# thunlp/OpenMatch

Measured on AMD Instinct MI355X. Metric: passages/sec encode (bert-base DPR bi-encoder, 128 tok -> 768-d) [+ queries/sec exact top-1000 over 8.8M x 768 in `search`], higher is better.
Workload: dtype f16; 1 GPU; bert-base DPR bi-encoder encode+search, MS MARCO 8.8M x 128-tok -> 768-d (BASELINE configs[1]); seq_len=128, global_batch=1024, index_rows=8841823, queries=6980, topk=1000, weights=random-init BertConfig() seed 0, parallelism=shard1

## Files before the change

### include/openmatch_hip.h

```cpp
#ifndef OPENMATCH_HIP_H
#define OPENMATCH_HIP_H

#include <stddef.h>
#include <stdint.h>

#ifdef __cplusplus
extern "C" {
#endif

#define OM_ABI_VERSION 6

#define OM_F32 0
#define OM_BF16 1
#define OM_F16 2

#define OM_ACT_NONE 0
#define OM_ACT_GELU_ERF 1
#define OM_ACT_RELU 2
#define OM_ACT_GELU_TANH 3
#define OM_ACT_SILU 5
#define OM_ACT_MUL_RESID 0x100
#define OM_ACT_PRE_GRAD 0x200

#define OM_ARCH_BERT 0
#define OM_ARCH_T5 1
#define OM_ARCH_MODERNBERT 2

#define OM_ARCH_CAUSAL 3

#define OM_ARCH_NOMICBERT 4

#define OM_POOL_NONE 0
#define OM_POOL_FIRST 1
#define OM_POOL_MEAN 2
#define OM_POOL_LAST 3

#define OM_SEARCH_F32 0
#define OM_SEARCH_F16_RESCORE 1

const char* om_last_error(void);
int om_abi_version(void);

int om_device_count(void);

#define OM_TIMING_GEMM_BF16 0
#define OM_TIMING_GEMM_F32 1
#define OM_TIMING_SCAN 2
void om_debug_gemm_trace(unsigned long long* buf);
void om_debug_gemm_gen(int gen);
#define OM_GEMM_FAMILY_V1 1
#define OM_GEMM_FAMILY_V2 2
#define OM_GEMM_FAMILY_V6 6
#define OM_GEMM_FAMILY_G7 7
#define OM_GEMM_FAMILY_G7_ONE_TILE 70
#define OM_GEMM_FAMILY_G7C16 71
#define OM_GEMM_FAMILY_G7R16 72
#define OM_GEMM_FAMILY_SKINNY 9
int om_debug_gemm_last(void);
int om_debug_gemm_plan(int in_dtype, const void* A, int64_t lda, const void* B, int64_t ldb, int out_dtype, void* C, int64_t ldc,
                       int64_t M, int64_t N, int64_t K, const float* bias, const void* resid, int64_t ldr, int act);
typedef struct OmDebugGemmEpilogue {
  const float* bias; const void* resid; int64_t ldr; int act;
  void* pre_act; int64_t ldp; float drop_p; uint64_t seed; const int* drop_rows;
  const float* ln_stats; const float* ln_colsum; const float* rln_stats; const float* rln_g; const float* rln_b; float* stats_out;
  const void* resid_lo; void* out_lo;
  const float* resid32; float* out32;
  const float* a_ln32; const float* a_ln_g; const float* a_ln_b; float* a_ln_stats_out; const float* rln32; const float* rln32_stats;
  int lo8; float ln_inv_h, ln_eps; int ln_rms; int reverse;
  const int* rows_dev;
} OmDebugGemmEpilogue;
int om_debug_gemm_ex(int in_dtype, const void* A, int64_t lda, const void* B, int64_t ldb, int out_dtype, void* C, int64_t ldc,
                     int64_t M, int64_t N, int64_t K, const OmDebugGemmEpilogue* ep, void* stream);
int om_debug_gemm_plan_ex(int in_dtype, const void* A, int64_t lda, const void* B, int64_t ldb, int out_dtype, void* C, int64_t ldc,
                          int64_t M, int64_t N, int64_t K, const OmDebugGemmEpilogue* ep);
int om_debug_gemm_splitk(int in_dtype, const void* A, int64_t lda, const void* B, int64_t ldb, float* C, int64_t ldc, int64_t M,
                         int64_t N, int64_t K, void* stream);
#define OM_OPT_ENCODER_FUSED_LN 0
#define OM_OPT_ENCODER_DEBUG 1
#define OM_OPT_ATTENTION_FAST 2
#define OM_OPT_SCAN_GEN7 3
#define OM_OPT_SCAN_GROWTH 4
#define OM_OPT_WGRAD_DEBUG 5
#define OM_OPT_GEMM_GROUP_M 6
#define OM_OPT_SCAN_QGROUP 7
#define OM_OPT_TRAIN_WGRAD_STREAM 8
#define OM_OPT_ATTENTION_DEBUG 9
#define OM_OPT_ENCODER_PINGPONG 10
#define OM_OPT_ENCODER_TWO_PLANE 11
#define OM_OPT_GEMM_VARIANT 12
#define OM_OPT_SEARCH_DEBUG 13
#define OM_OPT_TRAIN_WGRAD_BATCH 14
#define OM_OPT_GEMM_MAX_GRID 15
#define OM_OPT_GEMM_CONT 16
#define OM_OPT_TRAIN_TAPE_GRAD 17
#define OM_OPT_TRAIN_RES32 18
#define OM_OPT_GEMM_SKINNY_M 19
#define OM_OPT_GEMM_SKINNY_CFG 20
#define OM_OPT_FEW_ROWS_LN_FUSE 21
#define OM_OPT_ENCODER_SKIP_PAD 22
#define OM_OPT_ENCODER_CLS_TAIL 23
#define OM_OPT_COUNT 24
int om_debug_option(int opt, int value);
int om_debug_option_value(int opt);
int om_debug_attention(const void* qkv, void* ctx, const int64_t* mask, int64_t B, int L, int H, int heads, void* stream);
int om_debug_attention_ex(int dtype, const void* qkv, void* ctx, const int64_t* mask, const float* pos_bias, int64_t B, int L, int H,
                          int heads, float scale, float drop_p, uint64_t seed, void* stream, int reverse, const int* kmax,
                          const int* cu, int w);
int om_debug_rope(int dtype, void* qkv, int64_t M, int L, int H, float theta, void* stream);
int om_debug_rope_rows(int dtype, void* qkv, int64_t rows, int L, int H, float theta, const int* row_map, void* stream);
int om_debug_swiglu_rows(int dtype, const void* in, void* out, int64_t M, int F, void* stream);
int om_debug_embed(int dtype, const int64_t* ids, const int64_t* type_ids, const float* word, const float* pos, const float* type,
                   const float* g, const float* b, void* out, int64_t M, int L, int H, int vocab, int type_vocab, float eps, void* stream);
int om_debug_attention_causal(int dtype, const void* qkv, void* ctx, const int64_t* mask, int64_t B, int L, int n_heads, int n_kv_heads,
                              float scale, void* stream);
int om_debug_rope_gqa(int dtype, void* qkv, int64_t M, int L, int n_heads, int n_kv_heads, const float* inv_freq, float scaling, void* stream);
int om_debug_attention_causal_packed(int dtype, const void* qkv, void* ctx, const int64_t* mask, const int* cu, int64_t B, int L, int n_heads,
                                     int n_kv_heads, float scale, void* stream);
int om_debug_rope_gqa_rows(int dtype, void* qkv, int64_t rows, int L, int n_heads, int n_kv_heads, const float* inv_freq, float scaling,
                           const int* row_map, void* stream);
int om_debug_attention_causal_hd(int dtype, const void* qkv, void* ctx, const int64_t* mask, int64_t B, int L, int n_heads, int n_kv_heads,
                                 int head_dim, float scale, void* stream);
int om_debug_attention_causal_hd_packed(int dtype, const void* qkv, void* ctx, const int64_t* mask, const int* cu, int64_t B, int L,
                                        int n_heads, int n_kv_heads, int head_dim, float scale, void* stream);
int om_debug_qknorm_rope(int dtype, void* qkv, int64_t M, int L, int n_heads, int n_kv_heads, int head_dim, const float* q_norm_g,
                         const float* k_norm_g, float eps, const float* inv_freq, float scaling, void* stream);
int om_debug_qknorm_rope_rows(int dtype, void* qkv, int64_t rows, int L, int n_heads, int n_kv_heads, int head_dim, const float* q_norm_g,
                              const float* k_norm_g, float eps, const float* inv_freq, float scaling, const int* row_map, void* stream);
int om_debug_attention_gqa_d256(int dtype, const void* qkv, void* ctx, const int64_t* mask, int64_t B, int L, int n_heads, int n_kv_heads,
                                float scale, int w, void* stream);
int om_debug_qknorm_rope_d256(int dtype, void* qkv, int64_t M, int L, int n_heads, int n_kv_heads, const float* q_norm_g, const float* k_norm_g,
                              float eps, const float* inv_freq, float scaling, void* stream);
int om_debug_attention_gqa_d256_packed(int dtype, const void* qkv, void* ctx, const int64_t* mask, const int* cu, int64_t B, int L, int n_heads,
                                       int n_kv_heads, float scale, int w, void* stream);
int om_debug_qknorm_rope_d256_rows(int dtype, void* qkv, int64_t rows, int L, int n_heads, int n_kv_heads, const float* q_norm_g,
                                   const float* k_norm_g, float eps, const float* inv_freq, float scaling, const int* row_map, void* stream);
int om_debug_rmsnorm_add(int dtype, const void* h, int64_t ldh, float* x, int64_t ldx, const float* g, int64_t M, int H, float eps, void* stream);
int om_debug_mask_extent(const int64_t* mask, int64_t B, int L, int* kmax, void* stream);
int om_debug_pack_rows(const int* kmax, int64_t B, int L, int64_t rows, int* cu, int* cls_rows, int* row_map, void* stream);
#define OM_ATTN_FAMILY_GENERIC 1
#define OM_ATTN_FAMILY_FWD16 2
#define OM_ATTN_FAMILY_FWD16_KMAX4 3
#define OM_ATTN_FAMILY_FWD16C 4
#define OM_ATTN_FAMILY_LONG 5
#define OM_ATTN_FAMILY_D32 6
#define OM_ATTN_FAMILY_BAND16 7
#define OM_ATTN_FAMILY_BAND32 8
int om_debug_attention_last(void);
int om_debug_attention_plan(int dtype, int64_t B, int L, int H, int heads, int has_bias, float drop_p, int has_kmax, int has_cu, int w);
#define OM_ATTN_BWD_FAMILY_BWD16 1
#define OM_ATTN_BWD_FAMILY_GENERIC 2
#define OM_ATTN_BWD_FAMILY_LONG 3
#define OM_ATTN_BWD_FAMILY_D32 4
int om_debug_attention_bwd_last(void);
int om_debug_attention_bwd_plan(int dtype, int64_t B, int L, int H, int heads, int has_bias, int has_drel, int has_cu, int packed);
int om_debug_attention_bwd_ex(int dtype, const void* qkv, const void* ctx, const void* dctx, void* dqkv, const int64_t* mask,
                              const float* pos_bias, float* drel, float* stats, int64_t B, int L, int H, int heads, float scale,
                              float drop_p, uint64_t seed, const int* cu, int packed, void* stream);
size_t om_debug_attention_bwd_stats_bytes(int64_t B, int heads);
#define OM_ENC_PATH_BERT_FUSED 1
#define OM_ENC_PATH_BERT_PENDING_LN 2
#define OM_ENC_PATH_BERT_FEW32 3
#define OM_ENC_PATH_BERT_PLAIN 4
#define OM_ENC_PATH_MODERNBERT 5
#define OM_ENC_PATH_T5_FUSED 6
#define OM_ENC_PATH_T5_PLAIN 7
struct OmEncoderConfig;
int om_debug_encoder_plan(const struct OmEncoderConfig* cfg, int gated_ffn, int has_rel_bias, int64_t B, int64_t L, int64_t packed_rows,
                          int want_hidden);
int om_debug_encoder_skip_pad(const struct OmEncoderConfig* cfg, int gated_ffn, int has_rel_bias, int64_t B, int64_t L, int want_hidden);
int om_debug_encoder_cls_tail(const struct OmEncoderConfig* cfg, int gated_ffn, int has_rel_bias, int64_t B, int64_t L, int64_t packed_rows,
                              int want_hidden);
int om_debug_gather_rows(const void* src0, void* dst0, const void* src1, void* dst1, const void* src2, void* dst2, const float* stats_src,
                         float* stats_dst, const int* rows, int64_t B, int64_t L, int64_t Mc, int H, void* stream);
int om_debug_attn_drop_keep(uint64_t seed, int64_t b, int h, int heads, int Lm, int q, int key, float p);
int om_debug_wave_sum_check(const float* in, float* out_shuffle, float* out_dpp, int64_t groups, void* stream);
#define OM_ROW_FWD_GENERIC 1
#define OM_ROW_FWD_X8 2
#define OM_ROW_LN_BWD 3
int om_debug_row_kernel_last(void);
int om_debug_layernorm(int dtype, const void* x, int64_t ldx, void* y, int64_t ldy, const float* g, const float* b, int64_t M, int H,
                       float eps, int rms, const void* x_lo, int lo8, void* stream);
int om_debug_layernorm_f32out(int dtype, const void* x, int64_t ldx, float* y, int64_t ldy, const float* g, const float* b, int64_t M,
                              int H, float eps, int rms, const void* x_lo, const int* rows, int lo8, void* stream);
int om_debug_layernorm_from_f32(int dtype, const float* x, int64_t ldx, void* y, int64_t ldy, const float* g, const float* b, int64_t M,
                                int H, float eps, int rms, void* stream);
int om_debug_layernorm_dual(int dtype, const float* x, int64_t ldx, void* y, float* y32, int64_t ldy, const float* g, const float* b,
                            int64_t M, int H, float eps, void* stream);
int om_debug_norm_bwd(int dtype, const void* dy, const void* x, const float* g, void* dx, float* dg, float* db, int64_t M, int H,
                      float eps, int rms, const void* add, void* stream);
int om_debug_ln_bwd_drop(int dtype, const void* dy, const void* x, const float* g, void* dx, void* dx_drop, float drop_p,
                         uint64_t drop_seed, float* dg, float* db, int64_t M, int H, float eps, const float* dy32, const float* x32,
                         float* partial, int* partial_blocks , const int* drop_rows, void* stream);
typedef struct OmLnSite { const float* partial; float* dg; float* db; int blocks; } OmLnSite;
int om_debug_ln_param_reduce(const OmLnSite* sites , int n, int H, void* stream);
int om_debug_embed_bwd(int dtype, const void* dy, const int64_t* ids, const int64_t* type_ids, const float* word, const float* pos,
                       const float* type, const float* g, float* dword, float* dpos, float* dtype_, float* dg, float* db, int64_t M,
                       int L, int H, int vocab, int type_vocab, float eps, const int* cu, void* stream);
int om_debug_pool(int dtype, const void* x, const int64_t* mask, float* out, int64_t B, int L, int H, int mode, const int* cu,
                  void* stream);
int om_debug_pool_bwd(int dtype, const float* dp, const int64_t* mask, void* dh, int64_t B, int L, int H, int mode, const int* cu,
                      void* stream);
int om_debug_l2norm(const float* x, float* y, int64_t M, int D, void* stream);
int om_debug_l2norm_bwd(const float* x, const float* dy, float* dx, int64_t M, int D, void* stream);
int om_debug_colsum(int dtype, const void* x, int64_t ld, int64_t M, int N, float* out, void* stream);
int om_debug_dropout(int dtype, const void* x, void* y, int64_t n, float p, uint64_t seed, const int* rows, int H, void* stream);
int om_debug_ln_fold(int dtype, const void* W, const float* gamma, const float* beta, const float* b, void* Wf, float* colsum,
                     float* bf, int N, int K, void* stream);
int om_debug_ln_stats_reduce(const float* slots, int nslots, int64_t M, float* out, void* stream);
int om_kernel_timing_enable(int enable);
int om_kernel_timing_read(int kernel_class, double* total_ms, int64_t* launches, double* flops);

int om_gemm_nt(int in_dtype, const void* A, int64_t lda, const void* B, int64_t ldb,
               int out_dtype, void* C, int64_t ldc, int64_t M, int64_t N, int64_t K,
               const float* bias, const void* resid, int64_t ldr, int act, void* stream);

int om_gemm_tn_acc(int in_dtype, const void* A, int64_t lda, const void* B, int64_t ldb,
                   float* C, int64_t ldc, float* bias, int64_t M, int64_t N, int64_t K, void* stream);

typedef struct OmTnProblem {
  const void* A; const void* B; float* C; float* bias;
  int64_t lda, ldb, ldc, N, K;
} OmTnProblem;
int om_gemm_tn_acc_batch(int in_dtype, const OmTnProblem* problems, int n, int64_t M, void* stream);

typedef struct OmLayerWeights {
  const void* qkv_w;
  const float* qkv_b;
  const void* o_w;
  const float* o_b;
  const float* ln1_g;
  const float* ln1_b;
  const void* ffn1_w;
  const float* ffn1_b;
  const void* ffn1g_w;
  const void* ffn2_w;
  const float* ffn2_b;
  const float* ln2_g;
  const float* ln2_b;
} OmLayerWeights;

typedef struct OmEncoderConfig {
  int arch;
  int dtype;
  int hidden;
  int n_layers;
  int n_heads;
  int head_dim;
  int ffn;
  int vocab;
  int max_pos;
  int type_vocab;
  int act;
  float ln_eps;
  int rel_buckets;
  int rel_max_dist;
  int pooling;
  int head_in;
  int head_out;
  int normalize;
  float rope_theta_global;
  float rope_theta_local;
  int half_window;
  uint64_t sliding_layers;
} OmEncoderConfig;

typedef struct OmEncoderWeights {
  const float* word_emb;
  const float* pos_emb;
  const float* type_emb;
  const float* emb_ln_g;
  const float* emb_ln_b;
  const OmLayerWeights* layers_host;
  const float* final_ln_g;
  const float* rel_bias;
  const float* head_w;
  const void* folded;
  const float* final_ln_b;
} OmEncoderWeights;

size_t om_encoder_fold_bytes(const OmEncoderConfig* cfg);
int om_encoder_fold_weights(const OmEncoderConfig* cfg, const OmEncoderWeights* w, void* folded, size_t bytes, void* stream);

size_t om_encoder_workspace_bytes(const OmEncoderConfig* cfg, int64_t B, int64_t L);

int om_t5_relative_bucket(int relative_position, int num_buckets, int max_distance);

int om_encoder_forward(const OmEncoderConfig* cfg, const OmEncoderWeights* w,
                       const int64_t* input_ids, const int64_t* attention_mask,
                       const int64_t* token_type_ids, int64_t B, int64_t L,
                       void* out_hidden, float* out_reps, void* workspace,
                       size_t workspace_bytes, void* stream);

int om_encoder_packed_supported(const OmEncoderConfig* cfg, int gated_ffn, int64_t B, int64_t L, int64_t packed_rows);
size_t om_encoder_workspace_bytes_packed(const OmEncoderConfig* cfg, int64_t B, int64_t L, int64_t packed_rows);
int om_encoder_forward_packed(const OmEncoderConfig* cfg, const OmEncoderWeights* w,
                              const int64_t* input_ids, const int64_t* attention_mask,
                              const int64_t* token_type_ids, int64_t B, int64_t L, int64_t packed_rows,
                              float* out_reps, void* workspace, size_t workspace_bytes, void* stream);

typedef struct OmCausalConfig {
  OmEncoderConfig base;
  int n_kv_heads;
  float rope_attention_scaling;
  float inv_freq[32];
} OmCausalConfig;
size_t om_causal_encoder_workspace_bytes(const OmCausalConfig* cfg, int64_t B, int64_t L);
int om_causal_encoder_forward(const OmCausalConfig* cfg, const OmEncoderWeights* w, const int64_t* input_ids,
                              const int64_t* attention_mask, int64_t B, int64_t L, void* out_hidden, float* out_reps,
                              void* workspace, size_t workspace_bytes, void* stream);
int om_causal_encoder_packed_supported(const OmCausalConfig* cfg, int64_t B, int64_t L, int64_t packed_rows);
size_t om_causal_encoder_workspace_bytes_packed(const OmCausalConfig* cfg, int64_t B, int64_t L, int64_t packed_rows);
int om_causal_encoder_forward_packed(const OmCausalConfig* cfg, const OmEncoderWeights* w, const int64_t* input_ids,
                                     const int64_t* attention_mask, int64_t B, int64_t L, int64_t packed_rows, float* out_reps,
                                     void* workspace, size_t workspace_bytes, void* stream);

typedef struct OmCausalConfig2 {
  OmCausalConfig base;
  int qk_norm;
  int reserved;
  float inv_freq[64];
} OmCausalConfig2;
typedef struct OmCausalQkNorm {
  const float* q_norm_g;
  const float* k_norm_g;
} OmCausalQkNorm;
size_t om_causal2_encoder_workspace_bytes(const OmCausalConfig2* cfg, int64_t B, int64_t L);
int om_causal2_encoder_forward(const OmCausalConfig2* cfg, const OmEncoderWeights* w, const OmCausalQkNorm* qk_norm_host,
                               const int64_t* input_ids, const int64_t* attention_mask, int64_t B, int64_t L, void* out_hidden,
                               float* out_reps, void* workspace, size_t workspace_bytes, void* stream);
int om_causal2_encoder_packed_supported(const OmCausalConfig2* cfg, int64_t B, int64_t L, int64_t packed_rows);
size_t om_causal2_encoder_workspace_bytes_packed(const OmCausalConfig2* cfg, int64_t B, int64_t L, int64_t packed_rows);
int om_causal2_encoder_forward_packed(const OmCausalConfig2* cfg, const OmEncoderWeights* w, const OmCausalQkNorm* qk_norm_host,
                                      const int64_t* input_ids, const int64_t* attention_mask, int64_t B, int64_t L, int64_t packed_rows,
                                      float* out_reps, void* workspace, size_t workspace_bytes, void* stream);

#define OM_ARCH_GEMMA3 5
typedef struct OmGemma3Config {
  OmCausalConfig base;
  float attn_scale;
  int half_window;
  uint64_t sliding_layers;
  float full_scaling;
  float sliding_scaling;
  float attn_logit_softcapping;
  int bidirectional;
  float full_inv_freq[128];
  float sliding_inv_freq[128];
} OmGemma3Config;
typedef struct OmGemma3Norms {
  const float* q_norm_g;
  const float* k_norm_g;
  const float* post_attention_norm_g;
  const float* post_feedforward_norm_g;
} OmGemma3Norms;
size_t om_gemma3_encoder_workspace_bytes(const OmGemma3Config* cfg, int64_t B, int64_t L);
int om_gemma3_encoder_forward(const OmGemma3Config* cfg, const OmEncoderWeights* w, const OmGemma3Norms* norms_host, const int64_t* input_ids,
                              const int64_t* attention_mask, int64_t B, int64_t L, void* out_hidden, float* out_reps, void* workspace,
                              size_t workspace_bytes, void* stream);
int om_gemma3_encoder_packed_supported(const OmGemma3Config* cfg, int64_t B, int64_t L, int64_t packed_rows);
size_t om_gemma3_encoder_workspace_bytes_packed(const OmGemma3Config* cfg, int64_t B, int64_t L, int64_t packed_rows);
int om_gemma3_encoder_forward_packed(const OmGemma3Config* cfg, const OmEncoderWeights* w, const OmGemma3Norms* norms_host,
                                     const int64_t* input_ids, const int64_t* attention_mask, int64_t B, int64_t L, int64_t packed_rows,
                                     float* out_reps, void* workspace, size_t workspace_bytes, void* stream);

typedef struct OmT5DecoderLayer {
  const void* sa_v_w;
  const void* sa_o_w;
  const float* sa_ln_g;
  const void* ca_q_w;
  const void* ca_kv_w;
  const void* ca_o_w;
  const float* ca_ln_g;
  const void* ffn1_w;
  const void* ffn1g_w;
  const void* ffn2_w;
  const float* ffn_ln_g;
} OmT5DecoderLayer;
typedef struct OmT5DecoderWeights {
  const float* start_emb;
  const float* final_ln_g;
  const OmT5DecoderLayer* layers_host;
  int n_layers;
} OmT5DecoderWeights;
size_t om_t5_decoder_workspace_bytes(const OmEncoderConfig* cfg, int64_t B, int64_t L);
int om_t5_decoder_step(const OmEncoderConfig* cfg, const OmT5DecoderWeights* w, const void* enc_hidden,
                       const int64_t* attention_mask, int64_t B, int64_t L, float* out_hidden,
                       void* workspace, size_t workspace_bytes, void* stream);

typedef struct OmT5DecoderLayerGrads {
  float* sa_v_w;  float* sa_o_w; float* sa_ln_g;
  float* ca_q_w;  float* ca_kv_w; float* ca_o_w; float* ca_ln_g;
  float* ffn1_w;  float* ffn1g_w; float* ffn2_w; float* ffn_ln_g;
} OmT5DecoderLayerGrads;
typedef struct OmT5DecoderGrads {
  float* start_emb;
  float* final_ln_g;
  const OmT5DecoderLayerGrads* layers_host;
} OmT5DecoderGrads;
size_t om_t5_decoder_tape_bytes(const OmEncoderConfig* cfg, int n_layers, int64_t B, int64_t L);
size_t om_t5_decoder_train_workspace_bytes(const OmEncoderConfig* cfg, int n_layers, int64_t B, int64_t L);
int om_t5_decoder_train_forward(const OmEncoderConfig* cfg, const OmT5DecoderWeights* w, const void* enc_hidden,
                                const int64_t* attention_mask, int64_t B, int64_t L, float dropout, uint64_t seed,
                                void* tape, size_t tape_bytes, float* out_hidden, void* workspace,
                                size_t workspace_bytes, void* stream);
int om_t5_decoder_train_backward(const OmEncoderConfig* cfg, const OmT5DecoderWeights* w, const void* enc_hidden,
                                 const int64_t* attention_mask, int64_t B, int64_t L, float dropout, uint64_t seed,
                                 const void* tape, const float* d_out, const OmT5DecoderGrads* grads,
                                 void* d_enc_hidden, void* workspace, size_t workspace_bytes, void* stream);

int om_linear_f32_backward(const float* dy, const float* x, const float* w, float* dw, float* dx, int B, int D, int K,
                           void* stream);

typedef struct OmLayerGrads {
  float* qkv_w;  float* qkv_b;  float* o_w;    float* o_b;   float* ln1_g; float* ln1_b;
  float* ffn1_w; float* ffn1_b; float* ffn2_w; float* ffn2_b; float* ln2_g; float* ln2_b;
  float* ffn1g_w;
} OmLayerGrads;

typedef struct OmEncoderGrads {
  float* word_emb; float* pos_emb; float* type_emb; float* emb_ln_g; float* emb_ln_b;
  const OmLayerGrads* layers_host;
  float* head_w;
  float* final_ln_g;
  float* rel_bias;
} OmEncoderGrads;

size_t om_encoder_tape_bytes(const OmEncoderConfig* cfg, int64_t B, int64_t L);
size_t om_encoder_train_workspace_bytes(const OmEncoderConfig* cfg, int64_t B, int64_t L);

int om_encoder_train_forward(const OmEncoderConfig* cfg, const OmEncoderWeights* w,
                             const int64_t* input_ids, const int64_t* attention_mask,
                             const int64_t* token_type_ids, int64_t B, int64_t L,
                             float hidden_dropout, float attn_dropout, uint64_t seed, void* tape,
                             size_t tape_bytes, float* out_reps, void* workspace,
                             size_t workspace_bytes, void* stream);

int om_encoder_train_backward(const OmEncoderConfig* cfg, const OmEncoderWeights* w,
                              const int64_t* input_ids, const int64_t* attention_mask,
                              const int64_t* token_type_ids, int64_t B, int64_t L,
                              float hidden_dropout, float attn_dropout, uint64_t seed,
                              const void* tape, const float* d_reps, const OmEncoderGrads* grads,
                              void* workspace, size_t workspace_bytes, void* stream);

int om_encoder_train_packed_supported(const OmEncoderConfig* cfg, int64_t B, int64_t L, int64_t packed_rows);
size_t om_encoder_tape_bytes_packed(const OmEncoderConfig* cfg, int64_t B, int64_t L, int64_t packed_rows);
size_t om_encoder_train_workspace_bytes_packed(const OmEncoderConfig* cfg, int64_t B, int64_t L, int64_t packed_rows);
int om_encoder_train_forward_packed(const OmEncoderConfig* cfg, const OmEncoderWeights* w,
                                    const int64_t* input_ids, const int64_t* attention_mask,
                                    const int64_t* token_type_ids, int64_t B, int64_t L, int64_t packed_rows,
                                    float hidden_dropout, float attn_dropout, uint64_t seed,
                                    void* tape, size_t tape_bytes, float* out_reps,
                                    void* workspace, size_t workspace_bytes, void* stream);
int om_encoder_train_backward_packed(const OmEncoderConfig* cfg, const OmEncoderWeights* w,
                                     const int64_t* input_ids, const int64_t* attention_mask,
                                     const int64_t* token_type_ids, int64_t B, int64_t L, int64_t packed_rows,
                                     float hidden_dropout, float attn_dropout, uint64_t seed,
                                     const void* tape, const float* d_reps, const OmEncoderGrads* grads,
                                     void* workspace, size_t workspace_bytes, void* stream);

int om_encoder_train_forward_hidden(const OmEncoderConfig* cfg, const OmEncoderWeights* w,
                                    const int64_t* input_ids, const int64_t* attention_mask,
                                    const int64_t* token_type_ids, int64_t B, int64_t L,
                                    float hidden_dropout, float attn_dropout, uint64_t seed, void* tape,
                                    size_t tape_bytes, void* out_hidden, void* workspace,
                                    size_t workspace_bytes, void* stream);
int om_encoder_train_backward_hidden(const OmEncoderConfig* cfg, const OmEncoderWeights* w,
                                     const int64_t* input_ids, const int64_t* attention_mask,
                                     const int64_t* token_type_ids, int64_t B, int64_t L,
                                     float hidden_dropout, float attn_dropout, uint64_t seed,
                                     const void* tape, const void* d_hidden, const OmEncoderGrads* grads,
                                     void* workspace, size_t workspace_bytes, void* stream);

int om_encoder_train_set_layer_events(void* const* events, int n);

#define OM_ADAM_CHUNK 16384
typedef struct OmAdamTensor {
  float* p; const float* g; float* m; float* v;
  void* shadow0; void* shadow1;
  int64_t n;
  float weight_decay;
  int shadow0_dtype, shadow1_dtype, reserved;
} OmAdamTensor;
int om_grad_sqnorm(const OmAdamTensor* tensors, const int32_t* chunks, int n_chunks, float* partial, float* out_sq, void* stream);
int om_adamw_step(const OmAdamTensor* tensors, const int32_t* chunks, int n_chunks, float lr, float beta1, float beta2, float eps,
                  int64_t step, const float* gnorm_sq, float max_norm, float grad_scale, int skip_nonfinite,
                  const float* scale_state ,
                  void* stream);
int om_loss_scale_update(const float* gnorm_sq, float* state4, int growth_interval, void* stream);


int om_index_to_f16(const float* rows_f32, int64_t N, int d, void* rows_f16, float* stats,
                    void* stream);

size_t om_sim_topk_workspace_bytes(int64_t n_queries, int d, int k);

int om_sim_topk(int mode, const float* queries, int64_t n_queries, const float* index_f32,
                const void* index_f16, const float* stats, int64_t N, int d, int k,
                int64_t id_offset, float* out_scores, int64_t* out_ids, void* workspace,
                size_t workspace_bytes, void* stream);

void om_sim_topk_info(int64_t out[8]);

#define OM_SCAN_FAMILY_GENERIC 1
#define OM_SCAN_FAMILY_WIDE 2
#define OM_SCAN_FAMILY_STREAM32 3
#define OM_SCAN_FAMILY_STREAM16 4
int om_debug_scan_plan(int half, int64_t nq, int d, int out[4]);
int om_debug_sim_stream(const void* rows16, int64_t nrows, uint32_t row_base, const void* queries16, int64_t nq, int d, const float* thr,
                        uint64_t* keys, unsigned* cnt, int grid, void* stream);

int om_topk_merge(const float* part_scores, const int64_t* part_ids, int W, int64_t n_queries,
                  int k_in, int k_out, float* out_scores, int64_t* out_ids, void* stream);

int om_contrastive_fwd_bwd(const float* q, const float* p, int Qg, int Pg, int d, int n_psg,
                           float loss_scale, int q_row0, int q_rows, int p_row0, int p_rows,
                           float* loss, float* scores, float* d_q, float* d_p, float* workspace,
                           void* stream);

int om_contrastive_fwd_bwd_ex(const float* q, const float* p, int Qg, int Pg, int d, const int64_t* target, int n_psg,
                              int reduction, const float* row_grad, float loss_scale, int q_row0, int q_rows,
                              int p_row0, int p_rows, float* loss, float* scores, float* d_q, float* d_p,
                              float* workspace, void* stream);

#define OM_COMM_ID_BYTES 128
int om_comm_unique_id(void* id128);
int om_comm_init(const void* id128, int world, int rank, void** comm);
int om_comm_destroy(void* comm);
int om_comm_count(void* comm, int* count);
int om_allgather_rows(void* comm, const void* send, void* recv, int64_t rows, int64_t row_bytes, void* stream);
int om_allreduce_grads(void* comm, float* buf, int64_t n, int average, void* stream);
int om_exchange_topk(void* comm, int world, const float* D, const int64_t* I, int64_t q_block, int k, float* recvD,
                     int64_t* recvI, void* stream);

#ifdef __cplusplus
}
#endif
#endif
```

### openmatch_amd/csrc/abi.cpp

```cpp
#include "common.h"

static thread_local std::string g_last_error;
void om_set_error(const std::string& msg) { g_last_error = msg; }

extern "C" const char* om_last_error(void) { return g_last_error.c_str(); }
extern "C" int om_abi_version(void) { return OM_ABI_VERSION; }
extern "C" int om_device_count(void) {
  int n = 0;
  hipError_t e = hipGetDeviceCount(&n);
  if (e != hipSuccess) {
    om_set_error(std::string("hipGetDeviceCount: ") + hipGetErrorString(e));
    return -1;
  }
  return n;
}

#include <mutex>
#include <vector>
namespace {
struct Span { hipEvent_t a, b; };
struct ClassStat { std::vector<Span> spans; double flops = 0; size_t used = 0; };
bool g_timing = false;
ClassStat g_stat[3];
std::mutex g_mu;
}
bool om_timing_on() { return g_timing; }
void om_timing_begin(int c, hipStream_t s) {
  std::lock_guard<std::mutex> lk(g_mu);
  ClassStat& st = g_stat[c];
  if (st.used == st.spans.size()) {
    Span sp;
    (void)hipEventCreate(&sp.a);
    (void)hipEventCreate(&sp.b);
    st.spans.push_back(sp);
  }
  (void)hipEventRecord(st.spans[st.used].a, s);
}
void om_timing_end(int c, hipStream_t s, double flops) {
  std::lock_guard<std::mutex> lk(g_mu);
  ClassStat& st = g_stat[c];
  (void)hipEventRecord(st.spans[st.used].b, s);
  st.used++;
  st.flops += flops;
}
extern "C" int om_kernel_timing_enable(int enable) { g_timing = enable != 0; return 0; }
extern "C" int om_kernel_timing_read(int c, double* total_ms, int64_t* launches, double* flops) {
  if (c < 0 || c > 2) { om_set_error("om_kernel_timing_read: bad class"); return 1; }
  std::lock_guard<std::mutex> lk(g_mu);
  ClassStat& st = g_stat[c];
  double ms = 0;
  for (size_t i = 0; i < st.used; ++i) {
    hipError_t e = hipEventSynchronize(st.spans[i].b);
    float t = 0;
    if (e == hipSuccess) e = hipEventElapsedTime(&t, st.spans[i].a, st.spans[i].b);
    if (e != hipSuccess) { om_set_error(std::string("om_kernel_timing_read: ") + hipGetErrorString(e)); return 1; }
    ms += t;
  }
  if (total_ms) *total_ms = ms;
  if (launches) *launches = (int64_t)st.used;
  if (flops) *flops = st.flops;
  st.used = 0; st.flops = 0;
  return 0;
}

#include <atomic>
#include <map>
#include <tuple>
namespace {
std::atomic<int> g_opt[OM_OPT_COUNT];
std::atomic<bool> g_opt_init{false};
std::mutex g_opt_mu;
void opt_init() {
  std::lock_guard<std::mutex> lk(g_opt_mu);
  if (g_opt_init.load()) return;
  const char* e = getenv("OM_ENCODER_FUSED_LN");
  g_opt[OM_OPT_ENCODER_FUSED_LN] = e ? atoi(e) : 1;
  g_opt[OM_OPT_ENCODER_DEBUG] = getenv("OM_ENCODER_DEBUG") ? 1 : 0;
  e = getenv("OM_ATTENTION_FAST");
  g_opt[OM_OPT_ATTENTION_FAST] = e ? atoi(e) : 1;
  e = getenv("OM_SCAN_GEN7");
  g_opt[OM_OPT_SCAN_GEN7] = e ? atoi(e) : 1;
  e = getenv("OM_SCAN_GROWTH");
  g_opt[OM_OPT_SCAN_GROWTH] = e ? atoi(e) : 60;
  g_opt[OM_OPT_WGRAD_DEBUG] = 0;
  g_opt[OM_OPT_ATTENTION_DEBUG] = 0;
  e = getenv("OM_ENCODER_PINGPONG");
  g_opt[OM_OPT_ENCODER_PINGPONG] = e ? atoi(e) : 1;
  e = getenv("OM_TRAIN_WGRAD_STREAM");
  g_opt[OM_OPT_TRAIN_WGRAD_STREAM] = e ? atoi(e) : 1;
  e = getenv("OM_SCAN_QGROUP");
  g_opt[OM_OPT_SCAN_QGROUP] = e ? atoi(e) : 8;
  e = getenv("OM_GEMM_GROUP_M");
  g_opt[OM_OPT_GEMM_GROUP_M] = e ? atoi(e) : 8;
  e = getenv("OM_ENCODER_TWO_PLANE");
  g_opt[OM_OPT_ENCODER_TWO_PLANE] = e ? atoi(e) : 3;
  e = getenv("OM_GEMM_VARIANT");
  g_opt[OM_OPT_GEMM_VARIANT] = e ? atoi(e) : 0;
  e = getenv("OM_SEARCH_DEBUG");
  g_opt[OM_OPT_SEARCH_DEBUG] = e ? (atoi(e) ? atoi(e) : 1) : 0;
  e = getenv("OM_TRAIN_WGRAD_BATCH");
  g_opt[OM_OPT_TRAIN_WGRAD_BATCH] = e ? atoi(e) : 4;
  e = getenv("OM_GEMM_MAX_GRID");
  g_opt[OM_OPT_GEMM_MAX_GRID] = e ? atoi(e) : 0;
  e = getenv("OM_TRAIN_TAPE_GRAD");
  g_opt[OM_OPT_TRAIN_TAPE_GRAD] = e ? atoi(e) : 1;
  e = getenv("OM_TRAIN_RES32");
  g_opt[OM_OPT_TRAIN_RES32] = e ? atoi(e) : 1;
  e = getenv("OM_GEMM_CONT");
  g_opt[OM_OPT_GEMM_CONT] = e ? atoi(e) : 495;
  e = getenv("OM_GEMM_SKINNY_M");
  g_opt[OM_OPT_GEMM_SKINNY_M] = e ? atoi(e) : 1024;
  e = getenv("OM_FEW_ROWS_LN_FUSE");
  g_opt[OM_OPT_FEW_ROWS_LN_FUSE] = e ? atoi(e) : 64;
  e = getenv("OM_ENCODER_SKIP_PAD");
  g_opt[OM_OPT_ENCODER_SKIP_PAD] = e ? atoi(e) : 1;
  e = getenv("OM_ENCODER_CLS_TAIL");
  g_opt[OM_OPT_ENCODER_CLS_TAIL] = e ? atoi(e) : 1;
  g_opt_init.store(true);
}
}
bool om_option_is_set(int opt) {
  if (opt == OM_OPT_SCAN_GROWTH) return getenv("OM_SCAN_GROWTH") != nullptr;
  return false;
}
int om_option(int opt) {
  if (!g_opt_init.load(std::memory_order_acquire)) opt_init();
  return g_opt[opt].load(std::memory_order_relaxed);
}
extern "C" int om_debug_option(int opt, int value) {
  if (opt < 0 || opt >= OM_OPT_COUNT) { om_set_error("om_debug_option: unknown option"); return 1; }
  if (!g_opt_init.load(std::memory_order_acquire)) opt_init();
  g_opt[opt].store(value);
  return 0;
}
extern "C" int om_debug_option_value(int opt) {
  if (opt < 0 || opt >= OM_OPT_COUNT) { om_set_error("om_debug_option_value: unknown option"); return -1; }
  return om_option(opt);
}

int om_t5_lut_device(int L, int buckets, int max_dist, const int** out) {
  static std::mutex mu;
  static std::map<std::tuple<int, int, int, int>, int*> cache;
  int dev = 0;
  OM_HIP(hipGetDevice(&dev));
  std::lock_guard<std::mutex> lk(mu);
  auto key = std::make_tuple(dev, L, buckets, max_dist);
  auto it = cache.find(key);
  if (it == cache.end()) {
    std::vector<int> lut(2 * L);
    for (int rel = -(L - 1); rel <= L - 1; ++rel) lut[rel + (L - 1)] = om_t5_relative_bucket(rel, buckets, max_dist);
    int* d = nullptr;
    OM_HIP(hipMalloc(&d, (size_t)(2 * L) * sizeof(int)));
    OM_HIP(hipMemcpy(d, lut.data(), (size_t)(2 * L - 1) * sizeof(int), hipMemcpyHostToDevice));
    it = cache.emplace(key, d).first;
  }
  *out = it->second;
  return 0;
}
```

### openmatch_amd/csrc/encoder.hip

```cpp
#include <math.h>

#include <stdlib.h>

#include <algorithm>
#include <map>
#include <mutex>
#include <utility>
#include <vector>

#include "encoder_plan.h"

namespace {
struct FoldSlot { size_t w, cs, bf; };
struct FoldLayout { size_t per_layer, total; FoldSlot qkv, ffn1; };
FoldLayout fold_layout(const OmEncoderConfig* c) {
  const size_t H = c->hidden, F = enc_ffn1_cols(c);
  size_t off = 0;
  auto take = [&](size_t bytes) { size_t o = off; off = align_up(off + bytes, 256); return o; };
  FoldLayout L;
  L.qkv.w = take(3 * H * H * 2); L.qkv.cs = take(3 * H * 4); L.qkv.bf = take(3 * H * 4);
  L.ffn1.w = take(F * H * 2); L.ffn1.cs = take(F * 4); L.ffn1.bf = take(F * 4);
  L.per_layer = off;
  L.total = off * (size_t)c->n_layers;
  return L;
}
bool fold_applies(const OmEncoderConfig* c) {
  return c->arch != OM_ARCH_MODERNBERT && (c->dtype == OM_BF16 || c->dtype == OM_F16) && c->n_layers > 0 && c->hidden % 256 == 0 && c->ffn % 256 == 0;
}
}

extern "C" size_t om_encoder_fold_bytes(const OmEncoderConfig* cfg) {
  if (!cfg || !fold_applies(cfg)) return 0;
  return fold_layout(cfg).total;
}

extern "C" int om_encoder_fold_weights(const OmEncoderConfig* c, const OmEncoderWeights* w, void* blob, size_t bytes, void* stream) {
  if (!c || !w || !blob) OM_FAIL("null argument");
  if (!fold_applies(c)) OM_FAIL("nothing to fold for this configuration (om_encoder_fold_bytes is 0)");
  const FoldLayout L = fold_layout(c);
  if (bytes < L.total || ((uintptr_t)blob & 255)) OM_FAIL("fold buffer too small or not 256-byte aligned");
  const OmLayerWeights* Ls = w->layers_host;
  if (!Ls) OM_FAIL("layers_host is null");
  hipStream_t s = (hipStream_t)stream;
  const int H = c->hidden, F = enc_ffn1_cols(c);
  const bool bert = enc_bert_family(c);
  for (int l = 0; l < c->n_layers; ++l) {
    char* base = (char*)blob + (size_t)l * L.per_layer;
    const OmLayerWeights& lw = Ls[l];
    if (l > 0) {
      const float* g = bert ? Ls[l - 1].ln2_g : lw.ln1_g;
      const float* beta = bert ? Ls[l - 1].ln2_b : nullptr;
      if (omk_ln_fold(c->dtype, lw.qkv_w, g, beta, bert ? lw.qkv_b : nullptr, base + L.qkv.w, (float*)(base + L.qkv.cs),
                      (float*)(base + L.qkv.bf), 3 * H, H, s)) return 1;
    }
    if (!lw.ffn1g_w) {
      const float* g = bert ? lw.ln1_g : lw.ln2_g;
      const float* beta = bert ? lw.ln1_b : nullptr;
      if (omk_ln_fold(c->dtype, lw.ffn1_w, g, beta, bert ? lw.ffn1_b : nullptr, base + L.ffn1.w, (float*)(base + L.ffn1.cs),
                      (float*)(base + L.ffn1.bf), F, H, s)) return 1;
    }
  }
  return 0;
}

static int folded_weights(const OmEncoderConfig* c, const OmEncoderWeights* w, int layer, bool ffn1, const void* W, const float* g,
                          const float* beta, const float* b, int N, int K, void* scratch_w, float* scratch_cs, float* scratch_bf,
                          hipStream_t s, const void** Wf, const float** cs, const float** bf) {
  if (w->folded) {
    const FoldLayout L = fold_layout(c);
    const char* base = (const char*)w->folded + (size_t)layer * L.per_layer;
    const FoldSlot& sl = ffn1 ? L.ffn1 : L.qkv;
    *Wf = base + sl.w; *cs = (const float*)(base + sl.cs); *bf = (const float*)(base + sl.bf);
    return 0;
  }
  if (omk_ln_fold(c->dtype, W, g, beta, b, scratch_w, scratch_cs, scratch_bf, N, K, s)) return 1;
  *Wf = scratch_w; *cs = scratch_cs; *bf = scratch_bf;
  return 0;
}

struct EncWs {
  char *x, *y, *x1, *qkv, *ctx, *ff, *ff2;
  float *pooled, *headout, *posbias;
  float* final32;
  int* lut;
  int* kmax;
  int *cu, *cls_rows, *row_map;
  char* wfold;
  float *colsum, *bfold, *stats1, *stats2, *slots;
  char *y_lo, *x1_lo;
  float *r32a, *r32b, *y32;
  size_t total;
};

static EncWs carve(const OmEncoderConfig* c, const EncPlan& p, int64_t B, int64_t L, int64_t packed_rows, char* base) {
  const bool half = c->dtype == OM_BF16 || c->dtype == OM_F16;
  const size_t es = half ? 2 : 4;
  const size_t Mreal = (size_t)p.M, M = (size_t)p.Mp, H = c->hidden, F = c->ffn, F1 = enc_ffn1_cols(c);
  const bool bertf = enc_bert_family(c);
  size_t off = 0;
  auto take = [&](size_t bytes) { size_t o = off; off = align_up(off + bytes, 256); return base + o; };
  EncWs w;
  w.x = take(M * H * es);
  w.y = take(M * H * es);
  w.x1 = take(M * H * es);
  w.qkv = take(M * 3 * H * es);
  w.ctx = take(M * H * es);
  w.ff = take(M * F1 * es);
  w.ff2 = take(c->arch == OM_ARCH_T5 || c->arch == OM_ARCH_MODERNBERT || c->arch == OM_ARCH_NOMICBERT ? M * F * es : 0);
  w.pooled = (float*)take((size_t)B * H * 4);
  w.headout = (float*)take((size_t)B * (c->head_out > 0 ? c->head_out : 1) * 4);
  const bool rel = c->arch == OM_ARCH_T5 || (c->arch == OM_ARCH_BERT && c->rel_buckets > 0);
  w.posbias = (float*)take(rel ? (size_t)c->n_heads * L * L * 4 : 0);
  w.lut = (int*)take(rel ? (size_t)(2 * L) * 4 : 0);
  w.kmax = (int*)take((size_t)B * 4);
  w.cu = (int*)take(packed_rows > 0 ? (size_t)(B + 2) * 4 : 0);
  w.cls_rows = (int*)take(packed_rows > 0 ? (size_t)B * 4 : 0);
  w.row_map = (int*)take(packed_rows > 0 ? (size_t)packed_rows * 4 : 0);
  w.final32 = (float*)take(half && c->pooling != OM_POOL_NONE ? (c->pooling == OM_POOL_FIRST ? (size_t)B : Mreal) * H * 4 : 0);
  const bool fuse = half && c->arch != OM_ARCH_MODERNBERT;
  const size_t wide = std::max((size_t)3 * H, F1);
  w.wfold = take(fuse ? wide * H * es : 0);
  w.colsum = (float*)take(fuse ? wide * 4 : 0);
  w.bfold = (float*)take(fuse ? wide * 4 : 0);
  w.stats1 = (float*)take(fuse ? (size_t)2 * c->n_layers * M * 8 : 0);
  w.stats2 = w.stats1 ? w.stats1 + (size_t)c->n_layers * M * 2 : nullptr;
  w.slots = (float*)take(fuse ? (size_t)2 * ((H + 255) / 256) * M * 8 : 0);
  const bool two = fuse && bertf;
  w.y_lo = take(two ? M * H * es : 0);
  w.x1_lo = take(two ? M * H * es : 0);
  w.r32a = (float*)take(p.alloc_few32 ? Mreal * H * 4 : 0);
  w.r32b = (float*)take(p.alloc_few32 ? Mreal * H * 4 : 0);
  w.y32 = (float*)take(p.alloc_few32 ? Mreal * H * 4 : 0);
  w.total = off;
  return w;
}

static size_t workspace_bytes(const OmEncoderConfig* c, int64_t B, int64_t L, int64_t packed_rows) {
  const EncPlan p = encoder_plan_checked(EncPlanIn{c, B, L, packed_rows, false, false, false, false}, encoder_switches());
  return carve(c, p, B, L, packed_rows, nullptr).total;
}

extern "C" size_t om_encoder_workspace_bytes(const OmEncoderConfig* cfg, int64_t B, int64_t L) {
  if (!cfg || B <= 0 || L <= 0) return 0;
  return workspace_bytes(cfg, B, L, 0);
}

extern "C" size_t om_encoder_workspace_bytes_packed(const OmEncoderConfig* cfg, int64_t B, int64_t L, int64_t packed_rows) {
  if (!cfg || B <= 0 || L <= 0 || packed_rows <= 0) return 0;
  return workspace_bytes(cfg, B, L, packed_rows);
}

extern "C" int om_encoder_packed_supported(const OmEncoderConfig* c, int gated_ffn, int64_t B, int64_t L, int64_t packed_rows) {
  return encoder_packed_ok(c, gated_ffn != 0, B, L, packed_rows, encoder_switches()) ? 1 : 0;
}

extern "C" int om_debug_encoder_plan(const OmEncoderConfig* c, int gated_ffn, int has_rel_bias, int64_t B, int64_t L, int64_t packed_rows,
                                     int want_hidden) {
  if (!c) {
    om_set_error("om_debug_encoder_plan: null argument");
    return -1;
  }
  const EncPlan p = encoder_plan(EncPlanIn{c, B, L, packed_rows, want_hidden != 0, gated_ffn != 0, has_rel_bias != 0, c->type_vocab > 0},
                                 encoder_switches());
  if (p.error) {
    om_set_error(std::string("om_debug_encoder_plan: ") + p.error);
    return -1;
  }
  return p.path | (int)p.few_rows << 8 | (int)p.two << 9 | p.lo8 << 10;
}

extern "C" int om_debug_encoder_skip_pad(const OmEncoderConfig* c, int gated_ffn, int has_rel_bias, int64_t B, int64_t L, int want_hidden) {
  if (!c) {
    om_set_error("om_debug_encoder_skip_pad: null argument");
    return -1;
  }
  const EncPlanIn in = {c, B, L, 0, want_hidden != 0, gated_ffn != 0, has_rel_bias != 0, c->type_vocab > 0};
  const EncSwitches sw = encoder_switches();
  return encoder_skip_pad(in, encoder_plan(in, sw), sw) ? 1 : 0;
}

extern "C" int om_debug_encoder_cls_tail(const OmEncoderConfig* c, int gated_ffn, int has_rel_bias, int64_t B, int64_t L, int64_t packed_rows,
                                         int want_hidden) {
  if (!c) {
    om_set_error("om_debug_encoder_cls_tail: null argument");
    return -1;
  }
  const EncPlanIn in = {c, B, L, packed_rows, want_hidden != 0, gated_ffn != 0, has_rel_bias != 0, c->type_vocab > 0};
  const EncSwitches sw = encoder_switches();
  return encoder_cls_tail(in, encoder_plan(in, sw), sw) ? 1 : 0;
}

extern "C" int om_t5_relative_bucket(int relative_position, int num_buckets, int max_distance) {
  int nb = num_buckets / 2;
  int bucket = relative_position > 0 ? nb : 0;
  const int n = relative_position < 0 ? -relative_position : relative_position;
  const int max_exact = nb / 2;
  if (n < max_exact) return bucket + n;
  const double v = log((double)n / max_exact) / log((double)max_distance / max_exact) * (nb - max_exact);
  int large = max_exact + (int)v;
  if (large > nb - 1) large = nb - 1;
  return bucket + large;
}

static int check_cfg(const OmEncoderConfig* c) {
  if (const char* why = encoder_cfg_error(c)) OM_FAIL(why);
  return 0;
}

struct EncCall {
  const OmEncoderConfig* c;
  const OmEncoderWeights* w;
  const int64_t* mask;
  int64_t B, L;
  const EncPlan& p;
  const EncWs& ws;
  const float* posbias;
  const int* cu;
  const int* row_map;
  void* out_hidden;
  hipStream_t s;
  const int* rows_dev;
  int64_t cls_mc;
};

struct EncStream {
  const void* x;
  const void* x_lo;
  int lo8;
  const float *g, *b;
  int rms;
  void* spare;
  char* hidden;
  const float* rows32;
  bool cls_compact;
};

#define GEMM(A_, lda_, W_, ldw_, C_, ldc_, N_, K_, bias_, res_, ldr_, act_)                        \
  do {                                                                                             \
    if (om_gemm_nt(dt, A_, lda_, W_, ldw_, dt, C_, ldc_, Mg, N_, K_, bias_, res_, ldr_, act_, s)) \
      return 1;                                                                                    \
  } while (0)
#define RUN(expr) do { if (expr) return 1; } while (0)
#define ENC_LOCALS                                                                                                   \
  const OmEncoderConfig* c = k.c; const EncWs& ws = k.ws; const OmLayerWeights* Ls = k.w->layers_host; hipStream_t s = k.s;     \
  const int dt = c->dtype, H = c->hidden, F = c->ffn, nh = c->n_heads;                                              \
  const int64_t B = k.B, L = k.L, M = k.p.M, Mg = k.p.Mg
#define NOMIC_LOCALS                                                                                                 \
  const bool nomic = c->arch == OM_ARCH_NOMICBERT;                                                                   \
  const int F1 = enc_ffn1_cols(c), act1 = nomic ? OM_ACT_NONE : c->act;                                             \
  const void* const ffa = nomic ? ws.ff2 : ws.ff
#define NOMIC_ROPE() do { if (nomic) RUN(omk_rope(dt, ws.qkv, M, (int)L, H, c->rope_theta_global, s, k.row_map)); } while (0)
#define NOMIC_SWIGLU(rows_) do { if (nomic) RUN(omk_swiglu_rows(dt, ws.ff, ws.ff2, rows_, F, s)); } while (0)

static int bert_fused(const EncCall& k, EncStream* out) {
  ENC_LOCALS;
  NOMIC_LOCALS;
  const float scale = 1.0f / sqrtf((float)c->head_dim);
  const float inv_h = 1.0f / (float)H;
  const bool two = k.p.two;
  const int lo8 = k.p.lo8;
  const int nslots = 2 * (H / 256);
  const bool pingpong = k.p.pingpong;
  int walk = 1;
  const int64_t Mc = k.cls_mc;
  const size_t cplane = (size_t)Mc * H * 2;
  char* const cbase = ws.qkv;
  float* const cst2p = (float*)(cbase + 7 * cplane);
  float* const cst1 = cst2p + 2 * Mc;
  if (Mc > 0 && ((char*)(cst1 + 2 * Mc) > ws.qkv + (size_t)Mg * 3 * H * 2 || Mc > Mg || c->n_layers < 2 || lo8))
    OM_FAIL("[CLS] tail: the compact buffers do not fit the qkv area");
#define OM_WALK() (pingpong ? (walk ^= 1, walk ^ 1) : 0)
  for (int l = 0; l < c->n_layers; ++l) {
    const OmLayerWeights& lw = Ls[l];
    const bool last = l == c->n_layers - 1, tail = last && Mc > 0;
    float* st1 = tail ? cst1 : ws.stats1 + (size_t)l * Mg * 2;
    float* st2 = ws.stats2 + (size_t)l * Mg * 2;
    const float* st2p = l ? ws.stats2 + (size_t)(l - 1) * Mg * 2 : nullptr;
    const int64_t Mr = tail ? Mc : Mg;
    const int* const rdev = tail ? nullptr : k.rows_dev;
    const char *ctx = ws.ctx, *xin = ws.x1, *xin_lo = ws.x1_lo;
    char *y = ws.y, *y_lo = ws.y_lo, *xout = ws.x1, *xout_lo = ws.x1_lo;
    GemmEpilogue e = {};
    if (l == 0) {
      e.bias = lw.qkv_b; e.reverse = OM_WALK(); e.rows_dev = k.rows_dev;
      RUN(omk_gemm(dt, ws.x, H, lw.qkv_w, H, dt, ws.qkv, 3 * H, Mg, 3 * H, H, e, s));
    } else {
      const OmLayerWeights& pw = Ls[l - 1];
      const void* wf; const float *cs, *bfp;
      RUN(folded_weights(c, k.w, l, false, lw.qkv_w, pw.ln2_g, pw.ln2_b, lw.qkv_b, 3 * H, H, ws.wfold, ws.colsum, ws.bfold, s, &wf, &cs, &bfp));
      e.bias = bfp; e.ln_stats = st2p; e.ln_colsum = cs; e.ln_inv_h = inv_h; e.ln_eps = c->ln_eps; e.reverse = OM_WALK(); e.rows_dev = k.rows_dev;
      RUN(omk_gemm(dt, ws.x1, H, wf, H, dt, ws.qkv, 3 * H, Mg, 3 * H, H, e, s));
    }
    NOMIC_ROPE();
    RUN(omk_attention(dt, ws.qkv, ws.ctx, k.mask, k.posbias, B, (int)L, H, nh, scale, 0.f, 0, s, OM_WALK(), ws.kmax, k.cu));
    if (tail) {
      const GatherPlane planes[3] = {{ws.ctx, cbase}, {ws.x1, cbase + cplane}, {two ? ws.x1_lo : nullptr, cbase + 2 * cplane}};
      RUN(omk_gather_rows(planes, st2p, cst2p, k.cu ? ws.cls_rows : nullptr, B, L, Mc, H, s));
      ctx = cbase; xin = cbase + cplane; xin_lo = cbase + 2 * cplane; st2p = cst2p;
      y = cbase + 3 * cplane; y_lo = cbase + 4 * cplane; xout = cbase + 5 * cplane; xout_lo = cbase + 6 * cplane;
    }
    e = GemmEpilogue{};
    e.bias = lw.o_b; e.ldr = H; e.stats_out = ws.slots; e.ln_inv_h = inv_h; e.ln_eps = c->ln_eps;
    if (two) { e.out_lo = y_lo; e.lo8 = lo8; }
    if (l == 0) {
      e.resid = ws.x;
    } else {
      const OmLayerWeights& pw = Ls[l - 1];
      e.resid = xin; e.rln_stats = st2p; e.rln_g = pw.ln2_g; e.rln_b = pw.ln2_b;
      if (two) e.resid_lo = xin_lo;
    }
    e.reverse = OM_WALK(); e.rows_dev = rdev;
    RUN(omk_gemm(dt, ctx, H, lw.o_w, H, dt, y, H, Mr, H, H, e, s));
    RUN(omk_ln_stats_reduce(ws.slots, nslots, Mr, st1, s));
    const void* wf1; const float *cs1, *bf1;
    RUN(folded_weights(c, k.w, l, true, lw.ffn1_w, lw.ln1_g, lw.ln1_b, lw.ffn1_b, F1, H, ws.wfold, ws.colsum, ws.bfold, s, &wf1, &cs1, &bf1));
    e = GemmEpilogue{};
    e.bias = bf1; e.act = act1; e.ln_stats = st1; e.ln_colsum = cs1; e.ln_inv_h = inv_h; e.ln_eps = c->ln_eps;
    e.reverse = OM_WALK(); e.rows_dev = rdev;
    RUN(omk_gemm(dt, y, H, wf1, H, dt, ws.ff, F1, Mr, F1, H, e, s));
    NOMIC_SWIGLU(Mr);
    e = GemmEpilogue{};
    e.bias = lw.ffn2_b; e.resid = y; e.ldr = H; e.rln_stats = st1; e.rln_g = lw.ln1_g; e.rln_b = lw.ln1_b;
    e.stats_out = ws.slots; e.ln_inv_h = inv_h; e.ln_eps = c->ln_eps;
    if (two) { e.resid_lo = y_lo; e.out_lo = xout_lo; e.lo8 = lo8; }
    e.reverse = OM_WALK(); e.rows_dev = rdev;
    RUN(omk_gemm(dt, ffa, F, lw.ffn2_w, F, dt, xout, H, Mr, H, F, e, s));
    if (!last) RUN(omk_ln_stats_reduce(ws.slots, nslots, Mg, st2, s));
  }
#undef OM_WALK
  const OmLayerWeights& lastw = Ls[c->n_layers - 1];
  *out = EncStream{ws.x1, two ? ws.x1_lo : nullptr, lo8, lastw.ln2_g, lastw.ln2_b, 0, ws.x};
  if (Mc > 0) { out->x = cbase + 5 * cplane; out->x_lo = two ? cbase + 6 * cplane : nullptr; out->cls_compact = true; }
  return 0;
}

static int bert_pending_ln(const EncCall& k, EncStream* out) {
  ENC_LOCALS;
  NOMIC_LOCALS;
  const float scale = 1.0f / sqrtf((float)c->head_dim);
  float* const y_a = ws.y32;
  float* const y_b = ws.r32b;
  for (int l = 0; l < c->n_layers; ++l) {
    const OmLayerWeights& lw = Ls[l];
    float* const st1 = ws.stats1 + (size_t)l * M * 2;
    float* const st2p = l ? ws.stats2 + (size_t)(l - 1) * M * 2 : nullptr;
    GemmEpilogue e = {};
    e.bias = lw.qkv_b; e.ln_eps = c->ln_eps;
    if (l) { e.a_ln32 = y_b; e.a_ln_g = Ls[l - 1].ln2_g; e.a_ln_b = Ls[l - 1].ln2_b; e.a_ln_stats_out = st2p; }
    RUN(omk_gemm(dt, ws.x, H, lw.qkv_w, H, dt, ws.qkv, 3 * H, Mg, 3 * H, H, e, s));
    NOMIC_ROPE();
    RUN(omk_attention(dt, ws.qkv, ws.ctx, k.mask, k.posbias, B, (int)L, H, nh, scale, 0.f, 0, s, 0, ws.kmax));
    e = GemmEpilogue{};
    e.bias = lw.o_b; e.ldr = H; e.out32 = y_a; e.ln_eps = c->ln_eps;
    if (l) { e.rln32 = y_b; e.rln32_stats = st2p; e.rln_g = Ls[l - 1].ln2_g; e.rln_b = Ls[l - 1].ln2_b; }
    else e.resid32 = ws.r32a;
    RUN(omk_gemm(dt, ws.ctx, H, lw.o_w, H, dt, ws.y, H, Mg, H, H, e, s));
    e = GemmEpilogue{};
    e.bias = lw.ffn1_b; e.act = act1; e.ln_eps = c->ln_eps;
    e.a_ln32 = y_a; e.a_ln_g = lw.ln1_g; e.a_ln_b = lw.ln1_b; e.a_ln_stats_out = st1;
    RUN(omk_gemm(dt, ws.x1, H, lw.ffn1_w, H, dt, ws.ff, F1, Mg, F1, H, e, s));
    NOMIC_SWIGLU(Mg);
    e = GemmEpilogue{};
    e.bias = lw.ffn2_b; e.ldr = H; e.out32 = y_b; e.ln_eps = c->ln_eps;
    e.rln32 = y_a; e.rln32_stats = st1; e.rln_g = lw.ln1_g; e.rln_b = lw.ln1_b;
    RUN(omk_gemm(dt, ffa, F, lw.ffn2_w, F, dt, ws.y, H, Mg, H, F, e, s));
  }
  const OmLayerWeights& last = Ls[c->n_layers - 1];
  void* dst = k.out_hidden ? k.out_hidden : (void*)ws.x;
  RUN(omk_layernorm_dual(dt, y_b, H, dst, ws.r32a, H, last.ln2_g, last.ln2_b, M, H, c->ln_eps, s));
  *out = EncStream{};
  out->hidden = (char*)dst; out->rows32 = ws.r32a;
  return 0;
}

static int bert_few32(const EncCall& k, EncStream* out) {
  ENC_LOCALS;
  NOMIC_LOCALS;
  const float scale = 1.0f / sqrtf((float)c->head_dim);
  void* dst = ws.x;
  for (int l = 0; l < c->n_layers; ++l) {
    const OmLayerWeights& lw = Ls[l];
    GEMM(ws.x, H, lw.qkv_w, H, ws.qkv, 3 * H, 3 * H, H, lw.qkv_b, nullptr, 0, OM_ACT_NONE);
    NOMIC_ROPE();
    RUN(omk_attention(dt, ws.qkv, ws.ctx, k.mask, k.posbias, B, (int)L, H, nh, scale, 0.f, 0, s, 0, ws.kmax));
    GemmEpilogue e = {};
    e.bias = lw.o_b; e.resid32 = ws.r32a; e.ldr = H; e.out32 = ws.y32;
    RUN(omk_gemm(dt, ws.ctx, H, lw.o_w, H, dt, ws.y, H, Mg, H, H, e, s));
    RUN(omk_layernorm_dual(dt, ws.y32, H, ws.x1, ws.r32b, H, lw.ln1_g, lw.ln1_b, M, H, c->ln_eps, s));
    GEMM(ws.x1, H, lw.ffn1_w, H, ws.ff, F1, F1, H, lw.ffn1_b, nullptr, 0, act1);
    NOMIC_SWIGLU(Mg);
    e = GemmEpilogue{};
    e.bias = lw.ffn2_b; e.resid32 = ws.r32b; e.ldr = H; e.out32 = ws.y32;
    RUN(omk_gemm(dt, ffa, F, lw.ffn2_w, F, dt, ws.y, H, Mg, H, F, e, s));
    if (l == c->n_layers - 1 && k.out_hidden) dst = k.out_hidden;
    RUN(omk_layernorm_dual(dt, ws.y32, H, dst, ws.r32a, H, lw.ln2_g, lw.ln2_b, M, H, c->ln_eps, s));
  }
  *out = EncStream{};
  out->hidden = (char*)dst; out->rows32 = ws.r32a;
  return 0;
}

static int bert_plain(const EncCall& k, EncStream* out) {
  ENC_LOCALS;
  NOMIC_LOCALS;
  const float scale = 1.0f / sqrtf((float)c->head_dim);
  for (int l = 0; l < c->n_layers; ++l) {
    const OmLayerWeights& lw = Ls[l];
    if (l) RUN(omk_layernorm(dt, ws.y, H, ws.x, H, Ls[l - 1].ln2_g, Ls[l - 1].ln2_b, M, H, c->ln_eps, 0, s));
    GEMM(ws.x, H, lw.qkv_w, H, ws.qkv, 3 * H, 3 * H, H, lw.qkv_b, nullptr, 0, OM_ACT_NONE);
    NOMIC_ROPE();
    RUN(omk_attention(dt, ws.qkv, ws.ctx, k.mask, k.posbias, B, (int)L, H, nh, scale, 0.f, 0, s, 0, ws.kmax));
    GEMM(ws.ctx, H, lw.o_w, H, ws.y, H, H, H, lw.o_b, ws.x, H, OM_ACT_NONE);
    RUN(omk_layernorm(dt, ws.y, H, ws.x1, H, lw.ln1_g, lw.ln1_b, M, H, c->ln_eps, 0, s));
    GEMM(ws.x1, H, lw.ffn1_w, H, ws.ff, F1, F1, H, lw.ffn1_b, nullptr, 0, act1);
    NOMIC_SWIGLU(Mg);
    GEMM(ffa, F, lw.ffn2_w, F, ws.y, H, H, F, lw.ffn2_b, ws.x1, H, OM_ACT_NONE);
  }
  *out = EncStream{};
  if (c->n_layers > 0) *out = EncStream{ws.y, nullptr, 0, Ls[c->n_layers - 1].ln2_g, Ls[c->n_layers - 1].ln2_b, 0, ws.x};
  else out->hidden = ws.x;
  return 0;
}

static int modernbert(const EncCall& k, EncStream* out) {
  ENC_LOCALS;
  const float scale = 1.0f / sqrtf((float)c->head_dim);
  for (int l = 0; l < c->n_layers; ++l) {
    const OmLayerWeights& lw = Ls[l];
    if (!lw.ffn1g_w) OM_FAIL("ModernBERT layers need the gate half of Wi (ffn1g_w)");
    const void* a_in = ws.x;
    if (lw.ln1_g) {
      RUN(omk_layernorm(dt, ws.x, H, ws.y, H, lw.ln1_g, lw.ln1_b, M, H, c->ln_eps, 0, s));
      a_in = ws.y;
    }
    GEMM(a_in, H, lw.qkv_w, H, ws.qkv, 3 * H, 3 * H, H, lw.qkv_b, nullptr, 0, OM_ACT_NONE);
    const bool sliding = ((c->sliding_layers >> l) & 1) != 0;
    RUN(omk_rope(dt, ws.qkv, M, (int)L, H, sliding ? c->rope_theta_local : c->rope_theta_global, s));
    RUN(omk_attention(dt, ws.qkv, ws.ctx, k.mask, nullptr, B, (int)L, H, nh, scale, 0.f, 0, s, 0, ws.kmax, nullptr, sliding ? c->half_window : 0));
    GEMM(ws.ctx, H, lw.o_w, H, ws.x, H, H, H, lw.o_b, ws.x, H, OM_ACT_NONE);
    RUN(omk_layernorm(dt, ws.x, H, ws.y, H, lw.ln2_g, lw.ln2_b, M, H, c->ln_eps, 0, s));
    GEMM(ws.y, H, lw.ffn1g_w, H, ws.ff2, F, F, H, nullptr, nullptr, 0, OM_ACT_NONE);
    GEMM(ws.y, H, lw.ffn1_w, H, ws.ff, F, F, H, lw.ffn1_b, ws.ff2, F, c->act | OM_ACT_MUL_RESID);
    GEMM(ws.ff, F, lw.ffn2_w, F, ws.x, H, H, F, lw.ffn2_b, ws.x, H, OM_ACT_NONE);
  }
  *out = EncStream{ws.x, nullptr, 0, k.w->final_ln_g, k.w->final_ln_b, 0, ws.y};
  return 0;
}

static int t5_fused(const EncCall& k, EncStream* out) {
  ENC_LOCALS;
  const float inv_h = 1.0f / (float)H;
  const int nslots = 2 * (H / 256);
  auto folded = [&](int layer_, bool ffn1_, const void* A_, const void* W_, const float* g_, const float* stats_, void* C_, int N_, int act_,
                    const void* res_, int64_t ldr_) -> int {
    const void* wf; const float *cs, *bfp;
    if (folded_weights(c, k.w, layer_, ffn1_, W_, g_, nullptr, nullptr, N_, H, ws.wfold, ws.colsum, ws.bfold, s, &wf, &cs, &bfp)) return 1;
    (void)cs; (void)bfp;
    GemmEpilogue e = {};
    e.act = act_; e.resid = res_; e.ldr = ldr_;
    e.ln_stats = stats_; e.ln_rms = 1; e.ln_inv_h = inv_h; e.ln_eps = c->ln_eps; e.rows_dev = k.rows_dev;
    return omk_gemm(dt, A_, H, wf, H, dt, C_, N_, Mg, N_, H, e, s);
  };
  for (int l = 0; l < c->n_layers; ++l) {
    const OmLayerWeights& lw = Ls[l];
    float* st1 = ws.stats1 + (size_t)l * Mg * 2;
    float* st2 = ws.stats2 + (size_t)l * Mg * 2;
    if (l == 0) {
      RUN(omk_layernorm(dt, ws.x, H, ws.y, H, lw.ln1_g, nullptr, M, H, c->ln_eps, 1, s));
      GemmEpilogue e0 = {};
      e0.rows_dev = k.rows_dev;
      RUN(omk_gemm(dt, ws.y, H, lw.qkv_w, H, dt, ws.qkv, 3 * H, Mg, 3 * H, H, e0, s));
    } else {
      RUN(folded(l, false, ws.x, lw.qkv_w, lw.ln1_g, ws.stats2 + (size_t)(l - 1) * Mg * 2, ws.qkv, 3 * H, OM_ACT_NONE, nullptr, 0));
    }
    RUN(omk_attention(dt, ws.qkv, ws.ctx, k.mask, k.posbias, B, (int)L, H, nh, 1.0f, 0.f, 0, s, 0, ws.kmax, k.cu));
    GemmEpilogue e = {};
    e.resid = ws.x; e.ldr = H; e.stats_out = ws.slots; e.ln_inv_h = inv_h; e.ln_eps = c->ln_eps; e.rows_dev = k.rows_dev;
    RUN(omk_gemm(dt, ws.ctx, H, lw.o_w, H, dt, ws.x, H, Mg, H, H, e, s));
    RUN(omk_ln_stats_reduce(ws.slots, nslots, Mg, st1, s));
    RUN(folded(l, true, ws.x, lw.ffn1_w, lw.ln2_g, st1, ws.ff, F, c->act, nullptr, 0));
    e = GemmEpilogue{};
    e.resid = ws.x; e.ldr = H; e.stats_out = ws.slots; e.ln_inv_h = inv_h; e.ln_eps = c->ln_eps; e.rows_dev = k.rows_dev;
    RUN(omk_gemm(dt, ws.ff, F, lw.ffn2_w, F, dt, ws.x, H, Mg, H, F, e, s));
    RUN(omk_ln_stats_reduce(ws.slots, nslots, Mg, st2, s));
  }
  *out = EncStream{ws.x, nullptr, 0, k.w->final_ln_g, nullptr, 1, ws.y};
  return 0;
}

static int t5_plain(const EncCall& k, EncStream* out) {
  ENC_LOCALS;
  for (int l = 0; l < c->n_layers; ++l) {
    const OmLayerWeights& lw = Ls[l];
    RUN(omk_layernorm(dt, ws.x, H, ws.y, H, lw.ln1_g, nullptr, M, H, c->ln_eps, 1, s));
    GEMM(ws.y, H, lw.qkv_w, H, ws.qkv, 3 * H, 3 * H, H, nullptr, nullptr, 0, OM_ACT_NONE);
    RUN(omk_attention(dt, ws.qkv, ws.ctx, k.mask, k.posbias, B, (int)L, H, nh, 1.0f, 0.f, 0, s, 0, ws.kmax));
    GEMM(ws.ctx, H, lw.o_w, H, ws.x, H, H, H, nullptr, ws.x, H, OM_ACT_NONE);
    RUN(omk_layernorm(dt, ws.x, H, ws.y, H, lw.ln2_g, nullptr, M, H, c->ln_eps, 1, s));
    if (lw.ffn1g_w) {
      GEMM(ws.y, H, lw.ffn1g_w, H, ws.ff2, F, F, H, nullptr, nullptr, 0, OM_ACT_NONE);
      GEMM(ws.y, H, lw.ffn1_w, H, ws.ff, F, F, H, nullptr, ws.ff2, F, c->act | OM_ACT_MUL_RESID);
    } else {
      GEMM(ws.y, H, lw.ffn1_w, H, ws.ff, F, F, H, nullptr, nullptr, 0, c->act);
    }
    GEMM(ws.ff, F, lw.ffn2_w, F, ws.x, H, H, F, nullptr, ws.x, H, OM_ACT_NONE);
  }
  *out = EncStream{ws.x, nullptr, 0, k.w->final_ln_g, nullptr, 1, ws.y};
  return 0;
}

static int final_norm(const EncCall& k, const EncStream& n, char** hidden, const float** rows32, int64_t* n32) {
  const OmEncoderConfig* c = k.c; const EncWs& ws = k.ws; hipStream_t s = k.s;
  const int dt = c->dtype, H = c->hidden;
  const int64_t B = k.B, L = k.L, M = k.p.M;
  const bool pooled32 = dt != OM_F32 && c->pooling != OM_POOL_NONE;
  *hidden = n.hidden; *rows32 = ws.final32; *n32 = 0;
  if (!n.x) {
    if (n.rows32 && c->pooling != OM_POOL_NONE) { *rows32 = n.rows32; *n32 = M; }
    return 0;
  }
  if (k.out_hidden || !pooled32) {
    void* dst = k.out_hidden ? k.out_hidden : n.spare;
    RUN(omk_layernorm(dt, n.x, H, dst, H, n.g, n.b, M, H, c->ln_eps, n.rms, s, n.x_lo, n.lo8));
    *hidden = (char*)dst;
  }
  if (pooled32 && c->pooling == OM_POOL_FIRST) {
    const int* rows = k.cu && !n.cls_compact ? ws.cls_rows : nullptr;
    RUN(omk_layernorm_f32out(dt, n.x, rows || n.cls_compact ? H : L * H, ws.final32, H, n.g, n.b, B, H, c->ln_eps, n.rms, s, n.x_lo, rows, n.lo8));
    *n32 = B;
  } else if (pooled32) {
    RUN(omk_layernorm_f32out(dt, n.x, H, ws.final32, H, n.g, n.b, M, H, c->ln_eps, n.rms, s, n.x_lo, nullptr, n.lo8));
    *n32 = M;
  }
  return 0;
}

int omk_pooled_tail(const OmEncoderConfig* c, const OmEncoderWeights* w, const float* pooled, float* out_reps, int64_t B, const int* cu,
                    int64_t packed_rows, hipStream_t s) {
  int D = c->hidden;
  if (c->head_in > 0 && w->head_w) {
    D = c->head_out;
    RUN(om_gemm_nt(OM_F32, pooled, c->hidden, w->head_w, c->head_in, OM_F32, out_reps, D, B, D, c->head_in, nullptr, nullptr, 0, OM_ACT_NONE, s));
  }
  if (c->normalize) RUN(omk_l2norm(out_reps, out_reps, B, D, s));
  if (cu) RUN(omk_pack_overflow_poison(cu, B, packed_rows, out_reps, B * (int64_t)D, s));
  return 0;
}

static int skip_pad_buffer(hipStream_t s, size_t ints, int** out) {
  struct Buf { int* p = nullptr; size_t n = 0; bool captured = false; };
  static std::mutex mu;
  static std::map<std::pair<int, hipStream_t>, Buf> bufs;
  *out = nullptr;
  int dev = 0;
  OM_HIP(hipGetDevice(&dev));
  hipStreamCaptureStatus st = hipStreamCaptureStatusNone;
  if (hipStreamIsCapturing(s, &st) != hipSuccess) {
    (void)hipGetLastError();
    return 0;
  }
  const bool capturing = st != hipStreamCaptureStatusNone;
  std::lock_guard<std::mutex> lk(mu);
  Buf& b = bufs[std::make_pair(dev, s)];
  if (b.n < ints) {
    if (capturing) return 0;
    if (b.p && !b.captured) { OM_HIP(hipDeviceSynchronize()); OM_HIP(hipFree(b.p)); }
    b = Buf{};
    OM_HIP(hipMalloc(&b.p, ints * sizeof(int)));
    b.n = ints;
  }
  b.captured |= capturing;
  *out = b.p;
  return 0;
}

static int encoder_forward_impl(const OmEncoderConfig* c, const OmEncoderWeights* w,
                                const int64_t* input_ids, const int64_t* attention_mask,
                                const int64_t* token_type_ids, int64_t B, int64_t L,
                                void* out_hidden, float* out_reps, void* workspace,
                                size_t workspace_bytes, void* stream, int64_t packed_rows) {
  if (!c || !w || !input_ids || !attention_mask) OM_FAIL("null argument");
  if (check_cfg(c)) return 1;
  if (B <= 0) return 0;
  const OmLayerWeights* Ls = w->layers_host;
  if (!Ls) OM_FAIL("layers_host is null");
  const EncPlanIn plan_in = {c, B, L, packed_rows, out_hidden != nullptr, c->n_layers > 0 && Ls[0].ffn1g_w != nullptr, w->rel_bias != nullptr,
                             w->type_emb != nullptr};
  const EncSwitches sw = encoder_switches();
  const EncPlan plan = encoder_plan_checked(plan_in, sw);
  const bool bert = enc_bert_family(c);
  if (om_option(OM_OPT_ENCODER_DEBUG) && plan.path && bert)
    fprintf(stderr, "om_encoder_forward: M=%ld fused_ln=%d packed=%d few_rows=%d pending_ln=%d L=%ld head_dim=%d rel_bias=%d\n", (long)plan.M,
            (int)(plan.path == OM_ENC_PATH_BERT_FUSED), (int)(packed_rows > 0), (int)plan.few_rows, (int)(plan.path == OM_ENC_PATH_BERT_PENDING_LN), (long)L,
            c->head_dim, (int)plan.rel_bias);
  if (om_option(OM_OPT_ENCODER_DEBUG) && plan.path && c->arch == OM_ARCH_T5)
    fprintf(stderr, "om_encoder_forward (t5): M=%ld fused_norm=%d packed=%d\n", (long)plan.M, (int)(plan.path == OM_ENC_PATH_T5_FUSED), (int)(packed_rows > 0));
  if (plan.error) OM_FAIL(plan.error);
  if (c->arch == OM_ARCH_T5 && !w->final_ln_g) OM_FAIL("T5 needs rel_bias and final_ln_g");
  if (c->arch == OM_ARCH_MODERNBERT && (!w->emb_ln_g || !w->final_ln_g)) OM_FAIL("ModernBERT needs emb_ln_g and final_ln_g");
  if (c->arch == OM_ARCH_NOMICBERT && (!w->type_emb || w->pos_emb || w->rel_bias)) OM_FAIL("NomicBERT needs type_emb and takes no pos_emb or rel_bias");
  if (!workspace || ((uintptr_t)workspace & 255)) OM_FAIL("workspace must be 256-byte aligned");
  EncWs ws = carve(c, plan, B, L, packed_rows, (char*)workspace);
  if (ws.total > workspace_bytes) OM_FAIL("workspace too small");
  if (c->pooling != OM_POOL_NONE && !out_reps) OM_FAIL("out_reps required when pooling is set");
  hipStream_t s = (hipStream_t)stream;
  const int dt = c->dtype, H = c->hidden;
  const int64_t M = plan.M;
  int64_t pack_bound = packed_rows;
  bool skip = false;
  if (encoder_skip_pad(plan_in, plan, sw)) {
    int* side = nullptr;
    RUN(skip_pad_buffer(s, (size_t)(plan.Mp + 2 * B + 2), &side));
    if (side) {
      skip = true;
      pack_bound = plan.Mp;
      ws.cu = side; ws.cls_rows = side + (B + 2); ws.row_map = ws.cls_rows + B;
    }
  }
  const bool packed = pack_bound > 0;
  int64_t cls_mc = 0;
  if (!encoder_cls_tail(plan_in, plan, sw, &cls_mc)) cls_mc = 0;
  const int* const row_map = packed ? ws.row_map : nullptr;

  RUN(omk_mask_extent(attention_mask, B, (int)L, ws.kmax, s));
  if (packed) RUN(omk_pack_rows(ws.kmax, B, (int)L, pack_bound, ws.cu, ws.cls_rows, ws.row_map, s));
  if (plan.rel_bias) {
    const int* lut = nullptr;
    RUN(om_t5_lut_device((int)L, c->rel_buckets, c->rel_max_dist, &lut));
    RUN(omk_t5_bias(w->rel_bias, lut, ws.posbias, (int)L, c->n_heads, s));
  }
  const bool few32 = plan.path == OM_ENC_PATH_BERT_FEW32 || plan.path == OM_ENC_PATH_BERT_PENDING_LN;
  if (bert)
    RUN(omk_embed(dt, input_ids, token_type_ids, w->word_emb, w->pos_emb, w->type_emb, w->emb_ln_g, w->emb_ln_b, ws.x, M, (int)L, H,
                  c->vocab, c->type_vocab, c->ln_eps, 1, s, row_map, few32 ? ws.r32a : nullptr));
  else if (c->arch == OM_ARCH_MODERNBERT)
    RUN(omk_embed(dt, input_ids, nullptr, w->word_emb, nullptr, nullptr, w->emb_ln_g, w->emb_ln_b, ws.x, M, (int)L, H, c->vocab, 1, c->ln_eps, 1, s));
  else
    RUN(omk_embed(dt, input_ids, nullptr, w->word_emb, nullptr, nullptr, nullptr, nullptr, ws.x, M, (int)L, H, c->vocab, 1, c->ln_eps, 0, s, row_map));

  const EncCall k = {c, w, attention_mask, B, L, plan, ws, plan.rel_bias ? ws.posbias : nullptr, packed ? ws.cu : nullptr, row_map, out_hidden, s,
                     skip ? ws.cu + B : nullptr, cls_mc};
  EncStream stream_out = {};
  switch (plan.path) {
    case OM_ENC_PATH_BERT_FUSED: RUN(bert_fused(k, &stream_out)); break;
    case OM_ENC_PATH_BERT_PENDING_LN: RUN(bert_pending_ln(k, &stream_out)); break;
    case OM_ENC_PATH_BERT_FEW32: RUN(bert_few32(k, &stream_out)); break;
    case OM_ENC_PATH_BERT_PLAIN: RUN(bert_plain(k, &stream_out)); break;
    case OM_ENC_PATH_MODERNBERT: RUN(modernbert(k, &stream_out)); break;
    case OM_ENC_PATH_T5_FUSED: RUN(t5_fused(k, &stream_out)); break;
    case OM_ENC_PATH_T5_PLAIN: RUN(t5_plain(k, &stream_out)); break;
    default: OM_FAIL("no path planned");
  }
  char* final_hidden;
  const float* f32_rows;
  int64_t final32_rows;
  RUN(final_norm(k, stream_out, &final_hidden, &f32_rows, &final32_rows));

  if (c->pooling != OM_POOL_NONE) {
    float* pooled = c->head_in > 0 && w->head_w ? ws.pooled : out_reps;
    if (final32_rows == B && c->pooling == OM_POOL_FIRST && (f32_rows == ws.final32 || L == 1))
      OM_HIP(hipMemcpyAsync(pooled, f32_rows, (size_t)B * H * 4, hipMemcpyDeviceToDevice, s));
    else if (final32_rows == M)
      RUN(omk_pool(OM_F32, f32_rows, attention_mask, pooled, B, (int)L, H, c->pooling, s, k.cu));
    else
      RUN(omk_pool(dt, final_hidden, attention_mask, pooled, B, (int)L, H, c->pooling, s));
    RUN(omk_pooled_tail(c, w, pooled, out_reps, B, k.cu, pack_bound, s));
  }
  return 0;
}
#undef NOMIC_SWIGLU
#undef NOMIC_ROPE
#undef NOMIC_LOCALS
#undef ENC_LOCALS
#undef GEMM
#undef RUN

extern "C" int om_encoder_forward(const OmEncoderConfig* c, const OmEncoderWeights* w,
                                  const int64_t* input_ids, const int64_t* attention_mask,
                                  const int64_t* token_type_ids, int64_t B, int64_t L,
                                  void* out_hidden, float* out_reps, void* workspace,
                                  size_t workspace_bytes, void* stream) {
  return encoder_forward_impl(c, w, input_ids, attention_mask, token_type_ids, B, L, out_hidden, out_reps, workspace, workspace_bytes, stream, 0);
}

extern "C" int om_encoder_forward_packed(const OmEncoderConfig* c, const OmEncoderWeights* w,
                                         const int64_t* input_ids, const int64_t* attention_mask,
                                         const int64_t* token_type_ids, int64_t B, int64_t L, int64_t packed_rows,
                                         float* out_reps, void* workspace, size_t workspace_bytes, void* stream) {
  if (packed_rows <= 0) OM_FAIL("packed_rows must be positive");
  return encoder_forward_impl(c, w, input_ids, attention_mask, token_type_ids, B, L, nullptr, out_reps, workspace, workspace_bytes, stream, packed_rows);
}
```

### openmatch_amd/csrc/encoder_plan.h

```cpp
#pragma once
#include <algorithm>

#include "kernels.h"

bool omk_gemm_skinny_ok(int in_dtype, int out_dtype, int64_t M, int64_t N, int64_t K, const GemmEpilogue& ep, int max_m);

struct EncSwitches {
  int fused_ln;
  int two_plane;
  int pingpong;
  int skinny_m;
  int few_ln_fuse;
  int attention_fast;
  int skip_pad;
  int cls_tail;
};

static EncSwitches encoder_switches() {
  return EncSwitches{om_option(OM_OPT_ENCODER_FUSED_LN), om_option(OM_OPT_ENCODER_TWO_PLANE), om_option(OM_OPT_ENCODER_PINGPONG),
                     om_option(OM_OPT_GEMM_SKINNY_M), om_option(OM_OPT_FEW_ROWS_LN_FUSE), om_option(OM_OPT_ATTENTION_FAST),
                     om_option(OM_OPT_ENCODER_SKIP_PAD), om_option(OM_OPT_ENCODER_CLS_TAIL)};
}

struct EncPlanIn {
  const OmEncoderConfig* c;
  int64_t B, L, packed_rows;
  bool want_hidden;
  bool gated_ffn, has_rel_bias, has_type_emb;
};

struct EncPlan {
  int path;
  const char* error;
  int64_t M;
  int64_t Mp;
  int64_t Mg;
  bool few_rows;
  bool two;
  int lo8;
  bool pingpong;
  bool rel_bias;
  bool alloc_few32;
};

static const char* encoder_cfg_error(const OmEncoderConfig* c) {
  if (c->dtype != OM_F32 && c->dtype != OM_BF16 && c->dtype != OM_F16) return "dtype must be OM_F32, OM_BF16 or OM_F16";
  if (c->dtype == OM_F16 && c->arch == OM_ARCH_BERT && c->act != OM_ACT_GELU_ERF) return "float16 mode: erf-GELU BERT-family encoders only";
  if (c->dtype == OM_F16 && c->arch == OM_ARCH_T5 && c->act != OM_ACT_RELU && c->act != OM_ACT_GELU_TANH)
    return "float16 mode: T5 feed-forwards with ReLU or tanh-GELU only";
  if (c->arch != OM_ARCH_BERT && c->arch != OM_ARCH_T5 && c->arch != OM_ARCH_MODERNBERT && c->arch != OM_ARCH_NOMICBERT) return "unknown arch";
  if (c->arch == OM_ARCH_NOMICBERT) {
    if (c->head_dim != 64 || c->n_heads * 64 != c->hidden) return "NomicBERT: only head_dim 64 with n_heads*64 == hidden is supported";
    if (c->act != OM_ACT_SILU) return "NomicBERT: hidden_act must be \"silu\"";
    if (!(c->rope_theta_global > 0.f)) return "NomicBERT: a positive rope theta";
    if (c->rel_buckets != 0) return "NomicBERT: no relative position bias (rel_buckets must be 0)";
    if (c->hidden % 64 || c->ffn % 64 || c->ffn < 64) return "NomicBERT: hidden and ffn must be multiples of 64";
  }
  if (c->arch == OM_ARCH_MODERNBERT) {
    if (c->head_dim != 64 || c->n_heads * 64 != c->hidden) return "ModernBERT: only head_dim 64 with n_heads*64 == hidden is supported";
    if (c->act != OM_ACT_GELU_ERF) return "ModernBERT: hidden_activation must be \"gelu\" (erf)";
    if (c->n_layers > 64) return "ModernBERT: at most 64 layers";
    if (!(c->rope_theta_global > 0.f) || !(c->rope_theta_local > 0.f) || c->half_window < 0)
      return "ModernBERT: positive rope thetas and a non-negative half window";
  }
  if (c->arch == OM_ARCH_T5 && (c->head_dim != 64 || c->n_heads * 64 != c->hidden))
    return "T5 encoders: only d_kv 64 with n_heads*64 == d_model is supported";
  if ((c->head_dim != 32 && c->head_dim != 64) || c->n_heads * c->head_dim != c->hidden)
    return "head_dim must be 32 or 64 with n_heads*head_dim == hidden";
  if (c->arch == OM_ARCH_BERT && c->rel_buckets != 0 && (c->rel_buckets < 4 || c->rel_buckets % 2 || c->rel_max_dist <= c->rel_buckets / 4))
    return "relative position bias: an even number of buckets >= 4 and a maximum distance beyond the exact buckets";
  const int es = c->dtype == OM_F32 ? 4 : 2;
  if ((c->hidden * es) % 128 || (c->ffn * es) % 128) return "hidden/ffn rows must be multiples of 128 bytes";
  if (c->head_in > 0 && ((c->head_in * 4) % 128 || c->head_in != c->hidden)) return "head_in must equal hidden";
  return nullptr;
}

static inline bool enc_bert_family(const OmEncoderConfig* c) { return c->arch == OM_ARCH_BERT || c->arch == OM_ARCH_NOMICBERT; }
static inline int enc_ffn1_cols(const OmEncoderConfig* c) { return c->arch == OM_ARCH_NOMICBERT ? 2 * c->ffn : c->ffn; }

static bool enc_ln_fusable(int dt, int64_t rows, int H, int F, int F1) {
  return omk_gemm_ln_fusable(dt, rows, H, H) && omk_gemm_ln_fusable(dt, rows, F1, H) && omk_gemm_ln_fusable(dt, rows, 3 * H, H) &&
         omk_gemm_ln_fusable(dt, rows, H, F);
}

static bool enc_pending_ln_ok(int dt, int64_t M, int H, int F, int F1, int act, int max_m) {
  static const float one = 1.f;
  GemmEpilogue a = {}, r = {};
  a.a_ln32 = &one; a.a_ln_g = &one; a.a_ln_b = &one;
  r.rln32 = &one; r.rln32_stats = &one; r.rln_g = &one; r.rln_b = &one; r.out32 = const_cast<float*>(&one);
  GemmEpilogue f = a;
  f.act = act;
  return omk_gemm_skinny_ok(dt, dt, M, 3 * (int64_t)H, H, a, max_m) && omk_gemm_skinny_ok(dt, dt, M, F1, H, f, max_m) &&
         omk_gemm_skinny_ok(dt, dt, M, H, H, r, max_m) && omk_gemm_skinny_ok(dt, dt, M, H, F, r, max_m);
}

static EncPlan encoder_plan_checked(const EncPlanIn& in, const EncSwitches sw) {
  const OmEncoderConfig* c = in.c;
  EncPlan p = {};
  auto run = [&](int path) { p.path = path; return p; };
  auto refuse = [&](const char* why) { p.error = why; return p; };
  const int dt = c->dtype, H = c->hidden, F = c->ffn, F1 = enc_ffn1_cols(c);
  const bool half = dt == OM_BF16 || dt == OM_F16, packed = in.packed_rows > 0, bert = enc_bert_family(c), nomic = c->arch == OM_ARCH_NOMICBERT;
  p.M = packed ? in.packed_rows : in.B * in.L;
  p.Mp = half && p.M >= 512 ? (p.M + 255) / 256 * 256 : p.M;
  p.alloc_few32 = half && bert && !packed && p.M <= (int64_t)std::max(0, sw.skinny_m);
  if (in.B <= 0) return p;
  if (in.L < 1 || in.L > 1024) return refuse("sequence length must be in [1,1024]");
  if (packed) {
    if (dt == OM_F32 || in.want_hidden || c->pooling == OM_POOL_NONE || c->n_layers < 1)
      return refuse("packed rows: 16-bit inference that returns representations only");
    if (in.packed_rows % 256 || in.packed_rows < 512 || in.packed_rows > in.B * in.L + 255)
      return refuse("packed_rows: a multiple of 256 in [512, B * L + 255]");
  }
  p.few_rows = !packed && half && p.M <= (int64_t)sw.skinny_m && !(dt == OM_BF16 && bert && p.M >= 512 && (sw.two_plane & 1) != 0);
  p.Mg = p.few_rows ? p.M : p.Mp;
  const bool fusable = sw.fused_ln != 0 && !p.few_rows && c->n_layers > 0 && H % 8 == 0 && enc_ln_fusable(dt, p.Mg, H, F, F1);
  if (c->arch == OM_ARCH_MODERNBERT) {
    if (packed) return refuse("packed rows: not for ModernBERT (om_encoder_packed_supported is 0)");
    return run(OM_ENC_PATH_MODERNBERT);
  }
  if (!bert) {
    if (!in.has_rel_bias) return refuse("T5 needs rel_bias and final_ln_g");
    p.rel_bias = true;
    p.path = fusable && !in.gated_ffn ? OM_ENC_PATH_T5_FUSED : OM_ENC_PATH_T5_PLAIN;
    if (packed && p.path != OM_ENC_PATH_T5_FUSED) return refuse("packed rows need the fused 16-bit path (T5: widths of 256, no gated feed-forward)");
    return p;
  }
  if (in.L > c->max_pos) return refuse(nomic ? "NomicBERT: sequence longer than max_pos (max_position_embeddings)" : "sequence longer than the position table");
  if (in.has_rel_bias != (c->rel_buckets > 0)) return refuse("relative position bias: rel_bias and rel_buckets must be set together");
  if (in.has_type_emb && c->type_vocab <= 0) return refuse("token types: a type_emb table needs type_vocab > 0");
  p.rel_bias = in.has_rel_bias;
  const bool plane = (sw.two_plane & (dt == OM_BF16 ? 1 : 2)) != 0;
  if (fusable && (c->act == OM_ACT_GELU_ERF || nomic)) {
    p.two = plane;
    p.lo8 = plane && dt == OM_F16 && (sw.two_plane & 4) ? 1 : 0;
    p.pingpong = sw.pingpong != 0;
    return run(OM_ENC_PATH_BERT_FUSED);
  }
  const bool few32 = p.few_rows && c->n_layers > 0 && plane;
  p.path = !few32 ? OM_ENC_PATH_BERT_PLAIN
           : p.M <= (int64_t)sw.few_ln_fuse && enc_pending_ln_ok(dt, p.Mg, H, F, F1, nomic ? OM_ACT_NONE : c->act, sw.skinny_m) ? OM_ENC_PATH_BERT_PENDING_LN
                                                                                                       : OM_ENC_PATH_BERT_FEW32;
  if (packed) return refuse("packed rows need the fused 16-bit path (hidden, ffn multiples of 256; erf-GELU)");
  return p;
}

static EncPlan encoder_plan(const EncPlanIn& in, const EncSwitches sw) {
  if (const char* why = encoder_cfg_error(in.c)) {
    EncPlan p = {};
    p.error = why;
    return p;
  }
  return encoder_plan_checked(in, sw);
}

static bool encoder_packed_ok(const OmEncoderConfig* c, bool gated_ffn, int64_t B, int64_t L, int64_t packed_rows, const EncSwitches sw) {
  if (!c || B <= 0 || packed_rows <= 0) return false;
  if ((c->dtype != OM_BF16 && c->dtype != OM_F16) || (!enc_bert_family(c) && c->arch != OM_ARCH_T5)) return false;
  if (B * L <= (int64_t)sw.skinny_m) return false;
  if (c->dtype == OM_BF16 && !sw.attention_fast) return false;
  if (c->arch == OM_ARCH_T5 && c->dtype == OM_F16 && c->act != OM_ACT_RELU) return false;
  OmEncoderConfig q = *c;
  q.pooling = OM_POOL_FIRST;
  q.max_pos = 1024;
  const bool rel = c->arch == OM_ARCH_T5 || c->rel_buckets > 0;
  const EncPlan p = encoder_plan_checked(EncPlanIn{&q, B, L, packed_rows, false, gated_ffn, rel, false}, sw);
  return p.path && !p.error;
}

static bool encoder_skip_pad(const EncPlanIn& in, const EncPlan& p, const EncSwitches sw) {
  if (!sw.skip_pad || in.packed_rows != 0 || in.want_hidden || in.c->pooling == OM_POOL_NONE) return false;
  if (p.error || (p.path != OM_ENC_PATH_BERT_FUSED && p.path != OM_ENC_PATH_T5_FUSED)) return false;
  return encoder_packed_ok(in.c, in.gated_ffn, in.B, in.L, p.Mp, sw);
}

static bool encoder_cls_tail(const EncPlanIn& in, const EncPlan& p, const EncSwitches sw, int64_t* Mc = nullptr) {
  if (!sw.cls_tail || p.error || p.path != OM_ENC_PATH_BERT_FUSED || p.lo8) return false;
  if (in.c->pooling != OM_POOL_FIRST || in.want_hidden || in.c->n_layers < 2 || in.B < 512) return false;
  const int64_t mc = (in.B + 255) / 256 * 256;
  if (4 * mc > p.Mp) return false;
  if (Mc) *Mc = mc;
  return true;
}
```

### openmatch_amd/csrc/gemm.hip

```cpp
#include "gemm_core2.h"
#include "gemm_epilogue.h"
#include "gemm_plan.h"

template <typename T, typename OutT>
__global__ __launch_bounds__(GEMM_THREADS) void gemm_nt_kernel(
    const T* __restrict__ A, int64_t lda, const T* __restrict__ B, int64_t ldb, OutT* C,
    int64_t ldc, int64_t M, int64_t N, int64_t K, GemmEpilogue ep, int group_m) {
  extern __shared__ __attribute__((aligned(16))) char smem[];
  const int64_t ntm = (M + GEMM_BM - 1) / GEMM_BM, ntn = (N + GEMM_BN - 1) / GEMM_BN;
  int64_t tm, tn;
  gemm_tile_coords(ntm, ntn, group_m, tm, tn);
  const int64_t m0 = tm * GEMM_BM, n0 = tn * GEMM_BN;
  f32x16_t acc[2][2];
  gemm_mainloop<T>(A, lda, B, ldb, M, N, K, m0, n0, smem, acc);

  const int lane = threadIdx.x & 63, wave = threadIdx.x >> 6;
  const int wm = wave >> 1, wn = wave & 1;
  const EpiScalars es(ep);
#define OM_V1_CALL(A, TR) store_direct<OutT, A, TR>(acc[0][0], acc[0][1], acc[1][0], acc[1][1], m0 + wm * 64, n0 + wn * 64, C, ldc, M, N, ep, es)
  OM_EPI_SWITCH(es.act, es.train, OM_V1_CALL)
#undef OM_V1_CALL
}

template <typename T>
__global__ __launch_bounds__(GEMM_THREADS) void gemm_nt_splitk_kernel(
    const T* __restrict__ A, int64_t lda, const T* __restrict__ B, int64_t ldb, float* __restrict__ C,
    int64_t ldc, int64_t M, int64_t N, int64_t K, int steps_per_slice) {
  extern __shared__ __attribute__((aligned(16))) char smem[];
  const int64_t ntn = (N + GEMM_BN - 1) / GEMM_BN;
  const int64_t m0 = (blockIdx.x / ntn) * GEMM_BM, n0 = (blockIdx.x % ntn) * GEMM_BN;
  f32x16_t acc[2][2];
  gemm_mainloop<T>(A, lda, B, ldb, M, N, K, m0, n0, smem, acc,
                   (int64_t)blockIdx.y * steps_per_slice * GEMM_ROW_BYTES, steps_per_slice);
  const int lane = threadIdx.x & 63, wave = threadIdx.x >> 6;
  const int wm = wave >> 1, wn = wave & 1;
#pragma unroll
  for (int ni = 0; ni < 2; ++ni) {
    const int64_t n = n0 + wn * 64 + ni * 32 + (lane & 31);
    if (n >= N) continue;
#pragma unroll
    for (int mi = 0; mi < 2; ++mi) {
      const int64_t mbase = m0 + wm * 64 + mi * 32 + 4 * (lane >> 5);
#pragma unroll
      for (int r = 0; r < 16; ++r) {
        const int64_t m = mbase + (r & 3) + 8 * (r >> 2);
        if (m < M) atomicAdd(C + m * ldc + n, acc[mi][ni][r]);
      }
    }
  }
}

template <typename T, typename OutT>
__global__ __launch_bounds__(G2_THREADS) void gemm_nt_kernel2(
    const T* __restrict__ A, int64_t lda, const T* __restrict__ B, int64_t ldb, OutT* C,
    int64_t ldc, int64_t M, int64_t N, int64_t K, GemmEpilogue ep, int group_m) {
  extern __shared__ __attribute__((aligned(16))) char smem[];
  int64_t m0, n0;
  g2_tile_coords(M, N, group_m, m0, n0);
  f32x16_t acc[2][2];
  unsigned long long* tr = ep.trace ? ep.trace + (size_t)blockIdx.x * 32 : nullptr;
  if (tr && threadIdx.x == 0) tr[0] = clock64();
  gemm_mainloop2<T>(A, lda, B, ldb, M, N, K, m0, n0, smem, acc, tr);
  if (tr && threadIdx.x == 0) tr[15] = clock64();

  const int lane = threadIdx.x & 63, wave = threadIdx.x >> 6;
  const int wm = wave >> 1, wn = wave & 1;
  const EpiScalars es(ep);
  const int64_t nc = n0 + wn * 64;
  const float b0 = (ep.bias && nc + (lane & 31) < N) ? ep.bias[nc + (lane & 31)] : 0.f;
  const float b1 = (ep.bias && nc + 32 + (lane & 31) < N) ? ep.bias[nc + 32 + (lane & 31)] : 0.f;
  char* region = smem + wave * (32 * PATCH_STRIDE);
  __syncthreads();
#define OM_V2_CALL(A, TR)                                                                                   \
  store_patch<OutT, A, TR>(acc[0][0], acc[0][1], b0, b1, m0 + wm * 64, nc, C, ldc, M, N, ep, es, region);    \
  store_patch<OutT, A, TR>(acc[1][0], acc[1][1], b0, b1, m0 + wm * 64 + 32, nc, C, ldc, M, N, ep, es, region)
  OM_EPI_SWITCH(es.act, es.train, OM_V2_CALL)
#undef OM_V2_CALL
  if (tr && threadIdx.x == 0) { tr[28] = clock64(); tr[29] = blockIdx.x; }
}

static thread_local int g_gemm_last = 0;
void omk_gemm_note(int family) { g_gemm_last = family; }
extern "C" int om_debug_gemm_last(void) { return g_gemm_last; }

OM_DEFINE_LAUNCHER(launch_gemm, gemm_nt_kernel, GEMM_THREADS, GEMM_LDS_BYTES, GEMM_BM, GEMM_BN, OM_GEMM_FAMILY_V1)
OM_DEFINE_LAUNCHER(launch_gemm2, gemm_nt_kernel2, G2_THREADS, G2_LDS_BYTES, G2_BM, G2_BN, OM_GEMM_FAMILY_V2)

static unsigned long long* g_trace = nullptr;
extern "C" void om_debug_gemm_trace(unsigned long long* buf) { g_trace = buf; }
unsigned long long* omk_debug_trace() { return g_trace; }
static int g_debug_gen = 0;
extern "C" void om_debug_gemm_gen(int gen) { g_debug_gen = gen; }

bool omk_gemm_ln_fusable(int dtype, int64_t M, int64_t N, int64_t K) { return g7_shape_ok(dtype, M, N, K, gemm_switches(g_debug_gen)); }

int omk_gemm_wide7_f16(const GemmPlan& p, const void* A, int64_t lda, const void* B, int64_t ldb, void* C, int64_t ldc, int64_t M,
                       int64_t N, int64_t K, const GemmEpilogue& ep, hipStream_t s);
int omk_gemm_wide7(const GemmPlan& p, const void* A, int64_t lda, const void* B, int64_t ldb, void* C, int64_t ldc, int64_t M,
                   int64_t N, int64_t K, const GemmEpilogue& ep, hipStream_t s);
int omk_gemm_skinny(int dtype, const void* A, int64_t lda, const void* W, int64_t ldw, void* C, int64_t ldc, int64_t M, int64_t N,
                    int64_t K, const GemmEpilogue& ep, hipStream_t s);

int omk_gemm(int in_dtype, const void* A, int64_t lda, const void* B, int64_t ldb, int out_dtype, void* C, int64_t ldc, int64_t M,
             int64_t N, int64_t K, const GemmEpilogue& ep_in, hipStream_t s) {
  GemmEpilogue ep = ep_in;
  ep.trace = g_trace, g_gemm_last = 0;
  const GemmPlan p = gemm_plan(in_dtype, (uintptr_t)A, lda, (uintptr_t)B, ldb, out_dtype, (uintptr_t)C, ldc, M, N, K, ep, gemm_switches(g_debug_gen));
  if (p.error) OM_FAIL(p.error);
#define OM_GEMM_GO(TI, TO)                                                                                      \
  return p.family == OM_GEMM_FAMILY_V2 ? launch_gemm2<TI, TO>(A, lda, B, ldb, C, ldc, M, N, K, ep, s)           \
                                       : launch_gemm<TI, TO>(A, lda, B, ldb, C, ldc, M, N, K, ep, s)
  switch (p.family) {
    case 0: return 0;
    case OM_GEMM_FAMILY_SKINNY: return omk_gemm_skinny(in_dtype, A, lda, B, ldb, C, ldc, M, N, K, ep, s);
    case OM_GEMM_FAMILY_G7: case OM_GEMM_FAMILY_G7_ONE_TILE: case OM_GEMM_FAMILY_G7C16: case OM_GEMM_FAMILY_G7R16:
      return in_dtype == OM_F16 ? omk_gemm_wide7_f16(p, A, lda, B, ldb, C, ldc, M, N, K, ep, s)
                                : omk_gemm_wide7(p, A, lda, B, ldb, C, ldc, M, N, K, ep, s);
    case OM_GEMM_FAMILY_V6:
      return in_dtype == OM_F32 ? omk_gemm_wide6_f32(in_dtype, A, lda, B, ldb, out_dtype, C, ldc, M, N, K, ep, s)
                                : omk_gemm_wide6_b16(in_dtype, A, lda, B, ldb, out_dtype, C, ldc, M, N, K, ep, s);
    case OM_GEMM_FAMILY_V1: case OM_GEMM_FAMILY_V2:
      if (in_dtype == OM_F16 && out_dtype == OM_F16) OM_GEMM_GO(f16_t, f16_t);
      if (in_dtype == OM_BF16 && out_dtype == OM_BF16) OM_GEMM_GO(bf16_t, bf16_t);
      if (in_dtype == OM_BF16 && out_dtype == OM_F32) OM_GEMM_GO(bf16_t, float);
      if (in_dtype == OM_F32 && out_dtype == OM_F32) OM_GEMM_GO(float, float);
      if (in_dtype == OM_F16 && out_dtype == OM_F32) OM_GEMM_GO(f16_t, float);
      if (in_dtype == OM_F32 && out_dtype == OM_BF16) return launch_gemm<float, bf16_t>(A, lda, B, ldb, C, ldc, M, N, K, ep, s);
  }
#undef OM_GEMM_GO
  OM_FAIL("the plan names no launcher");
}

extern "C" int om_debug_gemm_plan(int in_dtype, const void* A, int64_t lda, const void* B, int64_t ldb, int out_dtype, void* C,
                                  int64_t ldc, int64_t M, int64_t N, int64_t K, const float* bias, const void* resid, int64_t ldr, int act) {
  GemmEpilogue ep = {};
  ep.bias = bias; ep.resid = resid; ep.ldr = ldr; ep.act = act;
  const GemmPlan p = gemm_plan(in_dtype, (uintptr_t)A, lda, (uintptr_t)B, ldb, out_dtype, (uintptr_t)C, ldc, M, N, K, ep, gemm_switches(g_debug_gen));
  return p.error ? -1 : p.family;
}

static GemmEpilogue debug_epilogue(const OmDebugGemmEpilogue& d) {
  GemmEpilogue ep = {};
  ep.bias = d.bias; ep.resid = d.resid; ep.ldr = d.ldr; ep.act = d.act;
  ep.pre_act = d.pre_act; ep.ldp = d.ldp; ep.drop_p = d.drop_p; ep.seed = d.seed; ep.drop_rows = d.drop_rows;
  ep.ln_stats = d.ln_stats; ep.ln_colsum = d.ln_colsum; ep.rln_stats = d.rln_stats; ep.rln_g = d.rln_g; ep.rln_b = d.rln_b;
  ep.stats_out = d.stats_out;
  ep.resid_lo = d.resid_lo; ep.out_lo = d.out_lo;
  ep.resid32 = d.resid32; ep.out32 = d.out32;
  ep.a_ln32 = d.a_ln32; ep.a_ln_g = d.a_ln_g; ep.a_ln_b = d.a_ln_b; ep.a_ln_stats_out = d.a_ln_stats_out;
  ep.rln32 = d.rln32; ep.rln32_stats = d.rln32_stats;
  ep.lo8 = d.lo8; ep.ln_inv_h = d.ln_inv_h; ep.ln_eps = d.ln_eps; ep.ln_rms = d.ln_rms; ep.reverse = d.reverse;
  ep.rows_dev = d.rows_dev;
  return ep;
}
extern "C" int om_debug_gemm_ex(int in_dtype, const void* A, int64_t lda, const void* B, int64_t ldb, int out_dtype, void* C, int64_t ldc,
                                int64_t M, int64_t N, int64_t K, const OmDebugGemmEpilogue* ep, void* stream) {
  if (!ep) OM_FAIL("om_debug_gemm_ex: null epilogue");
  return omk_gemm(in_dtype, A, lda, B, ldb, out_dtype, C, ldc, M, N, K, debug_epilogue(*ep), (hipStream_t)stream);
}
extern "C" int om_debug_gemm_plan_ex(int in_dtype, const void* A, int64_t lda, const void* B, int64_t ldb, int out_dtype, void* C,
                                     int64_t ldc, int64_t M, int64_t N, int64_t K, const OmDebugGemmEpilogue* ep) {
  if (!ep) return -1;
  const GemmPlan p = gemm_plan(in_dtype, (uintptr_t)A, lda, (uintptr_t)B, ldb, out_dtype, (uintptr_t)C, ldc, M, N, K, debug_epilogue(*ep),
                               gemm_switches(g_debug_gen));
  return p.error ? -1 : p.family;
}

int omk_gemm_splitk(int in_dtype, const void* A, int64_t lda, const void* B, int64_t ldb, float* C,
                    int64_t ldc, int64_t M, int64_t N, int64_t K, hipStream_t s) {
  if (M <= 0 || N <= 0 || K <= 0) return 0;
  const int64_t es = in_dtype == OM_F32 ? 4 : 2;
  if ((K * es) % GEMM_ROW_BYTES != 0) OM_FAIL("K*sizeof(elem) must be a multiple of 128 bytes");
  const int64_t tiles = ((M + GEMM_BM - 1) / GEMM_BM) * ((N + GEMM_BN - 1) / GEMM_BN);
  const int nk = (int)(K * es / GEMM_ROW_BYTES);
  int slices = (int)((1024 + tiles - 1) / tiles);
  if (slices > nk / 4) slices = nk / 4 > 0 ? nk / 4 : 1;
  const int per = (nk + slices - 1) / slices;
  slices = (nk + per - 1) / per;
  static std::atomic<bool> attr_bf16{false}, attr_f32{false};
  const bool timing = om_timing_on();
  const int tclass = es == 2 ? OM_TIMING_GEMM_BF16 : OM_TIMING_GEMM_F32;
  if (timing) om_timing_begin(tclass, s);
  if (in_dtype == OM_BF16) {
    if (!attr_bf16) { OM_HIP(hipFuncSetAttribute((const void*)gemm_nt_splitk_kernel<bf16_t>, hipFuncAttributeMaxDynamicSharedMemorySize, GEMM_LDS_BYTES)); attr_bf16 = true; }
    hipLaunchKernelGGL((gemm_nt_splitk_kernel<bf16_t>), dim3((unsigned)tiles, slices), dim3(GEMM_THREADS), GEMM_LDS_BYTES, s,
                       (const bf16_t*)A, lda, (const bf16_t*)B, ldb, C, ldc, M, N, K, per);
  } else if (in_dtype == OM_F16) {
    static std::atomic<bool> attr_f16{false};
    if (!attr_f16) { OM_HIP(hipFuncSetAttribute((const void*)gemm_nt_splitk_kernel<f16_t>, hipFuncAttributeMaxDynamicSharedMemorySize, GEMM_LDS_BYTES)); attr_f16 = true; }
    hipLaunchKernelGGL((gemm_nt_splitk_kernel<f16_t>), dim3((unsigned)tiles, slices), dim3(GEMM_THREADS), GEMM_LDS_BYTES, s,
                       (const f16_t*)A, lda, (const f16_t*)B, ldb, C, ldc, M, N, K, per);
  } else if (in_dtype == OM_F32) {
    if (!attr_f32) { OM_HIP(hipFuncSetAttribute((const void*)gemm_nt_splitk_kernel<float>, hipFuncAttributeMaxDynamicSharedMemorySize, GEMM_LDS_BYTES)); attr_f32 = true; }
    hipLaunchKernelGGL((gemm_nt_splitk_kernel<float>), dim3((unsigned)tiles, slices), dim3(GEMM_THREADS), GEMM_LDS_BYTES, s,
                       (const float*)A, lda, (const float*)B, ldb, C, ldc, M, N, K, per);
  } else {
    OM_FAIL("unsupported dtype");
  }
  if (timing) om_timing_end(tclass, s, 2.0 * (double)M * (double)N * (double)K);
  OM_LAUNCH_CHECK();
  return 0;
}
extern "C" int om_debug_gemm_splitk(int in_dtype, const void* A, int64_t lda, const void* B, int64_t ldb, float* C, int64_t ldc, int64_t M,
                                    int64_t N, int64_t K, void* stream) {
  return omk_gemm_splitk(in_dtype, A, lda, B, ldb, C, ldc, M, N, K, (hipStream_t)stream);
}

extern "C" int om_gemm_nt(int in_dtype, const void* A, int64_t lda, const void* B, int64_t ldb,
                          int out_dtype, void* C, int64_t ldc, int64_t M, int64_t N, int64_t K,
                          const float* bias, const void* resid, int64_t ldr, int act,
                          void* stream) {
  GemmEpilogue ep = {};
  ep.bias = bias; ep.resid = resid; ep.ldr = ldr; ep.act = act;
  return omk_gemm(in_dtype, A, lda, B, ldb, out_dtype, C, ldc, M, N, K, ep, (hipStream_t)stream);
}
```

### openmatch_amd/csrc/gemm_plan.h

```cpp
#pragma once
#include "kernels.h"

bool omk_gemm_wide7_has(int act, bool resid, int lnf);
bool omk_gemm_wide7_f16_has(int act, bool resid, int lnf);
bool omk_gemm_wide7_train_ok(int64_t M, int64_t N, int64_t K, int64_t ldc, const GemmEpilogue& ep);
bool omk_gemm_skinny_ok(int in_dtype, int out_dtype, int64_t M, int64_t N, int64_t K, const GemmEpilogue& ep, int max_m);

struct GemmSwitches {
  int variant;
  int cont;
  int skinny_m;
  int debug_gen;
};

static GemmSwitches gemm_switches(int debug_gen) {
  return GemmSwitches{om_option(OM_OPT_GEMM_VARIANT), om_option(OM_OPT_GEMM_CONT), om_option(OM_OPT_GEMM_SKINNY_M), debug_gen};
}

static bool g7_ring_ok(int64_t K) { return K * 2 >= 3 * 128; }

static bool g7_shape_ok(int dtype, int64_t M, int64_t N, int64_t K, const GemmSwitches& sw) {
  return M >= 512 && gemm_whole_tiles(M, N, K) && sw.variant == 0 && (dtype == OM_F16 || (dtype == OM_BF16 && sw.debug_gen != 6));
}

static bool g7_admits(int dtype, bool wide, int64_t M, int64_t N, int64_t K, const GemmEpilogue& ep, const GemmPlan& p, const GemmSwitches& sw) {
  const bool f16 = dtype == OM_F16;
  if (!wide || !g7_shape_ok(dtype, M, N, K, sw) || p.train || ((uintptr_t)ep.bias & 15)) return false;
  if (ep.ln_stats && (ep.rln_stats || ep.stats_out)) return false;
  if (p.lnf >= 2 && !ep.stats_out) return false;
  if (p.resid && (ep.ldr * 2) % 128 != 0) return false;
  if (f16 && (ep.act & OM_ACT_MUL_RESID) && (p.lnf != 0 || !p.resid)) return false;
  return f16 ? omk_gemm_wide7_f16_has(p.act, p.resid, p.lnf) : omk_gemm_wide7_has(p.act, p.resid, p.lnf);
}

static int g7_kernel(int dtype, int64_t K, const GemmPlan& p, const GemmSwitches& sw) {
  if (sw.debug_gen == 70 && dtype == OM_BF16 && p.lnf == 0 && !p.resid && (p.act == OM_ACT_NONE || p.act == OM_ACT_GELU_ERF))
    return OM_GEMM_FAMILY_G7_ONE_TILE;
  const bool ring = g7_ring_ok(K);
  if (!p.resid && p.lnf <= 1 && ring && (sw.cont & 1)) return OM_GEMM_FAMILY_G7C16;
  if (p.resid && (p.lnf == 0 || p.lnf == 2) && ring && (sw.cont & 2)) return OM_GEMM_FAMILY_G7R16;
  if (p.lnf == 4) return ring ? OM_GEMM_FAMILY_G7R16 : 0;
  if (p.resid && p.lnf == 3 && ring && (sw.cont & (dtype == OM_BF16 ? 512 : 256))) return OM_GEMM_FAMILY_G7R16;
  return OM_GEMM_FAMILY_G7;
}

static GemmPlan gemm_plan(int in_dtype, uintptr_t A, int64_t lda, uintptr_t B, int64_t ldb, int out_dtype, uintptr_t C, int64_t ldc,
                          int64_t M, int64_t N, int64_t K, const GemmEpilogue ep, const GemmSwitches sw) {
  const bool f16 = in_dtype == OM_F16, b16 = f16 || in_dtype == OM_BF16;
  GemmPlan p = {0, nullptr, ep.act & 0xff, ep.resid != nullptr, ep.pre_act != nullptr || ep.drop_p > 0.f, gemm_lnf(ep, f16)};
  auto run = [&](int family) { p.family = family; return p; };
  auto refuse = [&](const char* why) { p.error = why; return p; };
  if (M <= 0 || N <= 0) return p;
  if (K <= 0) return refuse("K must be positive");
  const int64_t es = in_dtype == OM_F32 ? 4 : 2;
  if ((K * es) % 128 != 0) return refuse("K*sizeof(elem) must be a multiple of 128 bytes");
  if ((lda * es) % 16 != 0 || (ldb * es) % 16 != 0) return refuse("lda/ldb must keep rows 16-byte aligned");
  if ((A & 15) || (B & 15)) return refuse("A/B must be 16-byte aligned");
  if (p.act == OM_ACT_GELU_ERF_GRAD && !p.resid) return refuse("gelu-grad epilogue needs resid");
  if (sw.variant == 0 && sw.debug_gen == 0 && omk_gemm_skinny_ok(in_dtype, out_dtype, M, N, K, ep, sw.skinny_m)) return run(OM_GEMM_FAMILY_SKINNY);
  if (ep.resid32 || ep.out32 || ep.a_ln32 || ep.rln32) return refuse("f32 residual / f32 sum / pending-LayerNorm epilogue: the few-rows kernel only (gemm_skinny.hip)");
  if ((ep.out_lo || ep.resid_lo) && p.lnf < 3) return refuse("two-plane residual stream: only with the output-side LayerNorm epilogue");
  const int64_t vec = out_dtype == OM_F32 ? 4 : 8;
  const bool wide = sw.variant != 1 && M >= 512 && N % vec == 0 && ldc % vec == 0 && (C & 15) == 0 &&
                    (!p.resid || (ep.ldr % vec == 0 && ((uintptr_t)ep.resid & 15) == 0));
  int gen = 1;
  if (wide) {
    auto rounds = [&](int64_t bm, int64_t bn, int64_t slots) {
      const int64_t tiles = ((M + bm - 1) / bm) * ((N + bn - 1) / bn);
      return (double)((tiles + slots - 1) / slots);
    };
    const double c4 = N >= 256 ? rounds(256, 256, 256) * (256.0 * 256.0) / 1.00 : 1e30;
    const double c2 = rounds(256, 128, 256) * (256.0 * 128.0) / 0.92;
    const double c1 = rounds(128, 128, 512) * (2 * 128.0 * 128.0) / 0.70;
    gen = c4 <= c2 && c4 <= c1 ? 6 : (c2 <= c1 ? 2 : 1);
    if (sw.variant == 2) gen = 2;
    if (sw.variant == 6) gen = N >= 256 ? 6 : 2;
    const bool plain16 = (in_dtype == OM_BF16 || (f16 && (sw.cont & 128))) && out_dtype == in_dtype && !ep.pre_act && ep.drop_p == 0.f &&
                         gemm_whole_tiles(M, N, K) && g7_ring_ok(K);
    if ((sw.cont & 16) && plain16) gen = 6;
    if ((sw.cont & 64) && plain16 && gen == 2 && sw.variant == 0) {
      const double c7 = rounds(256, 256, 256) * (256.0 * 256.0), c2r = rounds(256, 128, 256) * (256.0 * 128.0) / 0.55;
      if (c7 < c2r) gen = 6;
    }
  }
  if (wide && b16 && out_dtype == in_dtype && sw.variant == 0 && sw.debug_gen != 6 && (sw.cont & 32) && omk_gemm_wide7_train_ok(M, N, K, ldc, ep))
    return run(OM_GEMM_FAMILY_G7C16);
  if (f16 && out_dtype == OM_F16) {
    if (g7_admits(in_dtype, wide, M, N, K, ep, p, sw) && (p.lnf != 0 || gen == 6 || !(sw.cont & 128))) {
      const int k7 = g7_kernel(in_dtype, K, p, sw);
      return k7 ? run(k7) : refuse("two-plane residual epilogue with the eight-bit plane: K >= 192");
    }
    if (p.lnf) return refuse("float16: the fused LayerNorm epilogues need whole 256 x 256 tiles");
    return run(wide && gen != 1 ? OM_GEMM_FAMILY_V2 : OM_GEMM_FAMILY_V1);
  }
  if (p.lnf && !(wide && in_dtype == OM_BF16 && out_dtype == OM_BF16 && N >= 256)) return refuse("fused LayerNorm epilogue needs the 256x256 bf16 kernel");
  if (p.lnf) gen = 6;
  if (gen == 6) {
    const bool aligned = (((uintptr_t)ep.bias & 15) == 0) && (ep.ldp % 2 == 0) && (((uintptr_t)ep.pre_act & 3) == 0);
    if (!aligned && p.lnf) return refuse("fused LayerNorm epilogue needs 16-byte aligned bias");
    if (!aligned) gen = 2;
    else if (in_dtype == OM_BF16 && out_dtype == OM_BF16 && g7_admits(in_dtype, wide, M, N, K, ep, p, sw)) return run(g7_kernel(in_dtype, K, p, sw));
    else if (p.lnf) return refuse("fused LayerNorm epilogue: whole 256 x 256 tiles of bf16, inference only (generation 7)");
    else if (omk_gemm_wide6_b16_has(in_dtype, out_dtype, p.act, p.train, p.resid) || omk_gemm_wide6_f32_has(in_dtype, out_dtype, p.act, p.train, p.resid))
      return run(OM_GEMM_FAMILY_V6);
    else gen = 2;
  }
  if (in_dtype == OM_F32 && out_dtype == OM_BF16) return run(OM_GEMM_FAMILY_V1);
  if (!(out_dtype == OM_F32 ? (in_dtype == OM_F32 || b16) : (in_dtype == OM_BF16 && out_dtype == OM_BF16))) return refuse("unsupported dtype combination");
  return run(gen == 2 ? OM_GEMM_FAMILY_V2 : OM_GEMM_FAMILY_V1);
}
```

### openmatch_amd/csrc/kernels.h

```cpp
#pragma once
#include "common.h"

int omk_ln_fold(int dtype , const void* W, const float* gamma, const float* beta, const float* b, void* Wf,
                float* colsum, float* bf, int N, int K, hipStream_t s);
int omk_layernorm(int dtype, const void* x, int64_t ldx, void* y, int64_t ldy, const float* g,
                  const float* b, int64_t M, int H, float eps, int rms, hipStream_t s,
                  const void* x_lo = nullptr ,
                  int lo8 = 0 );
int omk_layernorm_dual(int dtype, const float* x, int64_t ldx, void* y, float* y32, int64_t ldy, const float* g, const float* b,
                       int64_t M, int H, float eps, hipStream_t s);
int omk_layernorm_f32out(int dtype, const void* x, int64_t ldx, float* y, int64_t ldy, const float* g, const float* b,
                         int64_t M, int H, float eps, int rms, hipStream_t s, const void* x_lo = nullptr,
                         const int* rows = nullptr ,
                         int lo8 = 0 );
int omk_layernorm_from_f32(int dtype, const float* x, int64_t ldx, void* y, int64_t ldy, const float* g, const float* b, int64_t M, int H,
                           float eps, int rms, hipStream_t s);
int omk_embed(int dtype, const int64_t* ids, const int64_t* type_ids, const float* word,
              const float* pos, const float* type, const float* g, const float* b, void* out,
              int64_t M, int L, int H, int vocab, int type_vocab, float eps, int bert,
              hipStream_t s, const int* row_map = nullptr ,
              float* out32 = nullptr );
int omk_pool(int dtype, const void* x, const int64_t* mask, float* out, int64_t B, int L, int H,
             int mode, hipStream_t s, const int* cu = nullptr );
int omk_l2norm(const float* x, float* y, int64_t M, int D, hipStream_t s);
int omk_swiglu_rows(int dtype, const void* in, void* out, int64_t M, int F, hipStream_t s);
void omk_row_note(int word);
int omk_t5_bias(const float* table, const int* lut, float* out, int L, int heads, hipStream_t s);

int omk_attention(int dtype, const void* qkv, void* ctx, const int64_t* mask,
                  const float* pos_bias, int64_t B, int L, int H, int heads, float scale,
                  float drop_p, uint64_t seed, hipStream_t s, int reverse = 0 ,
                  const int* kmax = nullptr ,
                  const int* cu = nullptr ,
                  int w = 0 );
struct AttnPlan;
int omk_attention_d32(const AttnPlan& p, int dtype, const void* qkv, void* ctx, const int64_t* mask, const float* pos_bias, int64_t B, int L,
                      int H, int heads, float scale, float drop_p, uint64_t seed, hipStream_t s, int reverse, const int* kmax, const int* cu);
int omk_rope(int dtype, void* qkv, int64_t M, int L, int H, float theta, hipStream_t s,
             const int* row_map = nullptr );
int omk_attention_band(int dtype, const void* qkv, void* ctx, const int64_t* mask, int64_t B, int L, int H, int heads, float scale,
                       int w, const int* kmax, hipStream_t s);
int omk_rope_gqa(int dtype, void* qkv, int64_t M, int L, int heads, int kv_heads, const float* inv_freq_host, float scaling, hipStream_t s,
                 const int* row_map = nullptr );
int omk_attention_causal(int dtype, const void* qkv, void* ctx, const int64_t* mask, int64_t B, int L, int heads, int kv_heads, float scale,
                         const int* kmax, hipStream_t s);
int omk_attention_causal_packed(int dtype, const void* qkv, void* ctx, const int64_t* mask, int64_t B, int L, int heads, int kv_heads, float scale,
                                const int* cu, hipStream_t s);
int omk_attention_causal_d128(int dtype, const void* qkv, void* ctx, const int64_t* mask, int64_t B, int L, int heads, int kv_heads, float scale,
                              const int* kmax, hipStream_t s);
int omk_attention_causal_d128_packed(int dtype, const void* qkv, void* ctx, const int64_t* mask, int64_t B, int L, int heads, int kv_heads,
                                     float scale, const int* cu, hipStream_t s);
int omk_qknorm_rope(int dtype, void* qkv, int64_t M, int L, int heads, int kv_heads, int head_dim, const float* q_norm_g, const float* k_norm_g,
                    float eps, const float* inv_freq_host, float scaling, hipStream_t s, const int* row_map = nullptr,
                    int gemma = 0 );
int omk_attention_gqa_d256(int dtype, const void* qkv, void* ctx, const int64_t* mask, int64_t B, int L, int heads, int kv_heads, float scale, int w,
                           const int* kmax, hipStream_t s);
int omk_attention_gqa_d256_packed(int dtype, const void* qkv, void* ctx, const int64_t* mask, int64_t B, int L, int heads, int kv_heads, float scale,
                                  int w, const int* cu, hipStream_t s);
int omk_rmsnorm_add(int dtype, const void* h, int64_t ldh, float* x, int64_t ldx, const float* g, int64_t M, int H, float eps, hipStream_t s);
int omk_rope_table(const float* inv_freq, int n, float scaling, const float2** out);
int omk_causal_debug_kmax(int64_t B, int** out);
int omk_pack_rows(const int* kmax, int64_t B, int L, int64_t rows, int* cu, int* cls_rows, int* row_map, hipStream_t s);
int omk_pack_overflow_poison(const int* cu, int64_t B, int64_t rows, float* out, int64_t n, hipStream_t s);
int omk_mask_extent(const int64_t* mask, int64_t B, int L, int* kmax, hipStream_t s);
int omk_pooled_tail(const OmEncoderConfig* c, const OmEncoderWeights* w, const float* pooled, float* out_reps, int64_t B, const int* cu,
                    int64_t packed_rows, hipStream_t s);

#define OM_ACT_GELU_ERF_GRAD 4
struct GemmEpilogue {
  const float* bias;
  const void* resid;
  int64_t ldr;
  int act;
  void* pre_act;
  int64_t ldp;
  float drop_p;
  uint64_t seed;
  const int* drop_rows;
  unsigned long long* trace;
  const float* ln_stats;
  const float* ln_colsum;
  const float* rln_stats;
  const float* rln_g;
  const float* rln_b;
  float* stats_out;
  const void* resid_lo;
  void* out_lo;
  const float* resid32;
  float* out32;
  const float* a_ln32;
  const float* a_ln_g;
  const float* a_ln_b;
  float* a_ln_stats_out;
  const float* rln32;
  const float* rln32_stats;
  int lo8;
  float ln_inv_h, ln_eps;
  int ln_rms;
  int reverse;
  const int* rows_dev;
};
__host__ __device__ inline size_t omk_lo8_offset(int64_t m, int64_t n, int64_t N) {
  const int64_t tile = (m >> 8) * (N >> 8) + (n >> 8);
  const int wave = (int)(((m >> 7) & 1) * 2 + ((n >> 7) & 1));
  const int r = (int)(m & 127), c = (int)(n & 127);
  const int P = 2 * (r >> 5) + (c >> 6);
  const int G = 2 * ((r >> 4) & 1) + ((c >> 5) & 1);
  const int lane = ((c >> 2) & 3) * 16 + (r & 15);
  return ((size_t)((tile * 4 + wave) * 8 + P)) * 2048 + (size_t)((G >> 1) * 1024 + lane * 16 + (G & 1) * 8 + ((c >> 4) & 1) * 4 + (c & 3));
}
int omk_ln_stats_reduce(const float* slots, int nslots, int64_t M, float* out, hipStream_t s);
struct GatherPlane { const void* src; void* dst; };
int omk_gather_rows(const GatherPlane (&planes)[3], const float* stats_src, float* stats_dst, const int* rows, int64_t B, int64_t L, int64_t Mc,
                    int H, hipStream_t s);
struct GemmPlan { int family; const char* error; int act ; bool resid, train ; int lnf ; };
inline int gemm_lnf(const GemmEpilogue& ep, bool f16) {
  return ep.ln_stats ? 1 : ((ep.rln_stats || ep.stats_out) ? (ep.out_lo ? (ep.lo8 && f16 ? 4 : 3) : 2) : 0);
}
inline bool gemm_whole_tiles(int64_t M, int64_t N, int64_t K) { return M % 256 == 0 && N % 256 == 0 && (K * 2) % 128 == 0; }
bool omk_gemm_ln_fusable(int dtype, int64_t M, int64_t N, int64_t K);
unsigned long long* omk_debug_trace();
bool omk_gemm_tn_ok(int dtype, int64_t M, int64_t N, int64_t K, int64_t lda, int64_t ldb);
int omk_gemm_tn(int dtype, const void* A, int64_t lda, const void* B, int64_t ldb, float* C, int64_t ldc, float* bias,
                int64_t M, int64_t N, int64_t K, hipStream_t s);
bool omk_gemm_tn_batch_ok(int dtype, int64_t M, int64_t N, int64_t K, int64_t lda, int64_t ldb);
int omk_gemm_tn_batch(int dtype, const OmTnProblem* probs, int n, int64_t M, hipStream_t s);
bool omk_gemm_wide6_b16_has(int in_dtype, int out_dtype, int act, bool train, bool resid);
int omk_gemm_wide6_b16(int in_dtype, const void* A, int64_t lda, const void* B, int64_t ldb, int out_dtype,
                       void* C, int64_t ldc, int64_t M, int64_t N, int64_t K, const GemmEpilogue& ep, hipStream_t s);
bool omk_gemm_wide6_f32_has(int in_dtype, int out_dtype, int act, bool train, bool resid);
int omk_gemm_wide6_f32(int in_dtype, const void* A, int64_t lda, const void* B, int64_t ldb, int out_dtype,
                       void* C, int64_t ldc, int64_t M, int64_t N, int64_t K, const GemmEpilogue& ep, hipStream_t s);
int omk_gemm(int in_dtype, const void* A, int64_t lda, const void* B, int64_t ldb, int out_dtype,
             void* C, int64_t ldc, int64_t M, int64_t N, int64_t K, const GemmEpilogue& ep,
             hipStream_t s);
void omk_gemm_note(int family);

int omk_gemm_splitk(int in_dtype, const void* A, int64_t lda, const void* B, int64_t ldb, float* C,
                    int64_t ldc, int64_t M, int64_t N, int64_t K, hipStream_t s);

__host__ __device__ inline uint64_t om_hash64(uint64_t seed, uint64_t idx) {
  uint64_t x = idx * 0x9E3779B97F4A7C15ull + seed;
  x ^= x >> 32; x *= 0xD6E8FEB86659FD93ull;
  x ^= x >> 32; x *= 0xD6E8FEB86659FD93ull;
  x ^= x >> 32;
  return x;
}
struct DropCfg {
  uint32_t thresh;
  float keep_scale;
  __host__ __device__ explicit DropCfg(float p) {
    thresh = p > 0.f ? (uint32_t)(p * 65536.0f + 0.5f) : 0u;
    if (thresh > 65535u) thresh = 65535u;
    keep_scale = 65536.0f / (float)(65536u - thresh);
  }
};
__host__ __device__ inline uint64_t dropout_bits(uint64_t seed, uint64_t group) { return om_hash64(seed, group); }
__host__ __device__ inline bool dropout_field(uint64_t bits, int e, uint32_t thresh) {
  return ((uint32_t)(bits >> (16 * e)) & 0xffffu) >= thresh;
}
__host__ __device__ inline bool dropout_keep(uint64_t seed, uint64_t idx, uint32_t thresh) {
  return dropout_field(dropout_bits(seed, idx >> 2), (int)(idx & 3), thresh);
}
```

### openmatch_amd/native.py

```python
import ctypes as C
import os

import torch

_HERE = os.path.dirname(os.path.abspath(__file__))
LIB_PATH = os.path.join(_HERE, "csrc", "libopenmatch_hip.so")

OM_F32, OM_BF16, OM_F16 = 0, 1, 2
ACT_NONE, ACT_GELU_ERF, ACT_RELU, ACT_GELU_TANH = 0, 1, 2, 3
ACT_SILU = 5
ACT_MUL_RESID = 0x100
ACT_GELU_ERF_GRAD, ACT_PRE_GRAD = 4, 0x200
ARCH_BERT, ARCH_T5, ARCH_MODERNBERT, ARCH_CAUSAL, ARCH_NOMICBERT, ARCH_GEMMA3 = 0, 1, 2, 3, 4, 5
POOL_NONE, POOL_FIRST, POOL_MEAN, POOL_LAST = 0, 1, 2, 3
OPT_TRAIN_WGRAD_BATCH, OPT_GEMM_MAX_GRID, OPT_GEMM_CONT = 14, 15, 16
OPT_GEMM_GROUP_M, OPT_GEMM_VARIANT, OPT_GEMM_SKINNY_M = 6, 12, 19
GEMM_FAMILY = {"v1": 1, "v2": 2, "v6": 6, "g7": 7, "g7_one_tile": 70, "7c16": 71, "7r16": 72, "skinny": 9}
ATTN_FAMILY = {"generic": 1, "fwd16": 2, "fwd16_kmax4": 3, "fwd16c": 4, "long": 5, "d32": 6, "band16": 7, "band32": 8}
ATTN_BWD_FAMILY = {"bwd16": 1, "generic": 2, "long": 3, "d32": 4}
ENC_PATH = {"bert_fused": 1, "bert_pending_ln": 2, "bert_few32": 3, "bert_plain": 4, "modernbert": 5, "t5_fused": 6, "t5_plain": 7}
SCAN_FAMILY = {"dense": 0, "generic": 1, "wide": 2, "stream32": 3, "stream16": 4}
SCAN_FAMILY_NAME = {v: k for k, v in SCAN_FAMILY.items()}
OPT_SCAN_GEN7 = 3
OPT_ATTENTION_FAST = 2
SEARCH_F32, SEARCH_F16_RESCORE = 0, 1
ABI_VERSION = 6

c_void_p, c_int, c_int64, c_float, c_size_t = C.c_void_p, C.c_int, C.c_int64, C.c_float, C.c_size_t


class OmLayerWeights(C.Structure):
    _fields_ = [(n, c_void_p) for n in (
        "qkv_w", "qkv_b", "o_w", "o_b", "ln1_g", "ln1_b", "ffn1_w", "ffn1_b", "ffn1g_w",
        "ffn2_w", "ffn2_b", "ln2_g", "ln2_b")]


class OmEncoderConfig(C.Structure):
    _fields_ = [("arch", c_int), ("dtype", c_int), ("hidden", c_int), ("n_layers", c_int),
                ("n_heads", c_int), ("head_dim", c_int), ("ffn", c_int), ("vocab", c_int),
                ("max_pos", c_int), ("type_vocab", c_int), ("act", c_int), ("ln_eps", c_float),
                ("rel_buckets", c_int), ("rel_max_dist", c_int), ("pooling", c_int),
                ("head_in", c_int), ("head_out", c_int), ("normalize", c_int),
                ("rope_theta_global", c_float), ("rope_theta_local", c_float), ("half_window", c_int),
                ("sliding_layers", C.c_uint64)]


class OmCausalConfig(C.Structure):
    _fields_ = [("base", OmEncoderConfig), ("n_kv_heads", c_int), ("rope_attention_scaling", c_float), ("inv_freq", c_float * 32)]


class OmCausalConfig2(C.Structure):
    _fields_ = [("base", OmCausalConfig), ("qk_norm", c_int), ("reserved", c_int), ("inv_freq", c_float * 64)]


class OmCausalQkNorm(C.Structure):
    _fields_ = [("q_norm_g", c_void_p), ("k_norm_g", c_void_p)]


class OmGemma3Config(C.Structure):
    _fields_ = [("base", OmCausalConfig), ("attn_scale", c_float), ("half_window", c_int), ("sliding_layers", C.c_uint64),
                ("full_scaling", c_float), ("sliding_scaling", c_float), ("attn_logit_softcapping", c_float), ("bidirectional", c_int),
                ("full_inv_freq", c_float * 128), ("sliding_inv_freq", c_float * 128)]


class OmGemma3Norms(C.Structure):
    _fields_ = [(n, c_void_p) for n in ("q_norm_g", "k_norm_g", "post_attention_norm_g", "post_feedforward_norm_g")]


class OmEncoderWeights(C.Structure):
    _fields_ = [("word_emb", c_void_p), ("pos_emb", c_void_p), ("type_emb", c_void_p),
                ("emb_ln_g", c_void_p), ("emb_ln_b", c_void_p),
                ("layers_host", C.POINTER(OmLayerWeights)), ("final_ln_g", c_void_p),
                ("rel_bias", c_void_p), ("head_w", c_void_p), ("folded", c_void_p), ("final_ln_b", c_void_p)]


class OmTnProblem(C.Structure):
    _fields_ = [("A", c_void_p), ("B", c_void_p), ("C", c_void_p), ("bias", c_void_p),
                ("lda", c_int64), ("ldb", c_int64), ("ldc", c_int64), ("N", c_int64), ("K", c_int64)]


class OmT5DecoderLayer(C.Structure):
    _fields_ = [(n, c_void_p) for n in (
        "sa_v_w", "sa_o_w", "sa_ln_g", "ca_q_w", "ca_kv_w", "ca_o_w", "ca_ln_g", "ffn1_w", "ffn1g_w", "ffn2_w", "ffn_ln_g")]


class OmT5DecoderWeights(C.Structure):
    _fields_ = [("start_emb", c_void_p), ("final_ln_g", c_void_p),
                ("layers_host", C.POINTER(OmT5DecoderLayer)), ("n_layers", c_int)]


class OmT5DecoderLayerGrads(C.Structure):
    _fields_ = [(n, c_void_p) for n in (
        "sa_v_w", "sa_o_w", "sa_ln_g", "ca_q_w", "ca_kv_w", "ca_o_w", "ca_ln_g", "ffn1_w", "ffn1g_w", "ffn2_w", "ffn_ln_g")]


class OmT5DecoderGrads(C.Structure):
    _fields_ = [("start_emb", c_void_p), ("final_ln_g", c_void_p), ("layers_host", C.POINTER(OmT5DecoderLayerGrads))]


class OmAdamTensor(C.Structure):
    _fields_ = [("p", c_void_p), ("g", c_void_p), ("m", c_void_p), ("v", c_void_p), ("shadow0", c_void_p), ("shadow1", c_void_p),
                ("n", c_int64), ("weight_decay", c_float), ("shadow0_dtype", c_int), ("shadow1_dtype", c_int), ("reserved", c_int)]


class OmDebugGemmEpilogue(C.Structure):
    _fields_ = [("bias", c_void_p), ("resid", c_void_p), ("ldr", c_int64), ("act", c_int),
                ("pre_act", c_void_p), ("ldp", c_int64), ("drop_p", c_float), ("seed", C.c_uint64), ("drop_rows", c_void_p),
                ("ln_stats", c_void_p), ("ln_colsum", c_void_p), ("rln_stats", c_void_p), ("rln_g", c_void_p), ("rln_b", c_void_p),
                ("stats_out", c_void_p), ("resid_lo", c_void_p), ("out_lo", c_void_p), ("resid32", c_void_p), ("out32", c_void_p),
                ("a_ln32", c_void_p), ("a_ln_g", c_void_p), ("a_ln_b", c_void_p), ("a_ln_stats_out", c_void_p), ("rln32", c_void_p),
                ("rln32_stats", c_void_p), ("lo8", c_int), ("ln_inv_h", c_float), ("ln_eps", c_float), ("ln_rms", c_int),
                ("reverse", c_int), ("rows_dev", c_void_p)]


class OmLnSite(C.Structure):
    _fields_ = [("partial", c_void_p), ("dg", c_void_p), ("db", c_void_p), ("blocks", c_int)]


ROW_KERNEL = {"fwd_generic": 1, "fwd_x8": 2, "ln_bwd": 3}
OPT_TRAIN_WGRAD_STREAM = 8
ADAM_CHUNK = 16384


class OmLayerGrads(C.Structure):
    _fields_ = [(n, c_void_p) for n in (
        "qkv_w", "qkv_b", "o_w", "o_b", "ln1_g", "ln1_b", "ffn1_w", "ffn1_b", "ffn2_w", "ffn2_b",
        "ln2_g", "ln2_b", "ffn1g_w")]


class OmEncoderGrads(C.Structure):
    _fields_ = [("word_emb", c_void_p), ("pos_emb", c_void_p), ("type_emb", c_void_p),
                ("emb_ln_g", c_void_p), ("emb_ln_b", c_void_p),
                ("layers_host", C.POINTER(OmLayerGrads)), ("head_w", c_void_p),
                ("final_ln_g", c_void_p), ("rel_bias", c_void_p)]


_SIGNATURES = {
    "om_last_error": (C.c_char_p, []),
    "om_abi_version": (c_int, []),
    "om_device_count": (c_int, []),
    "om_debug_gemm_trace": (None, [c_void_p]),
    "om_debug_gemm_gen": (None, [c_int]),
    "om_debug_option": (c_int, [c_int, c_int]),
    "om_debug_option_value": (c_int, [c_int]),
    "om_debug_gemm_last": (c_int, []),
    "om_debug_gemm_plan": (c_int, [c_int, c_void_p, c_int64, c_void_p, c_int64, c_int, c_void_p, c_int64,
                                   c_int64, c_int64, c_int64, c_void_p, c_void_p, c_int64, c_int]),
    "om_debug_gemm_ex": (c_int, [c_int, c_void_p, c_int64, c_void_p, c_int64, c_int, c_void_p, c_int64,
                                 c_int64, c_int64, c_int64, C.POINTER(OmDebugGemmEpilogue), c_void_p]),
    "om_debug_gemm_plan_ex": (c_int, [c_int, c_void_p, c_int64, c_void_p, c_int64, c_int, c_void_p, c_int64,
                                      c_int64, c_int64, c_int64, C.POINTER(OmDebugGemmEpilogue)]),
    "om_debug_gemm_splitk": (c_int, [c_int, c_void_p, c_int64, c_void_p, c_int64, c_void_p, c_int64, c_int64, c_int64, c_int64, c_void_p]),
    "om_debug_attention": (c_int, [c_void_p, c_void_p, c_void_p, c_int64, c_int, c_int, c_int, c_void_p]),
    "om_debug_attention_ex": (c_int, [c_int, c_void_p, c_void_p, c_void_p, c_void_p, c_int64, c_int, c_int, c_int, c_float, c_float,
                                      C.c_uint64, c_void_p, c_int, c_void_p, c_void_p, c_int]),
    "om_debug_rope": (c_int, [c_int, c_void_p, c_int64, c_int, c_int, c_float, c_void_p]),
    "om_debug_rope_rows": (c_int, [c_int, c_void_p, c_int64, c_int, c_int, c_float, c_void_p, c_void_p]),
    "om_debug_swiglu_rows": (c_int, [c_int, c_void_p, c_void_p, c_int64, c_int, c_void_p]),
    "om_debug_embed": (c_int, [c_int, c_void_p, c_void_p, c_void_p, c_void_p, c_void_p, c_void_p, c_void_p, c_void_p, c_int64, c_int, c_int,
                               c_int, c_int, c_float, c_void_p]),
    "om_debug_attention_causal": (c_int, [c_int, c_void_p, c_void_p, c_void_p, c_int64, c_int, c_int, c_int, c_float, c_void_p]),
    "om_debug_rope_gqa": (c_int, [c_int, c_void_p, c_int64, c_int, c_int, c_int, C.POINTER(c_float), c_float, c_void_p]),
    "om_debug_attention_causal_packed": (c_int, [c_int, c_void_p, c_void_p, c_void_p, c_void_p, c_int64, c_int, c_int, c_int, c_float, c_void_p]),
    "om_debug_rope_gqa_rows": (c_int, [c_int, c_void_p, c_int64, c_int, c_int, c_int, C.POINTER(c_float), c_float, c_void_p, c_void_p]),
    "om_debug_attention_causal_hd": (c_int, [c_int, c_void_p, c_void_p, c_void_p, c_int64, c_int, c_int, c_int, c_int, c_float, c_void_p]),
    "om_debug_attention_causal_hd_packed": (c_int, [c_int, c_void_p, c_void_p, c_void_p, c_void_p, c_int64, c_int, c_int, c_int, c_int, c_float,
                                                    c_void_p]),
    "om_debug_qknorm_rope": (c_int, [c_int, c_void_p, c_int64, c_int, c_int, c_int, c_int, c_void_p, c_void_p, c_float, C.POINTER(c_float),
                                     c_float, c_void_p]),
    "om_debug_qknorm_rope_rows": (c_int, [c_int, c_void_p, c_int64, c_int, c_int, c_int, c_int, c_void_p, c_void_p, c_float, C.POINTER(c_float),
                                          c_float, c_void_p, c_void_p]),
    "om_debug_attention_gqa_d256": (c_int, [c_int, c_void_p, c_void_p, c_void_p, c_int64, c_int, c_int, c_int, c_float, c_int, c_void_p]),
    "om_debug_qknorm_rope_d256": (c_int, [c_int, c_void_p, c_int64, c_int, c_int, c_int, c_void_p, c_void_p, c_float, C.POINTER(c_float), c_float,
                                          c_void_p]),
    "om_debug_attention_gqa_d256_packed": (c_int, [c_int, c_void_p, c_void_p, c_void_p, c_void_p, c_int64, c_int, c_int, c_int, c_float, c_int,
                                                   c_void_p]),
    "om_debug_qknorm_rope_d256_rows": (c_int, [c_int, c_void_p, c_int64, c_int, c_int, c_int, c_void_p, c_void_p, c_float, C.POINTER(c_float),
                                               c_float, c_void_p, c_void_p]),
    "om_debug_rmsnorm_add": (c_int, [c_int, c_void_p, c_int64, c_void_p, c_int64, c_void_p, c_int64, c_int, c_float, c_void_p]),
    "om_debug_mask_extent": (c_int, [c_void_p, c_int64, c_int, c_void_p, c_void_p]),
    "om_debug_pack_rows": (c_int, [c_void_p, c_int64, c_int, c_int64, c_void_p, c_void_p, c_void_p, c_void_p]),
    "om_debug_attention_last": (c_int, []),
    "om_debug_attention_plan": (c_int, [c_int, c_int64, c_int, c_int, c_int, c_int, c_float, c_int, c_int, c_int]),
    "om_debug_attention_bwd_last": (c_int, []),
    "om_debug_attention_bwd_plan": (c_int, [c_int, c_int64, c_int, c_int, c_int, c_int, c_int, c_int, c_int]),
    "om_debug_attention_bwd_ex": (c_int, [c_int, c_void_p, c_void_p, c_void_p, c_void_p, c_void_p, c_void_p, c_void_p, c_void_p, c_int64, c_int,
                                          c_int, c_int, c_float, c_float, C.c_uint64, c_void_p, c_int, c_void_p]),
    "om_debug_attention_bwd_stats_bytes": (c_size_t, [c_int64, c_int]),
    "om_debug_encoder_plan": (c_int, [C.POINTER(OmEncoderConfig), c_int, c_int, c_int64, c_int64, c_int64, c_int]),
    "om_debug_encoder_skip_pad": (c_int, [C.POINTER(OmEncoderConfig), c_int, c_int, c_int64, c_int64, c_int]),
    "om_debug_encoder_cls_tail": (c_int, [C.POINTER(OmEncoderConfig), c_int, c_int, c_int64, c_int64, c_int64, c_int]),
    "om_debug_gather_rows": (c_int, [c_void_p, c_void_p, c_void_p, c_void_p, c_void_p, c_void_p, c_void_p, c_void_p, c_void_p, c_int64, c_int64,
                                     c_int64, c_int, c_void_p]),
    "om_debug_attn_drop_keep": (c_int, [C.c_uint64, c_int64, c_int, c_int, c_int, c_int, c_int, c_float]),
    "om_debug_wave_sum_check": (c_int, [c_void_p, c_void_p, c_void_p, c_int64, c_void_p]),
    "om_debug_row_kernel_last": (c_int, []),
    "om_debug_layernorm": (c_int, [c_int, c_void_p, c_int64, c_void_p, c_int64, c_void_p, c_void_p, c_int64, c_int, c_float, c_int, c_void_p,
                                   c_int, c_void_p]),
    "om_debug_layernorm_f32out": (c_int, [c_int, c_void_p, c_int64, c_void_p, c_int64, c_void_p, c_void_p, c_int64, c_int, c_float, c_int,
                                          c_void_p, c_void_p, c_int, c_void_p]),
    "om_debug_layernorm_from_f32": (c_int, [c_int, c_void_p, c_int64, c_void_p, c_int64, c_void_p, c_void_p, c_int64, c_int, c_float, c_int,
                                            c_void_p]),
    "om_debug_layernorm_dual": (c_int, [c_int, c_void_p, c_int64, c_void_p, c_void_p, c_int64, c_void_p, c_void_p, c_int64, c_int, c_float,
                                        c_void_p]),
    "om_debug_norm_bwd": (c_int, [c_int, c_void_p, c_void_p, c_void_p, c_void_p, c_void_p, c_void_p, c_int64, c_int, c_float, c_int, c_void_p,
                                  c_void_p]),
    "om_debug_ln_bwd_drop": (c_int, [c_int, c_void_p, c_void_p, c_void_p, c_void_p, c_void_p, c_float, C.c_uint64, c_void_p, c_void_p, c_int64,
                                     c_int, c_float, c_void_p, c_void_p, c_void_p, C.POINTER(c_int), c_void_p, c_void_p]),
    "om_debug_ln_param_reduce": (c_int, [C.POINTER(OmLnSite), c_int, c_int, c_void_p]),
    "om_debug_embed_bwd": (c_int, [c_int, c_void_p, c_void_p, c_void_p, c_void_p, c_void_p, c_void_p, c_void_p, c_void_p, c_void_p, c_void_p,
                                   c_void_p, c_void_p, c_int64, c_int, c_int, c_int, c_int, c_float, c_void_p, c_void_p]),
    "om_debug_pool": (c_int, [c_int, c_void_p, c_void_p, c_void_p, c_int64, c_int, c_int, c_int, c_void_p, c_void_p]),
    "om_debug_pool_bwd": (c_int, [c_int, c_void_p, c_void_p, c_void_p, c_int64, c_int, c_int, c_int, c_void_p, c_void_p]),
    "om_debug_l2norm": (c_int, [c_void_p, c_void_p, c_int64, c_int, c_void_p]),
    "om_debug_l2norm_bwd": (c_int, [c_void_p, c_void_p, c_void_p, c_int64, c_int, c_void_p]),
    "om_debug_colsum": (c_int, [c_int, c_void_p, c_int64, c_int64, c_int, c_void_p, c_void_p]),
    "om_debug_dropout": (c_int, [c_int, c_void_p, c_void_p, c_int64, c_float, C.c_uint64, c_void_p, c_int, c_void_p]),
    "om_debug_ln_fold": (c_int, [c_int, c_void_p, c_void_p, c_void_p, c_void_p, c_void_p, c_void_p, c_void_p, c_int, c_int, c_void_p]),
    "om_debug_ln_stats_reduce": (c_int, [c_void_p, c_int, c_int64, c_void_p, c_void_p]),
    "om_encoder_fold_bytes": (c_size_t, [C.POINTER(OmEncoderConfig)]),
    "om_encoder_fold_weights": (c_int, [C.POINTER(OmEncoderConfig), C.POINTER(OmEncoderWeights), c_void_p, c_size_t, c_void_p]),
    "om_kernel_timing_enable": (c_int, [c_int]),
    "om_kernel_timing_read": (c_int, [c_int, C.POINTER(C.c_double), C.POINTER(c_int64), C.POINTER(C.c_double)]),
    "om_gemm_nt": (c_int, [c_int, c_void_p, c_int64, c_void_p, c_int64, c_int, c_void_p, c_int64,
                           c_int64, c_int64, c_int64, c_void_p, c_void_p, c_int64, c_int, c_void_p]),
    "om_gemm_tn_acc": (c_int, [c_int, c_void_p, c_int64, c_void_p, c_int64, c_void_p, c_int64, c_void_p,
                               c_int64, c_int64, c_int64, c_void_p]),
    "om_gemm_tn_acc_batch": (c_int, [c_int, C.POINTER(OmTnProblem), c_int, c_int64, c_void_p]),
    "om_encoder_workspace_bytes": (c_size_t, [C.POINTER(OmEncoderConfig), c_int64, c_int64]),
    "om_t5_decoder_workspace_bytes": (c_size_t, [C.POINTER(OmEncoderConfig), c_int64, c_int64]),
    "om_t5_decoder_step": (c_int, [C.POINTER(OmEncoderConfig), C.POINTER(OmT5DecoderWeights), c_void_p, c_void_p,
                                   c_int64, c_int64, c_void_p, c_void_p, c_size_t, c_void_p]),
    "om_t5_relative_bucket": (c_int, [c_int, c_int, c_int]),
    "om_encoder_forward": (c_int, [C.POINTER(OmEncoderConfig), C.POINTER(OmEncoderWeights), c_void_p,
                                   c_void_p, c_void_p, c_int64, c_int64, c_void_p, c_void_p,
                                   c_void_p, c_size_t, c_void_p]),
    "om_causal_encoder_workspace_bytes": (c_size_t, [C.POINTER(OmCausalConfig), c_int64, c_int64]),
    "om_causal_encoder_forward": (c_int, [C.POINTER(OmCausalConfig), C.POINTER(OmEncoderWeights), c_void_p, c_void_p, c_int64, c_int64,
                                          c_void_p, c_void_p, c_void_p, c_size_t, c_void_p]),
    "om_causal_encoder_packed_supported": (c_int, [C.POINTER(OmCausalConfig), c_int64, c_int64, c_int64]),
    "om_causal_encoder_workspace_bytes_packed": (c_size_t, [C.POINTER(OmCausalConfig), c_int64, c_int64, c_int64]),
    "om_causal_encoder_forward_packed": (c_int, [C.POINTER(OmCausalConfig), C.POINTER(OmEncoderWeights), c_void_p, c_void_p, c_int64, c_int64,
                                                 c_int64, c_void_p, c_void_p, c_size_t, c_void_p]),
    "om_causal2_encoder_workspace_bytes": (c_size_t, [C.POINTER(OmCausalConfig2), c_int64, c_int64]),
    "om_causal2_encoder_forward": (c_int, [C.POINTER(OmCausalConfig2), C.POINTER(OmEncoderWeights), C.POINTER(OmCausalQkNorm), c_void_p, c_void_p,
                                           c_int64, c_int64, c_void_p, c_void_p, c_void_p, c_size_t, c_void_p]),
    "om_causal2_encoder_packed_supported": (c_int, [C.POINTER(OmCausalConfig2), c_int64, c_int64, c_int64]),
    "om_causal2_encoder_workspace_bytes_packed": (c_size_t, [C.POINTER(OmCausalConfig2), c_int64, c_int64, c_int64]),
    "om_causal2_encoder_forward_packed": (c_int, [C.POINTER(OmCausalConfig2), C.POINTER(OmEncoderWeights), C.POINTER(OmCausalQkNorm), c_void_p,
                                                  c_void_p, c_int64, c_int64, c_int64, c_void_p, c_void_p, c_size_t, c_void_p]),
    "om_gemma3_encoder_workspace_bytes": (c_size_t, [C.POINTER(OmGemma3Config), c_int64, c_int64]),
    "om_gemma3_encoder_forward": (c_int, [C.POINTER(OmGemma3Config), C.POINTER(OmEncoderWeights), C.POINTER(OmGemma3Norms), c_void_p, c_void_p,
                                          c_int64, c_int64, c_void_p, c_void_p, c_void_p, c_size_t, c_void_p]),
    "om_gemma3_encoder_packed_supported": (c_int, [C.POINTER(OmGemma3Config), c_int64, c_int64, c_int64]),
    "om_gemma3_encoder_workspace_bytes_packed": (c_size_t, [C.POINTER(OmGemma3Config), c_int64, c_int64, c_int64]),
    "om_gemma3_encoder_forward_packed": (c_int, [C.POINTER(OmGemma3Config), C.POINTER(OmEncoderWeights), C.POINTER(OmGemma3Norms), c_void_p,
                                                 c_void_p, c_int64, c_int64, c_int64, c_void_p, c_void_p, c_size_t, c_void_p]),
    "om_encoder_packed_supported": (c_int, [C.POINTER(OmEncoderConfig), c_int, c_int64, c_int64, c_int64]),
    "om_encoder_workspace_bytes_packed": (c_size_t, [C.POINTER(OmEncoderConfig), c_int64, c_int64, c_int64]),
    "om_encoder_forward_packed": (c_int, [C.POINTER(OmEncoderConfig), C.POINTER(OmEncoderWeights), c_void_p,
                                          c_void_p, c_void_p, c_int64, c_int64, c_int64, c_void_p,
                                          c_void_p, c_size_t, c_void_p]),
    "om_encoder_tape_bytes": (c_size_t, [C.POINTER(OmEncoderConfig), c_int64, c_int64]),
    "om_encoder_train_workspace_bytes": (c_size_t, [C.POINTER(OmEncoderConfig), c_int64, c_int64]),
    "om_encoder_train_forward": (c_int, [C.POINTER(OmEncoderConfig), C.POINTER(OmEncoderWeights), c_void_p,
                                         c_void_p, c_void_p, c_int64, c_int64, c_float, c_float, C.c_uint64,
                                         c_void_p, c_size_t, c_void_p, c_void_p, c_size_t, c_void_p]),
    "om_encoder_train_backward": (c_int, [C.POINTER(OmEncoderConfig), C.POINTER(OmEncoderWeights), c_void_p,
                                          c_void_p, c_void_p, c_int64, c_int64, c_float, c_float, C.c_uint64,
                                          c_void_p, c_void_p, C.POINTER(OmEncoderGrads), c_void_p, c_size_t,
                                          c_void_p]),
    "om_encoder_train_packed_supported": (c_int, [C.POINTER(OmEncoderConfig), c_int64, c_int64, c_int64]),
    "om_encoder_tape_bytes_packed": (c_size_t, [C.POINTER(OmEncoderConfig), c_int64, c_int64, c_int64]),
    "om_encoder_train_workspace_bytes_packed": (c_size_t, [C.POINTER(OmEncoderConfig), c_int64, c_int64, c_int64]),
    "om_encoder_train_forward_packed": (c_int, [C.POINTER(OmEncoderConfig), C.POINTER(OmEncoderWeights), c_void_p,
                                                c_void_p, c_void_p, c_int64, c_int64, c_int64, c_float, c_float, C.c_uint64,
                                                c_void_p, c_size_t, c_void_p, c_void_p, c_size_t, c_void_p]),
    "om_encoder_train_backward_packed": (c_int, [C.POINTER(OmEncoderConfig), C.POINTER(OmEncoderWeights), c_void_p,
                                                 c_void_p, c_void_p, c_int64, c_int64, c_int64, c_float, c_float, C.c_uint64,
                                                 c_void_p, c_void_p, C.POINTER(OmEncoderGrads), c_void_p, c_size_t,
                                                 c_void_p]),
    "om_encoder_train_forward_hidden": (c_int, [C.POINTER(OmEncoderConfig), C.POINTER(OmEncoderWeights), c_void_p,
                                                c_void_p, c_void_p, c_int64, c_int64, c_float, c_float, C.c_uint64,
                                                c_void_p, c_size_t, c_void_p, c_void_p, c_size_t, c_void_p]),
    "om_encoder_train_backward_hidden": (c_int, [C.POINTER(OmEncoderConfig), C.POINTER(OmEncoderWeights), c_void_p,
                                                 c_void_p, c_void_p, c_int64, c_int64, c_float, c_float, C.c_uint64,
                                                 c_void_p, c_void_p, C.POINTER(OmEncoderGrads), c_void_p, c_size_t,
                                                 c_void_p]),
    "om_t5_decoder_tape_bytes": (c_size_t, [C.POINTER(OmEncoderConfig), c_int, c_int64, c_int64]),
    "om_t5_decoder_train_workspace_bytes": (c_size_t, [C.POINTER(OmEncoderConfig), c_int, c_int64, c_int64]),
    "om_t5_decoder_train_forward": (c_int, [C.POINTER(OmEncoderConfig), C.POINTER(OmT5DecoderWeights), c_void_p, c_void_p,
                                            c_int64, c_int64, c_float, C.c_uint64, c_void_p, c_size_t, c_void_p,
                                            c_void_p, c_size_t, c_void_p]),
    "om_t5_decoder_train_backward": (c_int, [C.POINTER(OmEncoderConfig), C.POINTER(OmT5DecoderWeights), c_void_p, c_void_p,
                                             c_int64, c_int64, c_float, C.c_uint64, c_void_p, c_void_p,
                                             C.POINTER(OmT5DecoderGrads), c_void_p, c_void_p, c_size_t, c_void_p]),
    "om_linear_f32_backward": (c_int, [c_void_p, c_void_p, c_void_p, c_void_p, c_void_p, c_int, c_int, c_int, c_void_p]),
    "om_index_to_f16": (c_int, [c_void_p, c_int64, c_int, c_void_p, c_void_p, c_void_p]),
    "om_sim_topk_workspace_bytes": (c_size_t, [c_int64, c_int, c_int]),
    "om_sim_topk": (c_int, [c_int, c_void_p, c_int64, c_void_p, c_void_p, c_void_p, c_int64, c_int,
                            c_int, c_int64, c_void_p, c_void_p, c_void_p, c_size_t, c_void_p]),
    "om_sim_topk_info": (None, [C.POINTER(c_int64)]),
    "om_debug_scan_plan": (c_int, [c_int, c_int64, c_int, C.POINTER(c_int)]),
    "om_debug_sim_stream": (c_int, [c_void_p, c_int64, C.c_uint32, c_void_p, c_int64, c_int, c_void_p, c_void_p, c_void_p, c_int, c_void_p]),
    "om_topk_merge": (c_int, [c_void_p, c_void_p, c_int, c_int64, c_int, c_int, c_void_p, c_void_p,
                              c_void_p]),
    "om_contrastive_fwd_bwd": (c_int, [c_void_p, c_void_p, c_int, c_int, c_int, c_int, c_float,
                                       c_int, c_int, c_int, c_int, c_void_p, c_void_p, c_void_p,
                                       c_void_p, c_void_p, c_void_p]),
    "om_encoder_train_set_layer_events": (c_int, [c_void_p, c_int]),
    "om_comm_unique_id": (c_int, [c_void_p]),
    "om_comm_init": (c_int, [c_void_p, c_int, c_int, C.POINTER(c_void_p)]),
    "om_comm_destroy": (c_int, [c_void_p]),
    "om_comm_count": (c_int, [c_void_p, C.POINTER(c_int)]),
    "om_allgather_rows": (c_int, [c_void_p, c_void_p, c_void_p, c_int64, c_int64, c_void_p]),
    "om_allreduce_grads": (c_int, [c_void_p, c_void_p, c_int64, c_int, c_void_p]),
    "om_exchange_topk": (c_int, [c_void_p, c_int, c_void_p, c_void_p, c_int64, c_int, c_void_p, c_void_p, c_void_p]),
    "om_grad_sqnorm": (c_int, [c_void_p, c_void_p, c_int, c_void_p, c_void_p, c_void_p]),
    "om_adamw_step": (c_int, [c_void_p, c_void_p, c_int, c_float, c_float, c_float, c_float, c_int64, c_void_p, c_float, c_float,
                              c_int, c_void_p, c_void_p]),
    "om_loss_scale_update": (c_int, [c_void_p, c_void_p, c_int, c_void_p]),
    "om_contrastive_fwd_bwd_ex": (c_int, [c_void_p, c_void_p, c_int, c_int, c_int, c_void_p, c_int, c_int, c_void_p,
                                          c_float, c_int, c_int, c_int, c_int, c_void_p, c_void_p, c_void_p,
                                          c_void_p, c_void_p, c_void_p]),
}

_lib = None


class NativeError(RuntimeError):
    pass


def lib():
    global _lib
    if _lib is None:
        if not os.path.exists(LIB_PATH):
            raise NativeError(
                f"{LIB_PATH} is missing: build the HIP library first "
                "(python -m openmatch_amd._build, or __graft_entry__.build()). "
                "openmatch_amd has no CPU / eager fallback.")
        handle = C.CDLL(LIB_PATH)
        for name, (res, args) in _SIGNATURES.items():
            try:
                fn = getattr(handle, name)
            except AttributeError as e:
                raise NativeError(f"{LIB_PATH} does not export {name}; rebuild it") from e
            fn.restype, fn.argtypes = res, args
        if handle.om_abi_version() != ABI_VERSION:
            raise NativeError("libopenmatch_hip.so ABI version mismatch; rebuild it")
        _lib = handle
    return _lib


def exported_symbols():
    return list(_SIGNATURES)


def check(rc):
    if rc != 0:
        raise NativeError(lib().om_last_error().decode("utf-8", "replace"))


def require_device(*tensors):
    for t in tensors:
        if t is None:
            continue
        if not t.is_cuda:
            raise NativeError(
                "openmatch_amd runs on MI355X only: got a CPU tensor. Move the model and the batch "
                "to the GPU (model.to('cuda')); there is no CPU / eager fallback.")
        if not t.is_contiguous():
            raise NativeError("non-contiguous tensor passed to the HIP boundary")


def ptr(t):
    return c_void_p(t.data_ptr()) if t is not None else c_void_p(0)


def stream_ptr(device=None):
    return c_void_p(torch.cuda.current_stream(device).cuda_stream)


class Workspace:
    _pool = {}

    @classmethod
    def get(cls, device, nbytes, tag="default"):
        key = (str(device), tag)
        buf = cls._pool.get(key)
        if buf is None or buf.numel() - ((-buf.data_ptr()) % 256) < nbytes:
            buf = torch.empty(int(nbytes) + 256, dtype=torch.uint8, device=device)
            cls._pool[key] = buf
        off = (-buf.data_ptr()) % 256
        return buf, buf.data_ptr() + off
```

Measured before the change: 73210 passages/s.

## Fork fused BERT encoder batch into two concurrent stream lanes

Splits a large fused-BERT encode batch into two halves that each run the full layer chain on separate HIP streams: the caller's stream and a cached non-blocking side stream, joined with events. Each lane works on its own slice of the workspace, and GEMM planning sees the whole-batch row count so both lanes pick the same kernel families. A dry-run probe compares these families against the unsplit chain and falls back if they differ, if the stream is being captured, or if timing is on. The aim is to overlap low-occupancy phases (attention, LN stat reductions, gathers) of one half with GEMMs of the other, at the cost of extra launches and possible contention between the two lanes.

```diff
diff --git a/include/openmatch_hip.h b/include/openmatch_hip.h
--- a/include/openmatch_hip.h
+++ b/include/openmatch_hip.h
@@ -99,7 +99,8 @@
 #define OM_OPT_FEW_ROWS_LN_FUSE 21
 #define OM_OPT_ENCODER_SKIP_PAD 22
 #define OM_OPT_ENCODER_CLS_TAIL 23
-#define OM_OPT_COUNT 24
+#define OM_OPT_ENCODER_LANES 24
+#define OM_OPT_COUNT 25
 int om_debug_option(int opt, int value);
 int om_debug_option_value(int opt);
 int om_debug_attention(const void* qkv, void* ctx, const int64_t* mask, int64_t B, int L, int H, int heads, void* stream);
@@ -170,6 +171,12 @@
 int om_debug_encoder_skip_pad(const struct OmEncoderConfig* cfg, int gated_ffn, int has_rel_bias, int64_t B, int64_t L, int want_hidden);
 int om_debug_encoder_cls_tail(const struct OmEncoderConfig* cfg, int gated_ffn, int has_rel_bias, int64_t B, int64_t L, int64_t packed_rows,
                               int want_hidden);
+int om_debug_encoder_lanes(const struct OmEncoderConfig* cfg, int gated_ffn, int has_rel_bias, int64_t B, int64_t L, int64_t packed_rows,
+                           int want_hidden, int64_t* B0);
+#define OM_ENCODER_LANE_RANGES 15
+int om_debug_encoder_lane_ranges(const struct OmEncoderConfig* cfg, int gated_ffn, int has_rel_bias, int64_t B, int64_t L, int lane,
+                                 int64_t* out, int cap);
+int64_t om_debug_encoder_lane_forks(void);
 int om_debug_gather_rows(const void* src0, void* dst0, const void* src1, void* dst1, const void* src2, void* dst2, const float* stats_src,
                          float* stats_dst, const int* rows, int64_t B, int64_t L, int64_t Mc, int H, void* stream);
 int om_debug_attn_drop_keep(uint64_t seed, int64_t b, int h, int heads, int Lm, int q, int key, float p);
diff --git a/openmatch_amd/csrc/abi.cpp b/openmatch_amd/csrc/abi.cpp
--- a/openmatch_amd/csrc/abi.cpp
+++ b/openmatch_amd/csrc/abi.cpp
@@ -116,6 +116,8 @@
   g_opt[OM_OPT_ENCODER_SKIP_PAD] = e ? atoi(e) : 1;
   e = getenv("OM_ENCODER_CLS_TAIL");
   g_opt[OM_OPT_ENCODER_CLS_TAIL] = e ? atoi(e) : 1;
+  e = getenv("OM_ENCODER_LANES");
+  g_opt[OM_OPT_ENCODER_LANES] = e ? atoi(e) : 65536;
   g_opt_init.store(true);
 }
 }
diff --git a/openmatch_amd/csrc/encoder.hip b/openmatch_amd/csrc/encoder.hip
--- a/openmatch_amd/csrc/encoder.hip
+++ b/openmatch_amd/csrc/encoder.hip
@@ -3,6 +3,7 @@
 #include <stdlib.h>
 
 #include <algorithm>
+#include <atomic>
 #include <map>
 #include <mutex>
 #include <utility>
@@ -221,6 +222,8 @@
   hipStream_t s;
   const int* rows_dev;
   int64_t cls_mc;
+  std::vector<int>* families;
+  int64_t whole_mg, whole_mc;
 };
 
 struct EncStream {
@@ -262,6 +265,15 @@
   const int nslots = 2 * (H / 256);
   const bool pingpong = k.p.pingpong;
   int walk = 1;
+  const bool probe = k.families != nullptr;
+  auto gemm = [&](const void* A, int64_t lda, const void* W, int64_t ldw, void* C, int64_t ldc, int64_t rows, int64_t N, int64_t K,
+                  const GemmEpilogue& ep) {
+    const int64_t as = rows == Mg ? k.whole_mg : k.whole_mc;
+    if (!probe) return omk_gemm(dt, A, lda, W, ldw, dt, C, ldc, rows, N, K, ep, s, as);
+    k.families->push_back(omk_gemm_family(dt, A, lda, W, ldw, dt, C, ldc, rows, N, K, ep, as));
+    return 0;
+  };
+#define LAUNCH(expr) do { if (!probe) RUN(expr); } while (0)
   const int64_t Mc = k.cls_mc;
   const size_t cplane = (size_t)Mc * H * 2;
   char* const cbase = ws.qkv;
@@ -283,19 +295,20 @@
     GemmEpilogue e = {};
     if (l == 0) {
       e.bias = lw.qkv_b; e.reverse = OM_WALK(); e.rows_dev = k.rows_dev;
-      RUN(omk_gemm(dt, ws.x, H, lw.qkv_w, H, dt, ws.qkv, 3 * H, Mg, 3 * H, H, e, s));
+      RUN(gemm(ws.x, H, lw.qkv_w, H, ws.qkv, 3 * H, Mg, 3 * H, H, e));
     } else {
       const OmLayerWeights& pw = Ls[l - 1];
       const void* wf; const float *cs, *bfp;
       RUN(folded_weights(c, k.w, l, false, lw.qkv_w, pw.ln2_g, pw.ln2_b, lw.qkv_b, 3 * H, H, ws.wfold, ws.colsum, ws.bfold, s, &wf, &cs, &bfp));
       e.bias = bfp; e.ln_stats = st2p; e.ln_colsum = cs; e.ln_inv_h = inv_h; e.ln_eps = c->ln_eps; e.reverse = OM_WALK(); e.rows_dev = k.rows_dev;
-      RUN(omk_gemm(dt, ws.x1, H, wf, H, dt, ws.qkv, 3 * H, Mg, 3 * H, H, e, s));
+      RUN(gemm(ws.x1, H, wf, H, ws.qkv, 3 * H, Mg, 3 * H, H, e));
     }
-    NOMIC_ROPE();
-    RUN(omk_attention(dt, ws.qkv, ws.ctx, k.mask, k.posbias, B, (int)L, H, nh, scale, 0.f, 0, s, OM_WALK(), ws.kmax, k.cu));
+    if (!probe) NOMIC_ROPE();
+    const int attn_walk = OM_WALK();
+    LAUNCH(omk_attention(dt, ws.qkv, ws.ctx, k.mask, k.posbias, B, (int)L, H, nh, scale, 0.f, 0, s, attn_walk, ws.kmax, k.cu));
     if (tail) {
       const GatherPlane planes[3] = {{ws.ctx, cbase}, {ws.x1, cbase + cplane}, {two ? ws.x1_lo : nullptr, cbase + 2 * cplane}};
-      RUN(omk_gather_rows(planes, st2p, cst2p, k.cu ? ws.cls_rows : nullptr, B, L, Mc, H, s));
+      LAUNCH(omk_gather_rows(planes, st2p, cst2p, k.cu ? ws.cls_rows : nullptr, B, L, Mc, H, s));
       ctx = cbase; xin = cbase + cplane; xin_lo = cbase + 2 * cplane; st2p = cst2p;
       y = cbase + 3 * cplane; y_lo = cbase + 4 * cplane; xout = cbase + 5 * cplane; xout_lo = cbase + 6 * cplane;
     }
@@ -310,23 +323,24 @@
       if (two) e.resid_lo = xin_lo;
     }
     e.reverse = OM_WALK(); e.rows_dev = rdev;
-    RUN(omk_gemm(dt, ctx, H, lw.o_w, H, dt, y, H, Mr, H, H, e, s));
-    RUN(omk_ln_stats_reduce(ws.slots, nslots, Mr, st1, s));
+    RUN(gemm(ctx, H, lw.o_w, H, y, H, Mr, H, H, e));
+    LAUNCH(omk_ln_stats_reduce(ws.slots, nslots, Mr, st1, s));
     const void* wf1; const float *cs1, *bf1;
     RUN(folded_weights(c, k.w, l, true, lw.ffn1_w, lw.ln1_g, lw.ln1_b, lw.ffn1_b, F1, H, ws.wfold, ws.colsum, ws.bfold, s, &wf1, &cs1, &bf1));
     e = GemmEpilogue{};
     e.bias = bf1; e.act = act1; e.ln_stats = st1; e.ln_colsum = cs1; e.ln_inv_h = inv_h; e.ln_eps = c->ln_eps;
     e.reverse = OM_WALK(); e.rows_dev = rdev;
-    RUN(omk_gemm(dt, y, H, wf1, H, dt, ws.ff, F1, Mr, F1, H, e, s));
-    NOMIC_SWIGLU(Mr);
+    RUN(gemm(y, H, wf1, H, ws.ff, F1, Mr, F1, H, e));
+    if (!probe) NOMIC_SWIGLU(Mr);
     e = GemmEpilogue{};
     e.bias = lw.ffn2_b; e.resid = y; e.ldr = H; e.rln_stats = st1; e.rln_g = lw.ln1_g; e.rln_b = lw.ln1_b;
     e.stats_out = ws.slots; e.ln_inv_h = inv_h; e.ln_eps = c->ln_eps;
     if (two) { e.resid_lo = y_lo; e.out_lo = xout_lo; e.lo8 = lo8; }
     e.reverse = OM_WALK(); e.rows_dev = rdev;
-    RUN(omk_gemm(dt, ffa, F, lw.ffn2_w, F, dt, xout, H, Mr, H, F, e, s));
-    if (!last) RUN(omk_ln_stats_reduce(ws.slots, nslots, Mg, st2, s));
-  }
+    RUN(gemm(ffa, F, lw.ffn2_w, F, xout, H, Mr, H, F, e));
+    if (!last) LAUNCH(omk_ln_stats_reduce(ws.slots, nslots, Mg, st2, s));
+  }
+#undef LAUNCH
 #undef OM_WALK
   const OmLayerWeights& lastw = Ls[c->n_layers - 1];
   *out = EncStream{ws.x1, two ? ws.x1_lo : nullptr, lo8, lastw.ln2_g, lastw.ln2_b, 0, ws.x};
@@ -574,6 +588,172 @@
   return 0;
 }
 
+struct EncChain {
+  const OmEncoderConfig* c;
+  const OmEncoderWeights* w;
+  const int64_t *input_ids, *attention_mask, *token_type_ids;
+  void* out_hidden;
+  float* out_reps;
+  EncPlanIn in;
+  EncPlan plan;
+  EncSwitches sw;
+  EncWs ws;
+  hipStream_t s;
+  int* side;
+  int64_t whole_mg, whole_mc;
+};
+
+static EncWs lane_view(const OmEncoderConfig* c, const EncWs& w, const EncPlan& lane, int h, int64_t B0, int64_t L) {
+  const size_t H = c->hidden, F = c->ffn, F1 = enc_ffn1_cols(c), es = 2;
+  const size_t row0 = h ? (size_t)(B0 * L) : 0, seq0 = h ? (size_t)B0 : 0;
+  EncWs v = {};
+  v.x = w.x + row0 * H * es; v.y = w.y + row0 * H * es; v.x1 = w.x1 + row0 * H * es;
+  v.qkv = w.qkv + row0 * 3 * H * es;
+  v.ctx = w.ctx + row0 * H * es;
+  v.ff = w.ff + row0 * F1 * es;
+  v.ff2 = c->arch == OM_ARCH_NOMICBERT ? w.ff2 + row0 * F * es : w.ff2;
+  v.y_lo = w.y_lo + row0 * H * es; v.x1_lo = w.x1_lo + row0 * H * es;
+  v.pooled = w.pooled + seq0 * H;
+  v.headout = w.headout + seq0 * (size_t)(c->head_out > 0 ? c->head_out : 1);
+  v.kmax = w.kmax + seq0;
+  v.final32 = w.final32 + (c->pooling == OM_POOL_FIRST ? seq0 : row0) * H;
+  v.stats1 = w.stats1 + 4 * (size_t)c->n_layers * row0;
+  v.stats2 = v.stats1 + (size_t)c->n_layers * (size_t)lane.Mg * 2;
+  v.slots = w.slots + 4 * ((H + 255) / 256) * row0;
+  v.total = w.total;
+  return v;
+}
+
+static void lane_ranges(const OmEncoderConfig* c, const EncWs& v, const EncPlan& lane, int64_t Bh, const char* base, int64_t* out) {
+  const size_t H = c->hidden, F = c->ffn, F1 = enc_ffn1_cols(c), es = 2, M = (size_t)lane.Mp, B = (size_t)Bh;
+  const bool nomic = c->arch == OM_ARCH_NOMICBERT;
+  const std::pair<const void*, size_t> f[OM_ENCODER_LANE_RANGES] = {
+      {v.x, M * H * es}, {v.y, M * H * es}, {v.x1, M * H * es}, {v.qkv, M * 3 * H * es}, {v.ctx, M * H * es}, {v.ff, M * F1 * es},
+      {v.ff2, nomic ? M * F * es : 0}, {v.pooled, B * H * 4}, {v.headout, B * (size_t)(c->head_out > 0 ? c->head_out : 1) * 4}, {v.kmax, B * 4},
+      {v.final32, (c->pooling == OM_POOL_FIRST ? B : (size_t)lane.M) * H * 4}, {v.stats1, (size_t)2 * c->n_layers * M * 8},
+      {v.slots, (size_t)2 * ((H + 255) / 256) * M * 8}, {v.y_lo, M * H * es}, {v.x1_lo, M * H * es}};
+  for (int i = 0; i < OM_ENCODER_LANE_RANGES; ++i) {
+    out[2 * i] = (int64_t)((const char*)f[i].first - base);
+    out[2 * i + 1] = (int64_t)f[i].second;
+  }
+}
+
+extern "C" int om_debug_encoder_lanes(const OmEncoderConfig* c, int gated_ffn, int has_rel_bias, int64_t B, int64_t L, int64_t packed_rows,
+                                      int want_hidden, int64_t* B0) {
+  if (!c) {
+    om_set_error("om_debug_encoder_lanes: null argument");
+    return -1;
+  }
+  const EncPlanIn in = {c, B, L, packed_rows, want_hidden != 0, gated_ffn != 0, has_rel_bias != 0, c->type_vocab > 0};
+  const EncSwitches sw = encoder_switches();
+  return encoder_lanes(in, encoder_plan(in, sw), sw, B0) ? 1 : 0;
+}
+
+extern "C" int om_debug_encoder_lane_ranges(const OmEncoderConfig* c, int gated_ffn, int has_rel_bias, int64_t B, int64_t L, int lane,
+                                            int64_t* out, int cap) {
+  if (!c || !out || cap < 2 * OM_ENCODER_LANE_RANGES || (lane != 0 && lane != 1)) {
+    om_set_error("om_debug_encoder_lane_ranges: null argument, a lane other than 0 | 1, or room for fewer than 15 pairs");
+    return -1;
+  }
+  EncPlanIn in = {c, B, L, 0, false, gated_ffn != 0, has_rel_bias != 0, c->type_vocab > 0};
+  const EncSwitches sw = encoder_switches();
+  const EncPlan whole = encoder_plan(in, sw);
+  int64_t B0 = 0;
+  if (!encoder_lanes(in, whole, sw, &B0)) {
+    om_set_error("om_debug_encoder_lane_ranges: this call does not fork (om_debug_encoder_lanes)");
+    return -1;
+  }
+  static char origin[1];
+  const EncWs ws = carve(c, whole, B, L, 0, origin);
+  in.B = lane ? B - B0 : B0;
+  const EncPlan lp = encoder_plan_checked(in, sw);
+  lane_ranges(c, lane_view(c, ws, lp, lane, B0, L), lp, in.B, origin, out);
+  return OM_ENCODER_LANE_RANGES;
+}
+
+static std::atomic<int64_t> g_lane_forks{0};
+extern "C" int64_t om_debug_encoder_lane_forks(void) { return g_lane_forks.load(); }
+
+struct LaneStream { hipStream_t side = nullptr; hipEvent_t fork = nullptr, join = nullptr; };
+static int lane_stream(hipStream_t s, LaneStream* out) {
+  static std::mutex mu;
+  static std::map<std::pair<int, hipStream_t>, LaneStream> lanes;
+  int dev = 0;
+  OM_HIP(hipGetDevice(&dev));
+  std::lock_guard<std::mutex> lk(mu);
+  LaneStream& l = lanes[std::make_pair(dev, s)];
+  if (!l.side) {
+    LaneStream n;
+    OM_HIP(hipStreamCreateWithFlags(&n.side, hipStreamNonBlocking));
+    OM_HIP(hipEventCreateWithFlags(&n.fork, hipEventDisableTiming));
+    OM_HIP(hipEventCreateWithFlags(&n.join, hipEventDisableTiming));
+    l = n;
+  }
+  *out = l;
+  return 0;
+}
+
+static int encoder_chain(const EncChain& q, std::vector<int>* families);
+
+static int encoder_fork(const EncChain& whole, int* forked) {
+  *forked = 0;
+  const OmEncoderConfig* c = whole.c;
+  const int64_t B = whole.in.B, L = whole.in.L;
+  int64_t B0 = 0;
+  if (!whole.w->folded || om_timing_on() || !encoder_lanes(whole.in, whole.plan, whole.sw, &B0)) return 0;
+  hipStreamCaptureStatus st = hipStreamCaptureStatusNone;
+  if (hipStreamIsCapturing(whole.s, &st) != hipSuccess) {
+    (void)hipGetLastError();
+    return 0;
+  }
+  if (st != hipStreamCaptureStatusNone) return 0;
+  LaneStream ls;
+  RUN(lane_stream(whole.s, &ls));
+  const bool skip = encoder_skip_pad(whole.in, whole.plan, whole.sw);
+  int64_t whole_mc = 0;
+  if (!encoder_cls_tail(whole.in, whole.plan, whole.sw, &whole_mc)) whole_mc = 0;
+  const int64_t D =c->head_in > 0 && whole.w->head_w ? c->head_out : c->hidden;
+  EncChain lane[2] = {whole, whole};
+  for (int h = 0; h < 2; ++h) {
+    EncChain& q = lane[h];
+    const int64_t seq0 = h ? B0 : 0;
+    q.in.B = h ? B - B0 : B0;
+    q.plan = encoder_plan_checked(q.in, q.sw);
+    q.ws = lane_view(c, whole.ws, q.plan, h, B0, L);
+    q.input_ids += seq0 * L; q.attention_mask += seq0 * L;
+    if (q.token_type_ids) q.token_type_ids += seq0 * L;
+    q.out_reps += seq0 * D;
+    if (h) q.s = ls.side;
+    q.whole_mg = whole.plan.Mg; q.whole_mc = whole_mc;
+    q.side = nullptr;
+    if (skip) {
+      RUN(skip_pad_buffer(q.s, (size_t)(q.plan.Mp + 2 * q.in.B + 2), &q.side));
+      if (!q.side) return 0;
+    }
+  }
+  if (lane[0].plan.Mp != B0 * L || lane[0].plan.Mp + lane[1].plan.Mp != whole.plan.Mp) return 0;
+  EncChain ask = whole;
+  ask.side = lane[0].side;
+  std::vector<int> fam_whole, fam_lane[2];
+  if (encoder_chain(ask, &fam_whole) || encoder_chain(lane[0], &fam_lane[0]) || encoder_chain(lane[1], &fam_lane[1])) return 0;
+  if (fam_lane[0] != fam_whole || fam_lane[1] != fam_whole || std::find_if(fam_whole.begin(), fam_whole.end(), [](int f) { return f <= 0; }) != fam_whole.end())
+    return 0;
+
+  OM_HIP(hipEventRecord(ls.fork, whole.s));
+  OM_HIP(hipStreamWaitEvent(ls.side, ls.fork, 0));
+  *forked = 1;
+  g_lane_forks.fetch_add(1);
+  int rc = encoder_chain(lane[0], nullptr);
+  if (!rc) rc = encoder_chain(lane[1], nullptr);
+  hipError_t e = hipEventRecord(ls.join, ls.side);
+  if (e == hipSuccess) e = hipStreamWaitEvent(whole.s, ls.join, 0);
+  if (e != hipSuccess) {
+    (void)hipStreamSynchronize(ls.side);
+    if (!rc) OM_FAIL(std::string("encoder lanes: join failed: ") + hipGetErrorString(e));
+  }
+  return rc;
+}
+
 static int encoder_forward_impl(const OmEncoderConfig* c, const OmEncoderWeights* w,
                                 const int64_t* input_ids, const int64_t* attention_mask,
                                 const int64_t* token_type_ids, int64_t B, int64_t L,
@@ -588,8 +768,7 @@
                              w->type_emb != nullptr};
   const EncSwitches sw = encoder_switches();
   const EncPlan plan = encoder_plan_checked(plan_in, sw);
-  const bool bert = enc_bert_family(c);
-  if (om_option(OM_OPT_ENCODER_DEBUG) && plan.path && bert)
+  if (om_option(OM_OPT_ENCODER_DEBUG) && plan.path && enc_bert_family(c))
     fprintf(stderr, "om_encoder_forward: M=%ld fused_ln=%d packed=%d few_rows=%d pending_ln=%d L=%ld head_dim=%d rel_bias=%d\n", (long)plan.M,
             (int)(plan.path == OM_ENC_PATH_BERT_FUSED), (int)(packed_rows > 0), (int)plan.few_rows, (int)(plan.path == OM_ENC_PATH_BERT_PENDING_LN), (long)L,
             c->head_dim, (int)plan.rel_bias);
@@ -600,27 +779,49 @@
   if (c->arch == OM_ARCH_MODERNBERT && (!w->emb_ln_g || !w->final_ln_g)) OM_FAIL("ModernBERT needs emb_ln_g and final_ln_g");
   if (c->arch == OM_ARCH_NOMICBERT && (!w->type_emb || w->pos_emb || w->rel_bias)) OM_FAIL("NomicBERT needs type_emb and takes no pos_emb or rel_bias");
   if (!workspace || ((uintptr_t)workspace & 255)) OM_FAIL("workspace must be 256-byte aligned");
-  EncWs ws = carve(c, plan, B, L, packed_rows, (char*)workspace);
-  if (ws.total > workspace_bytes) OM_FAIL("workspace too small");
+  EncChain whole = {c, w, input_ids, attention_mask, token_type_ids, out_hidden, out_reps, plan_in, plan, sw,
+                    carve(c, plan, B, L, packed_rows, (char*)workspace), (hipStream_t)stream, nullptr, 0, 0};
+  if (whole.ws.total > workspace_bytes) OM_FAIL("workspace too small");
   if (c->pooling != OM_POOL_NONE && !out_reps) OM_FAIL("out_reps required when pooling is set");
-  hipStream_t s = (hipStream_t)stream;
+  int forked = 0;
+  RUN(encoder_fork(whole, &forked));
+  if (forked) return 0;
+  if (encoder_skip_pad(plan_in, plan, sw)) RUN(skip_pad_buffer(whole.s, (size_t)(plan.Mp + 2 * B + 2), &whole.side));
+  return encoder_chain(whole, nullptr);
+}
+
+static int encoder_chain(const EncChain& q, std::vector<int>* families) {
+  const OmEncoderConfig* c = q.c; const OmEncoderWeights* w = q.w;
+  const int64_t *input_ids = q.input_ids, *attention_mask = q.attention_mask, *token_type_ids = q.token_type_ids;
+  void* const out_hidden = q.out_hidden; float* const out_reps = q.out_reps;
+  const EncPlanIn& plan_in = q.in; const EncPlan& plan = q.plan; const EncSwitches sw = q.sw;
+  const int64_t B = q.in.B, L = q.in.L, packed_rows = q.in.packed_rows;
+  const bool bert = enc_bert_family(c);
+  EncWs ws = q.ws;
+  hipStream_t s = q.s;
   const int dt = c->dtype, H = c->hidden;
   const int64_t M = plan.M;
   int64_t pack_bound = packed_rows;
-  bool skip = false;
-  if (encoder_skip_pad(plan_in, plan, sw)) {
-    int* side = nullptr;
-    RUN(skip_pad_buffer(s, (size_t)(plan.Mp + 2 * B + 2), &side));
-    if (side) {
-      skip = true;
-      pack_bound = plan.Mp;
-      ws.cu = side; ws.cls_rows = side + (B + 2); ws.row_map = ws.cls_rows + B;
-    }
+  const bool skip = q.side != nullptr;
+  if (skip) {
+    pack_bound = plan.Mp;
+    ws.cu = q.side; ws.cls_rows = q.side + (B + 2); ws.row_map = ws.cls_rows + B;
   }
   const bool packed = pack_bound > 0;
   int64_t cls_mc = 0;
   if (!encoder_cls_tail(plan_in, plan, sw, &cls_mc)) cls_mc = 0;
   const int* const row_map = packed ? ws.row_map : nullptr;
+  if (families) {
+    if (plan.path != OM_ENC_PATH_BERT_FUSED) OM_FAIL("encoder lanes: the fused BERT path only");
+    const EncCall k = {c, w, attention_mask, B, L, plan, ws, nullptr, packed ? ws.cu : nullptr, row_map, out_hidden, s, skip ? ws.cu + B : nullptr,
+                       cls_mc, families, q.whole_mg, q.whole_mc};
+    EncStream unused = {};
+    RUN(bert_fused(k, &unused));
+    if (c->head_in > 0 && w->head_w)
+      families->push_back(omk_gemm_family(OM_F32, ws.pooled, c->hidden, w->head_w, c->head_in, OM_F32, out_reps, c->head_out, B, c->head_out,
+                                          c->head_in, GemmEpilogue{}));
+    return 0;
+  }
 
   RUN(omk_mask_extent(attention_mask, B, (int)L, ws.kmax, s));
   if (packed) RUN(omk_pack_rows(ws.kmax, B, (int)L, pack_bound, ws.cu, ws.cls_rows, ws.row_map, s));
@@ -639,7 +840,7 @@
     RUN(omk_embed(dt, input_ids, nullptr, w->word_emb, nullptr, nullptr, nullptr, nullptr, ws.x, M, (int)L, H, c->vocab, 1, c->ln_eps, 0, s, row_map));
 
   const EncCall k = {c, w, attention_mask, B, L, plan, ws, plan.rel_bias ? ws.posbias : nullptr, packed ? ws.cu : nullptr, row_map, out_hidden, s,
-                     skip ? ws.cu + B : nullptr, cls_mc};
+                     skip ? ws.cu + B : nullptr, cls_mc, nullptr, q.whole_mg, q.whole_mc};
   EncStream stream_out = {};
   switch (plan.path) {
     case OM_ENC_PATH_BERT_FUSED: RUN(bert_fused(k, &stream_out)); break;
diff --git a/openmatch_amd/csrc/encoder_plan.h b/openmatch_amd/csrc/encoder_plan.h
--- a/openmatch_amd/csrc/encoder_plan.h
+++ b/openmatch_amd/csrc/encoder_plan.h
@@ -14,12 +14,13 @@
   int attention_fast;
   int skip_pad;
   int cls_tail;
+  int lanes;
 };
 
 static EncSwitches encoder_switches() {
   return EncSwitches{om_option(OM_OPT_ENCODER_FUSED_LN), om_option(OM_OPT_ENCODER_TWO_PLANE), om_option(OM_OPT_ENCODER_PINGPONG),
                      om_option(OM_OPT_GEMM_SKINNY_M), om_option(OM_OPT_FEW_ROWS_LN_FUSE), om_option(OM_OPT_ATTENTION_FAST),
-                     om_option(OM_OPT_ENCODER_SKIP_PAD), om_option(OM_OPT_ENCODER_CLS_TAIL)};
+                     om_option(OM_OPT_ENCODER_SKIP_PAD), om_option(OM_OPT_ENCODER_CLS_TAIL), om_option(OM_OPT_ENCODER_LANES)};
 }
 
 struct EncPlanIn {
@@ -182,3 +183,24 @@
   if (Mc) *Mc = mc;
   return true;
 }
+
+static const int64_t ENC_LANE_ROWS_END = 131072;
+static bool encoder_lanes(const EncPlanIn& in, const EncPlan& p, const EncSwitches sw, int64_t* B0 = nullptr) {
+  if (sw.lanes <= 0 || in.packed_rows != 0 || in.want_hidden || in.has_rel_bias || in.c->pooling == OM_POOL_NONE) return false;
+  if (p.error || p.path != OM_ENC_PATH_BERT_FUSED || p.rel_bias || in.B < 2 || in.L < 1) return false;
+  int64_t step = 256;
+  for (int64_t l = in.L; step > 1 && l % 2 == 0; l /= 2) step /= 2;
+  const int64_t b0 = in.B / 2 / step * step;
+  if (b0 <= 0 || b0 * in.L < (int64_t)sw.lanes || (in.B - b0) * in.L < (int64_t)sw.lanes) return false;
+  if ((in.B - b0) * in.L >= ENC_LANE_ROWS_END) return false;
+  const bool skip = encoder_skip_pad(in, p, sw), tail = encoder_cls_tail(in, p, sw);
+  for (const int64_t bh : {b0, in.B - b0}) {
+    EncPlanIn li = in;
+    li.B = bh;
+    const EncPlan lp = encoder_plan_checked(li, sw);
+    if (lp.error || lp.path != p.path || lp.two != p.two || lp.lo8 != p.lo8 || lp.pingpong != p.pingpong) return false;
+    if (encoder_skip_pad(li, lp, sw) != skip || encoder_cls_tail(li, lp, sw) != tail) return false;
+  }
+  if (B0) *B0 = b0;
+  return true;
+}
diff --git a/openmatch_amd/csrc/gemm.hip b/openmatch_amd/csrc/gemm.hip
--- a/openmatch_amd/csrc/gemm.hip
+++ b/openmatch_amd/csrc/gemm.hip
@@ -102,10 +102,12 @@
                     int64_t K, const GemmEpilogue& ep, hipStream_t s);
 
 int omk_gemm(int in_dtype, const void* A, int64_t lda, const void* B, int64_t ldb, int out_dtype, void* C, int64_t ldc, int64_t M,
-             int64_t N, int64_t K, const GemmEpilogue& ep_in, hipStream_t s) {
+             int64_t N, int64_t K, const GemmEpilogue& ep_in, hipStream_t s, int64_t plan_m) {
   GemmEpilogue ep = ep_in;
   ep.trace = g_trace, g_gemm_last = 0;
-  const GemmPlan p = gemm_plan(in_dtype, (uintptr_t)A, lda, (uintptr_t)B, ldb, out_dtype, (uintptr_t)C, ldc, M, N, K, ep, gemm_switches(g_debug_gen));
+  GemmSwitches sw = gemm_switches(g_debug_gen);
+  sw.plan_m = plan_m;
+  const GemmPlan p = gemm_plan(in_dtype, (uintptr_t)A, lda, (uintptr_t)B, ldb, out_dtype, (uintptr_t)C, ldc, M, N, K, ep, sw);
   if (p.error) OM_FAIL(p.error);
 #define OM_GEMM_GO(TI, TO)                                                                                      \
   return p.family == OM_GEMM_FAMILY_V2 ? launch_gemm2<TI, TO>(A, lda, B, ldb, C, ldc, M, N, K, ep, s)           \
@@ -129,6 +131,14 @@
   }
 #undef OM_GEMM_GO
   OM_FAIL("the plan names no launcher");
+}
+
+int omk_gemm_family(int in_dtype, const void* A, int64_t lda, const void* B, int64_t ldb, int out_dtype, const void* C, int64_t ldc, int64_t M,
+                    int64_t N, int64_t K, const GemmEpilogue& ep, int64_t plan_m) {
+  GemmSwitches sw = gemm_switches(g_debug_gen);
+  sw.plan_m = plan_m;
+  const GemmPlan p = gemm_plan(in_dtype, (uintptr_t)A, lda, (uintptr_t)B, ldb, out_dtype, (uintptr_t)C, ldc, M, N, K, ep, sw);
+  return p.error ? -1 : p.family;
 }
 
 extern "C" int om_debug_gemm_plan(int in_dtype, const void* A, int64_t lda, const void* B, int64_t ldb, int out_dtype, void* C,
diff --git a/openmatch_amd/csrc/gemm_plan.h b/openmatch_amd/csrc/gemm_plan.h
--- a/openmatch_amd/csrc/gemm_plan.h
+++ b/openmatch_amd/csrc/gemm_plan.h
@@ -11,10 +11,11 @@
   int cont;
   int skinny_m;
   int debug_gen;
+  int64_t plan_m;
 };
 
 static GemmSwitches gemm_switches(int debug_gen) {
-  return GemmSwitches{om_option(OM_OPT_GEMM_VARIANT), om_option(OM_OPT_GEMM_CONT), om_option(OM_OPT_GEMM_SKINNY_M), debug_gen};
+  return GemmSwitches{om_option(OM_OPT_GEMM_VARIANT), om_option(OM_OPT_GEMM_CONT), om_option(OM_OPT_GEMM_SKINNY_M), debug_gen, 0};
 }
 
 static bool g7_ring_ok(int64_t K) { return K * 2 >= 3 * 128; }
@@ -65,8 +66,9 @@
                     (!p.resid || (ep.ldr % vec == 0 && ((uintptr_t)ep.resid & 15) == 0));
   int gen = 1;
   if (wide) {
+    const int64_t Mt = sw.plan_m > 0 ? sw.plan_m : M;
     auto rounds = [&](int64_t bm, int64_t bn, int64_t slots) {
-      const int64_t tiles = ((M + bm - 1) / bm) * ((N + bn - 1) / bn);
+      const int64_t tiles = ((Mt + bm - 1) / bm) * ((N + bn - 1) / bn);
       return (double)((tiles + slots - 1) / slots);
     };
     const double c4 = N >= 256 ? rounds(256, 256, 256) * (256.0 * 256.0) / 1.00 : 1e30;
diff --git a/openmatch_amd/csrc/kernels.h b/openmatch_amd/csrc/kernels.h
--- a/openmatch_amd/csrc/kernels.h
+++ b/openmatch_amd/csrc/kernels.h
@@ -133,7 +133,9 @@
                        void* C, int64_t ldc, int64_t M, int64_t N, int64_t K, const GemmEpilogue& ep, hipStream_t s);
 int omk_gemm(int in_dtype, const void* A, int64_t lda, const void* B, int64_t ldb, int out_dtype,
              void* C, int64_t ldc, int64_t M, int64_t N, int64_t K, const GemmEpilogue& ep,
-             hipStream_t s);
+             hipStream_t s, int64_t plan_m = 0);
+int omk_gemm_family(int in_dtype, const void* A, int64_t lda, const void* B, int64_t ldb, int out_dtype, const void* C, int64_t ldc, int64_t M,
+                    int64_t N, int64_t K, const GemmEpilogue& ep, int64_t plan_m = 0);
 void omk_gemm_note(int family);
 
 int omk_gemm_splitk(int in_dtype, const void* A, int64_t lda, const void* B, int64_t ldb, float* C,
diff --git a/openmatch_amd/native.py b/openmatch_amd/native.py
--- a/openmatch_amd/native.py
+++ b/openmatch_amd/native.py
@@ -190,6 +190,9 @@
     "om_debug_encoder_plan": (c_int, [C.POINTER(OmEncoderConfig), c_int, c_int, c_int64, c_int64, c_int64, c_int]),
     "om_debug_encoder_skip_pad": (c_int, [C.POINTER(OmEncoderConfig), c_int, c_int, c_int64, c_int64, c_int]),
     "om_debug_encoder_cls_tail": (c_int, [C.POINTER(OmEncoderConfig), c_int, c_int, c_int64, c_int64, c_int64, c_int]),
+    "om_debug_encoder_lanes": (c_int, [C.POINTER(OmEncoderConfig), c_int, c_int, c_int64, c_int64, c_int64, c_int, C.POINTER(c_int64)]),
+    "om_debug_encoder_lane_ranges": (c_int, [C.POINTER(OmEncoderConfig), c_int, c_int, c_int64, c_int64, c_int, C.POINTER(c_int64), c_int]),
+    "om_debug_encoder_lane_forks": (c_int64, []),
     "om_debug_gather_rows": (c_int, [c_void_p, c_void_p, c_void_p, c_void_p, c_void_p, c_void_p, c_void_p, c_void_p, c_void_p, c_int64, c_int64,
                                      c_int64, c_int, c_void_p]),
     "om_debug_attn_drop_keep": (c_int, [C.c_uint64, c_int64, c_int, c_int, c_int, c_int, c_int, c_float]),
```

Measured after the change: 75490 passages/s (median of 6 runs). 3.1% higher.
